# yutongwangBIT/multi_orbslam3

Hardware: AMD Instinct MI355X
Metric: tracking+localBA frames/sec (aggregate over agents; 1 agent per GPU) (higher is better)
Workload: dtype u8/int32 (ORB front-end, Hamming), f64 (local BA)

## Files before the change

include/orbgpu.h:

```cpp
#ifndef ORBGPU_H_
#define ORBGPU_H_

#include <stdint.h>

#ifdef __cplusplus
extern "C" {
#endif

enum {
  ORBG_OK = 0,
  ORBG_EMPTY = -1,
  ORBG_BAD_ARG = -2,
  ORBG_CAP_EXCEEDED = -3,
  ORBG_HIP_ERROR = -4,
  ORBG_NO_DEVICE = -5,
  ORBG_INTERNAL = -6
};

enum {
  LBA_APPLIED = 0,
  LBA_ABORTED_BEFORE_OPT = 1,
  LBA_REJECTED_OUTLIERS = 2
};

// ... 4 lines not shown
#define ORBG_MAX_FRAME_FEATURES 65535


typedef struct orbx_config {
  int32_t n_features;
  float   scale_factor;
  int32_t n_levels;
  int32_t ini_th_fast;
  int32_t min_th_fast;
  int32_t max_width;
  int32_t max_height;
  int32_t n_cams;
  int32_t device;
  int32_t gauss_taps[4];
  int32_t octree_oldest_first;
} orbx_config;

typedef struct orbx_keypoint {
  float   x, y;
  float   size;
  float   angle;
  float   response;
  int32_t octave;
} orbx_keypoint;

typedef struct orbx_handle orbx_handle;

int orbx_create(const orbx_config* cfg, orbx_handle** out);
int orbx_destroy(orbx_handle* h);

int orbx_get_tables(const orbx_handle* h, float* scale, float* inv_scale, float* sigma2,
                    float* inv_sigma2, int32_t* features_per_level);

int orbx_extract(orbx_handle* h, int cam, const uint8_t* img, int width, int height, int stride,
                 int lap0, int lap1, orbx_keypoint* kps, uint8_t* desc, int cap, int* n, int* n_mono);

int orbx_extract_stereo(orbx_handle* h, const uint8_t* img_left, const uint8_t* img_right,
                        int width, int height, int stride,
                        orbx_keypoint* kps_left, uint8_t* desc_left, int cap_left, int* n_left,
                        orbx_keypoint* kps_right, uint8_t* desc_right, int cap_right, int* n_right);

int orbx_extract_stereo_dev(orbx_handle* h, const uint8_t* d_img_left, const uint8_t* d_img_right,
                            int width, int height, int stride,
                            orbx_keypoint* kps_left, uint8_t* desc_left, int cap_left, int* n_left,
                            orbx_keypoint* kps_right, uint8_t* desc_right, int cap_right, int* n_right);

int orbx_get_level(orbx_handle* h, int cam, int level, uint8_t* host_out, int* width, int* height);
int orbx_get_level_bordered(orbx_handle* h, int cam, int level, uint8_t* host_out, int* width, int* height);

int orbx_get_candidates(orbx_handle* h, int cam, int level, int32_t* xys, int cap, int* n);

int orbx_stereo_match(orbx_handle* h, float bf, float b, float* uright, float* depth);


typedef struct orbm_frame_view {
  int32_t n;
  const orbx_keypoint* kps;
  const uint8_t* desc;
  const float* uright;
  const float* depth;
  float min_x, max_x, min_y, max_y;
  float fx, fy, cx, cy, bf, b;
  int32_t n_levels;
  float   scale_factor;
} orbm_frame_view;

typedef struct orbm_frame orbm_frame;

int orbm_frame_create(int device, int cap_features, orbm_frame** out);
int orbm_frame_destroy(orbm_frame* f);
int orbm_frame_upload(orbm_frame* f, const orbm_frame_view* view);
int orbm_frame_from_extractor(orbm_frame* f, orbx_handle* h, const orbm_frame_view* view);
int orbx_frame_stereo(orbx_handle* h, orbm_frame* frame, const orbm_frame_view* view, const uint8_t* img_left,
                      const uint8_t* img_right, int width, int height, int stride, float bf, float b,
                      orbx_keypoint* kps_left, uint8_t* desc_left, float* uright, float* depth, int cap_left,
                      int* n_left, int* n_right);
int orbx_frame_stereo_dev(orbx_handle* h, orbm_frame* frame, const orbm_frame_view* view, const uint8_t* d_img_left,
                          const uint8_t* d_img_right, int width, int height, int stride, float bf, float b,
                          orbx_keypoint* kps_left, uint8_t* desc_left, float* uright, float* depth, int cap_left,
                          int* n_left, int* n_right);
int orbx_frame_stereo_dev_submit(orbx_handle* h, orbm_frame* frame, const orbm_frame_view* view, const uint8_t* d_img_left,
                                 const uint8_t* d_img_right, int width, int height, int stride, float bf, float b);
int orbx_frame_stereo_dev_wait(orbx_handle* h, int* n_left, int* n_right);
#define ORBX_SUBMIT_ASYNC 1
int orbx_set_frame_outputs(orbx_handle* h, orbx_keypoint* kps_left, uint8_t* desc_left, float* uright, float* depth, int cap_left);
int orbx_frame_stereo_submit(orbx_handle* h, orbm_frame* frame, const orbm_frame_view* view, const uint8_t* img_left,
                             const uint8_t* img_right, int width, int height, int stride, float bf, float b, int flags);
int orbx_frame_stereo_wait(orbx_handle* h, int* n_left, int* n_right);
typedef struct orbx_distortion { float k1, k2, p1, p2, k3; } orbx_distortion;
int orbx_frame_mono(orbx_handle* h, orbm_frame* frame, const orbm_frame_view* view, const orbx_distortion* dist, const uint8_t* img,
                    int width, int height, int stride, orbx_keypoint* kps, orbx_keypoint* kps_un, uint8_t* desc, int cap, int* n);
int orbx_frame_mono_dev(orbx_handle* h, orbm_frame* frame, const orbm_frame_view* view, const orbx_distortion* dist, const uint8_t* d_img,
                        int width, int height, int stride, orbx_keypoint* kps, orbx_keypoint* kps_un, uint8_t* desc, int cap, int* n);
int orbx_frame_mono_submit(orbx_handle* h, orbm_frame* frame, const orbm_frame_view* view, const orbx_distortion* dist, const uint8_t* img,
                           int width, int height, int stride, int flags);
int orbx_frame_mono_dev_submit(orbx_handle* h, orbm_frame* frame, const orbm_frame_view* view, const orbx_distortion* dist,
                               const uint8_t* d_img, int width, int height, int stride);
int orbx_frame_mono_wait(orbx_handle* h, int* n);
int orbx_set_frame_outputs_un(orbx_handle* h, orbx_keypoint* kps_un );
int orbx_undistort_points(int device, const float* xy_in, int n, float fx, float fy, float cx, float cy, const orbx_distortion* dist,
                          float* xy_out);
int orbm_frame_get_grid(orbm_frame* f, int32_t* cell_start , int32_t* cell_items );

int orbm_hamming_matrix(int device, const uint8_t* q, int nq, const uint8_t* t, int nt, int32_t* dist);
int orbm_hamming_best2(int device, const uint8_t* q, int nq, const uint8_t* t, int nt, int32_t* out4);

typedef struct orbm_mappoints_view {
  int32_t m;
  const uint8_t* track_in_view;
  const uint8_t* bad;
  const float* proj_x;
  const float* proj_y;
  const float* proj_xr;
  const float* track_depth;
  const int32_t* scale_level;
  const float* view_cos;
  const uint8_t* desc;
  const int32_t* n_obs;
} orbm_mappoints_view;

typedef struct orbm_worldpoints_view {
  int32_t m;
  const float* pos;
  const float* normal;
  const float* min_dist;
  const float* max_dist;
  const uint8_t* desc;
  const int32_t* n_obs;
  const uint8_t* bad;
  const uint8_t* skip;
} orbm_worldpoints_view;

int orbm_is_in_frustum(orbm_frame* f, const float* Tcw , const orbm_worldpoints_view* pts,
                       float viewing_cos_limit, uint8_t* track_in_view, float* proj_x, float* proj_y,
                       float* proj_xr, float* track_depth, int32_t* scale_level, float* view_cos);

int orbm_search_by_projection_mps(orbm_frame* f, const orbm_mappoints_view* mps, float th,
                                  int far_points, float th_far_points, float nnratio,
                                  int32_t* assigned_mp, int32_t* assigned_obs, int* nmatches);

typedef struct orbm_map orbm_map;
int orbm_map_create(int device, int cap_points, orbm_map** out);
int orbm_map_destroy(orbm_map* m);
int orbm_map_upload(orbm_map* m, const orbm_worldpoints_view* pts);
int orbm_map_set_observations(orbm_map* m, const int32_t* n_obs );
int orbm_search_local_points(orbm_frame* f, orbm_map* m, const float* Tcw, const uint8_t* skip ,
                             float th, int far_points, float th_far_points, float nnratio,
                             int32_t* assigned_mp, int32_t* assigned_obs, int* nmatches);
int orbm_search_local_points_vis(orbm_frame* f, orbm_map* m, const float* Tcw, const uint8_t* skip ,
                                 float th, int far_points, float th_far_points, float nnratio,
                                 int32_t* assigned_mp, int32_t* assigned_obs, int* nmatches, uint8_t* in_frustum );

typedef struct orbm_lastframe_view {
  int32_t n;
  const uint8_t* mp_valid;
  const uint8_t* outlier;
  const float* world_pos;
  const uint8_t* desc;
  const int32_t* octave;
  const float* angle;
  const int32_t* n_obs;
  float Tcw[16];
} orbm_lastframe_view;

int orbm_search_by_projection_frame(orbm_frame* cur, const float* Tcw_cur, const orbm_lastframe_view* last,
                                    float th, int mono, int check_orientation,
                                    int32_t* assigned_mp, int32_t* assigned_obs, int* nmatches);

typedef struct orbm_lastview orbm_lastview;
int orbm_lastview_create(int device, int cap_features, orbm_lastview** out);
int orbm_lastview_destroy(orbm_lastview* v);
int orbm_lastview_upload(orbm_lastview* v, const orbm_lastframe_view* last);
int orbm_search_by_projection_frame_resident(orbm_frame* cur, const float* Tcw_cur, orbm_lastview* last, float th, int mono,
                                             int check_orientation, int32_t* assigned_mp, int32_t* assigned_obs, int* nmatches);

typedef struct orbm_featvec_view {
  int32_t n_nodes;
  const uint32_t* node_id;
  const uint32_t* start;
  const uint32_t* feat_idx;
} orbm_featvec_view;

int orbm_search_by_bow(orbm_frame* f, const orbm_featvec_view* fv_frame,
                       const uint8_t* kf_desc, int nkf, const uint8_t* kf_mp_valid, const float* kf_angle,
                       const orbm_featvec_view* fv_kf, float nnratio, int check_orientation,
                       int32_t* matches, int* nmatches);

int orbm_search_by_projection_sim3(orbm_frame* kf, orbm_map* pts, const float* Scw ,
                                   const uint8_t* already_found, int th, float ratio_hamming, int camera_project,
                                   int32_t* matched, int* nmatches);

int orbm_search_by_projection_reloc(orbm_frame* cur, orbm_map* kf_points, const float* Tcw_cur , const uint8_t* already_found ,
                                    const float* kf_angle , float th, int orb_dist, int check_orientation,
                                    int32_t* assigned_mp, int* nmatches);
struct orbg_camera;
int orbm_search_by_projection_sim3_cam(orbm_frame* kf, orbm_map* pts, const float* Scw , const struct orbg_camera* cam,
                                       const uint8_t* already_found, int th, float ratio_hamming, int32_t* matched, int* nmatches);
int orbm_search_by_projection_reloc_cam(orbm_frame* cur, orbm_map* kf_points, const float* Tcw_cur , const struct orbg_camera* cam,
                                        const uint8_t* already_found , const float* kf_angle , float th, int orb_dist,
                                        int check_orientation, int32_t* assigned_mp, int* nmatches);
int orbm_search_by_bow_kf(orbm_frame* kf2, const orbm_featvec_view* fv2, const uint8_t* mp_valid2,
                          const uint8_t* desc1, int n1, const uint8_t* mp_valid1, const float* angle1,
                          const orbm_featvec_view* fv1, float nnratio, int check_orientation,
                          int32_t* matches12, int* nmatches);

typedef struct orbm_sim3_problem {
  uint32_t struct_size;
  int32_t  n;
  const float* X3Dc1;
  const float* X3Dc2;
  const uint32_t* max_err1;
  const uint32_t* max_err2;
  float fx1, fy1, cx1, cy1;
  float fx2, fy2, cx2, cy2;
  int32_t camera_model1, camera_model2;
  int32_t fix_scale;
} orbm_sim3_problem;

typedef struct orbm_sim3_params {
  double  probability;
  int32_t min_inliers;
  int32_t max_iterations;
} orbm_sim3_params;

typedef struct orbm_sim3_result {
  uint32_t struct_size;
  int32_t  no_more;
  int32_t  converged;
  int32_t  n_inliers;
  int32_t  iterations_done;
  int32_t  iterations_run;
  int32_t  improved_in_this_call;
  int32_t  best_iteration;
  int32_t  have_best;
  float    T12[16];
  float    R[9];
  float    t[3];
  float    s;
  uint8_t* inliers;
  int32_t* hyp_n_inliers;
  float*   hyp_T12;
  uint64_t* hyp_masks;
} orbm_sim3_result;

typedef struct orbm_sim3 orbm_sim3;

int orbm_sim3_create(int device, orbm_sim3** out);
int orbm_sim3_destroy(orbm_sim3* h);
int orbm_sim3_set_stream(orbm_sim3* h, void* hip_stream);
int orbm_sim3_set_problem(orbm_sim3* h, const orbm_sim3_problem* p);
int orbm_sim3_set_ransac_parameters(orbm_sim3* h, double probability, int min_inliers, int max_iterations);
int orbm_sim3_ransac_iterations(int n, double probability, int min_inliers, int max_iterations, int* out);
int orbm_sim3_resolve_draws(int n, const int32_t* draws, int n_iterations, int32_t* idx);
int orbm_sim3_iterate(orbm_sim3* h, int n_iterations, const int32_t* draws, orbm_sim3_result* result);
int orbm_sim3_solve_batch(int device, const orbm_sim3_problem* problems, int B, const orbm_sim3_params* params,
                          const int32_t* const* draws, orbm_sim3_result* results);

// ... 340 lines not shown
```

multi_orbslam3_amd/_capi.py:

```python
import ctypes as C
import os

import numpy as np

_HERE = os.path.dirname(os.path.abspath(__file__))
LIB_PATH = os.environ.get("ORBG_LIB") or os.path.join(_HERE, "liborbgpu.so")

ORBG_OK, ORBG_EMPTY, ORBG_BAD_ARG, ORBG_CAP_EXCEEDED, ORBG_HIP_ERROR, ORBG_NO_DEVICE, ORBG_INTERNAL = 0, -1, -2, -3, -4, -5, -6
LBA_APPLIED, LBA_ABORTED_BEFORE_OPT, LBA_REJECTED_OUTLIERS = 0, 1, 2
GRID_COLS, GRID_ROWS = 64, 48

u8p = C.POINTER(C.c_uint8)
i32p = C.POINTER(C.c_int32)
u32p = C.POINTER(C.c_uint32)
f32p = C.POINTER(C.c_float)
f64p = C.POINTER(C.c_double)

KEYPOINT_DTYPE = np.dtype([("x", "<f4"), ("y", "<f4"), ("size", "<f4"), ("angle", "<f4"),
                           ("response", "<f4"), ("octave", "<i4")])
EDGE_DTYPE = np.dtype([("pose", "<i4"), ("point", "<i4"), ("u", "<f4"), ("v", "<f4"), ("ur", "<f4"),
                       ("inv_sigma2", "<f4")])
assert KEYPOINT_DTYPE.itemsize == 24 and EDGE_DTYPE.itemsize == 24


# ... 136 lines not shown
                ("obs1", C.c_void_p), ("obs2", C.c_void_p), ("inv_sigma2_1", C.c_void_p), ("inv_sigma2_2", C.c_void_p),
                ("fx1", C.c_float), ("fy1", C.c_float), ("cx1", C.c_float), ("cy1", C.c_float),
                ("fx2", C.c_float), ("fy2", C.c_float), ("cx2", C.c_float), ("cy2", C.c_float),
                ("camera_model1", C.c_int32), ("camera_model2", C.c_int32), ("fix_scale", C.c_int32), ("th2", C.c_float),
                ("q", C.c_double * 4), ("t", C.c_double * 3), ("s", C.c_double), ("n_correspondences", C.c_int32)]


class Sim3OptResult(C.Structure):
    _fields_ = [("struct_size", C.c_uint32), ("n_in", C.c_int32), ("returned_early", C.c_int32), ("n_bad_round1", C.c_int32),
                ("q", C.c_double * 4), ("t", C.c_double * 3), ("s", C.c_double), ("removed", C.c_void_p),
                ("iters", C.c_int32 * 2), ("chi2", C.c_double * 2), ("trace", C.c_void_p), ("trace_cap", C.c_int32),
                ("trace_len", C.c_int32), ("edge_chi2", C.c_void_p)]


class NewPointsKF(C.Structure):
    _fields_ = [("struct_size", C.c_uint32), ("frame", C.c_void_p), ("featvec", FeatVecView), ("has_mp", C.c_void_p),
                ("keys_xy", C.c_void_p), ("Tcw", C.c_float * 12), ("Twc", C.c_float * 12), ("Ow", C.c_float * 3),
                ("fx", C.c_float), ("fy", C.c_float), ("cx", C.c_float), ("cy", C.c_float), ("invfx", C.c_float),
                ("invfy", C.c_float), ("mb", C.c_float), ("mbf", C.c_float), ("n_levels", C.c_int32),
                ("scale_factors", C.c_void_p), ("level_sigma2", C.c_void_p), ("scale_factor", C.c_float)]


class NewPointsParams(C.Structure):
    _fields_ = [("struct_size", C.c_uint32), ("only_stereo", C.c_int32), ("coarse", C.c_int32), ("check_orientation", C.c_int32),
                ("far_points", C.c_int32), ("th_far_points", C.c_float)]


NEWPOINTS_MAX_NEIGHBOURS = 64
(NP_ACCEPTED, NP_HAS_POINT, NP_NOT_STEREO, NP_NO_NODE, NP_NO_MATCH, NP_W_ZERO, NP_LOW_PARALLAX, NP_EMPTY, NP_Z1, NP_Z2, NP_REPROJ1,
 NP_REPROJ2, NP_DIST_ZERO, NP_FAR, NP_SCALE) = range(15)
NEWPOINTS_RECORD_DTYPE = np.dtype([("idx2", "<i4"), ("dist", "<i4"), ("status", "<i4"), ("x3D", "<f4", (3,)), ("w", "<f4"),
                                   ("cos_parallax", "<f4")])
NEWPOINT_DTYPE = np.dtype([("neighbour", "<i4"), ("idx1", "<i4"), ("idx2", "<i4"), ("x3D", "<f4", (3,))])
assert NEWPOINTS_RECORD_DTYPE.itemsize == 32 and NEWPOINT_DTYPE.itemsize == 24


class FuseKF(C.Structure):
    _fields_ = [("struct_size", C.c_uint32), ("frame", C.c_void_p), ("Tcw", C.c_float * 12), ("Ow", C.c_float * 3),
                ("Scw", C.c_float * 16), ("fx", C.c_float), ("fy", C.c_float), ("cx", C.c_float), ("cy", C.c_float),
                ("mbf", C.c_float), ("n_levels", C.c_int32), ("scale_factors", C.c_void_p), ("inv_level_sigma2", C.c_void_p),
                ("log_scale_factor", C.c_float)]


class FuseParams(C.Structure):
    _fields_ = [("struct_size", C.c_uint32), ("th", C.c_float), ("sim3_form", C.c_int32)]


FUSE_MAX_KEYFRAMES, FUSE_CAND_CAP = 512, 16
(FUSE_CANDIDATES, FUSE_NEG_DEPTH, FUSE_NOT_IN_IMAGE, FUSE_DISTANCE, FUSE_NORMAL, FUSE_EMPTY_WINDOW, FUSE_NO_CANDIDATE,
 FUSE_SKIPPED) = range(8)
FUSE_RECORD_DTYPE = np.dtype([("status", "<i4"), ("best_idx", "<i4"), ("best_dist", "<i4"), ("level", "<i4"), ("n_cand", "<i4")])
assert FUSE_RECORD_DTYPE.itemsize == 20


class PoseOptResult(C.Structure):
    _fields_ = [("Tcw", C.c_float * 16), ("outlier", C.c_void_p), ("n_inliers", C.c_int32), ("n_bad", C.c_int32),
                ("iters", C.c_int32 * 4), ("chi2", C.c_double * 4)]


def ptr(a):
    if a is None:
        return None
    assert a.flags["C_CONTIGUOUS"], "array must be C-contiguous"
    return a.ctypes.data


EXPORTED_SYMBOLS = [
    "orbx_create", "orbx_destroy", "orbx_get_tables", "orbx_extract", "orbx_extract_stereo",
    "orbx_extract_stereo_dev", "orbx_get_level", "orbx_get_level_bordered", "orbx_get_candidates", "orbx_stereo_match",
    "orbm_frame_create", "orbm_frame_destroy", "orbm_frame_upload", "orbm_frame_from_extractor", "orbx_frame_stereo_dev", "orbx_frame_stereo", "orbx_frame_stereo_dev_submit", "orbx_frame_stereo_dev_wait", "orbx_frame_stereo_submit", "orbx_frame_stereo_wait", "orbx_set_frame_outputs",
    "orbm_frame_get_grid", "orbm_hamming_matrix", "orbm_hamming_best2", "orbm_is_in_frustum",
    "orbm_search_by_projection_mps", "orbm_is_in_frustum_rig", "orbm_search_by_projection_mps_rig", "orbm_search_by_projection_frame_rig", "orbm_search_by_bow_rig", "orbx_fisheye_stereo_matches", "orbm_map_create", "orbm_map_destroy", "orbm_map_upload",
    "orbm_search_local_points", "orbm_search_local_points_vis", "orbm_search_by_projection_frame", "orbm_search_by_bow",
    "orbm_search_by_projection_sim3", "orbm_search_by_bow_kf",
    "orbv_vocab_create", "orbv_vocab_destroy", "orbv_text_load", "orbv_text_view", "orbv_text_free", "orbv_vocab_from_text", "orbv_transform", "orbv_transform_frame", "orbv_bow_assemble",
    "orbm_distinctive_descriptors", "orbv_score_l1", "orbk_wire_bytes", "orbk_pack_frame", "orbk_frame_from_wire",
    "orbm_frame_download",
    "lba_solve", "lba_create", "lba_destroy", "lba_solve_h", "lba_solve_async", "lba_wait", "pose_optimize",
    "lba_solve_b", "lba_solve_hb", "lba_solve_async_b",
    "lba_set_profiling", "lba_get_solver_stats", "lba_event_overhead", "lba_get_watchdog_count",
    "orbd_database_create", "orbd_database_destroy", "orbd_detect_n_best_candidates",
    "orbx_set_stream", "orbm_frame_set_stream", "orbm_map_set_stream", "lba_set_stream", "orbv_vocab_set_stream", "orbd_database_set_stream",
    "pose_opt_set_stream", "orbx_get_ctor_timeline", "orbm_map_set_observations", "orbm_search_by_projection_reloc", "orbm_search_by_projection_reloc_cam", "orbm_search_by_projection_sim3_cam", "orbm_lastview_create", "orbm_lastview_destroy", "orbm_lastview_upload",
    "orbm_search_by_projection_frame_resident", "orbg_quiesce", "orbg_set_wait_policy", "orbg_get_wait_policy",
    "orbx_frame_mono", "orbx_frame_mono_dev", "orbx_frame_mono_submit", "orbx_frame_mono_dev_submit", "orbx_frame_mono_wait",
    "orbx_set_frame_outputs_un", "orbx_undistort_points",
    "orbm_sim3_create", "orbm_sim3_destroy", "orbm_sim3_set_stream", "orbm_sim3_set_problem", "orbm_sim3_set_ransac_parameters",
    "orbm_sim3_ransac_iterations", "orbm_sim3_resolve_draws", "orbm_sim3_iterate", "orbm_sim3_solve_batch",
    "orbm_sim3_optimize", "orbm_sim3_optimize_batch",
    "orbm_create_new_points", "orbm_search_for_triangulation", "orbm_fuse",
    "orbg_version", "orbg_strerror", "orbg_device_count", "orbx_get_timings", "orbx_event_overhead", "orbx_set_profile_interval", "orbx_set_profile_kernel", "orbx_get_fast_kernel_stats", "orbx_set_profiling",
]

_lib = None


class OrbGpuError(RuntimeError):
    def __init__(self, code, where=""):
        self.code = code
        msg = "orbgpu error %d" % code
        try:
            msg += " (%s)" % load().orbg_strerror(code).decode()
        except Exception:
            pass
        super().__init__(msg + (" in " + where if where else ""))


def load():
    global _lib
    if _lib is not None:
        return _lib
    if not os.path.exists(LIB_PATH):
        raise ImportError("liborbgpu.so not built: run `python -c 'import __graft_entry__ as g; g.build()'` "
                          "(expected at %s). There is no CPU fallback." % LIB_PATH)
    try:
        import torch
    except ImportError:
        pass
    lib = C.CDLL(LIB_PATH)
    lib.orbg_version.restype = C.c_char_p
    lib.orbg_strerror.restype = C.c_char_p
    lib.orbg_strerror.argtypes = [C.c_int]
    lib.orbm_sim3_ransac_iterations.argtypes = [C.c_int, C.c_double, C.c_int, C.c_int, C.c_void_p]
    lib.orbm_sim3_set_ransac_parameters.argtypes = [C.c_void_p, C.c_double, C.c_int, C.c_int]
    lib.orbm_sim3_optimize.argtypes = [C.c_int, C.c_void_p, C.c_void_p]
    lib.orbm_sim3_optimize_batch.argtypes = [C.c_int, C.c_void_p, C.c_int, C.c_void_p]
    lib.orbm_create_new_points.argtypes = [C.c_void_p, C.c_void_p, C.c_int, C.c_void_p, C.c_void_p, C.c_int, C.c_void_p, C.c_void_p, C.c_void_p]
    lib.orbm_search_for_triangulation.argtypes = [C.c_void_p, C.c_void_p, C.c_void_p, C.c_void_p, C.c_int, C.c_void_p]
    lib.orbm_fuse.argtypes = [C.c_void_p, C.c_int, C.c_void_p, C.c_void_p, C.c_void_p, C.c_void_p, C.c_void_p]
    for name in EXPORTED_SYMBOLS:
        fn = getattr(lib, name)
        if name not in ("orbg_version", "orbg_strerror"):
            fn.restype = C.c_int
    _lib = lib
    return lib


def check(code, where=""):
    if code != ORBG_OK:
        raise OrbGpuError(code, where)
```

multi_orbslam3_amd/api.py:

```python
import ctypes as C

import numpy as np

from . import _capi as capi
from . import views


def _vp(a):
    return None if a is None else C.c_void_p(a.ctypes.data)


class ORBextractor:

    def __init__(self, nfeatures=1000, scaleFactor=1.2, nlevels=8, iniThFAST=20, minThFAST=7, max_width=640,
                 max_height=480, n_cams=1, device=0, gauss_taps=None, octree_oldest_first=False):
        self.lib = capi.load()
        self.cfg = capi.OrbxConfig(nfeatures, scaleFactor, nlevels, iniThFAST, minThFAST, max_width, max_height,
                                   n_cams, device, (C.c_int32 * 4)(*(gauss_taps or (0, 0, 0, 0))), int(bool(octree_oldest_first)))
        self.h = C.c_void_p()
        capi.check(self.lib.orbx_create(C.byref(self.cfg), C.byref(self.h)), "orbx_create")
        self.cap = 2 * nfeatures + 256

    def close(self):
        if getattr(self, "h", None):
# ... 65 lines not shown
        if download_left:
            return nl.value, nr.value, kl[: nl.value], dl[: nl.value]
        return nl.value, nr.value

    def frame_stereo(self, frame, fv, im_left, im_right, bf, b, download=True):
        im_left = np.ascontiguousarray(im_left, np.uint8)
        im_right = np.ascontiguousarray(im_right, np.uint8)
        self._host_imgs = (im_left, im_right)
        return self.frame_stereo_dev(frame, fv, im_left.ctypes.data, im_right.ctypes.data, im_left.shape[1], im_left.shape[0],
                                     im_left.strides[0], bf, b, download, _fn=self.lib.orbx_frame_stereo)

    def frame_stereo_dev_submit(self, frame, fv, d_left, d_right, width, height, stride, bf, b):
        self._pending = (frame, fv)
        rc = self.lib.orbx_frame_stereo_dev_submit(self.h, frame.h if frame is not None else None, C.byref(fv), C.c_void_p(d_left),
                                                   C.c_void_p(d_right), width, height, stride, C.c_float(bf), C.c_float(b))
        capi.check(rc, "orbx_frame_stereo_dev_submit")

    def frame_stereo_submit(self, frame, fv, im_left, im_right, bf, b, async_ingest=False):
        assert im_left.dtype == np.uint8 and im_right.dtype == np.uint8 and im_left.shape == im_right.shape
        assert im_left.strides[1] == 1 and im_right.strides == im_left.strides
        self._pending = (frame, fv, im_left, im_right)
        rc = self.lib.orbx_frame_stereo_submit(self.h, frame.h if frame is not None else None, C.byref(fv), C.c_void_p(im_left.ctypes.data),
                                               C.c_void_p(im_right.ctypes.data), im_left.shape[1], im_left.shape[0], im_left.strides[0],
                                               C.c_float(bf), C.c_float(b), 1 if async_ingest else 0)
        capi.check(rc, "orbx_frame_stereo_submit")

    def set_frame_outputs(self, cap):
        if cap <= 0:
            capi.check(self.lib.orbx_set_frame_outputs(self.h, None, None, None, None, 0), "orbx_set_frame_outputs")
            self._outputs = None
            return None
        out = dict(kps=np.zeros(cap, capi.KEYPOINT_DTYPE), desc=np.zeros((cap, 32), np.uint8), uright=np.zeros(cap, np.float32),
                   depth=np.zeros(cap, np.float32), kps_un=np.zeros(cap, capi.KEYPOINT_DTYPE))
        capi.check(self.lib.orbx_set_frame_outputs(self.h, C.c_void_p(capi.ptr(out["kps"])), C.c_void_p(capi.ptr(out["desc"])),
                                                   C.c_void_p(capi.ptr(out["uright"])), C.c_void_p(capi.ptr(out["depth"])), int(cap)),
                   "orbx_set_frame_outputs")
        capi.check(self.lib.orbx_set_frame_outputs_un(self.h, C.c_void_p(capi.ptr(out["kps_un"]))), "orbx_set_frame_outputs_un")
        self._outputs = out
        return out

    @staticmethod
    def _dist(dist):
        if dist is None:
            return None, None
        d = dist if isinstance(dist, capi.OrbxDistortion) else capi.OrbxDistortion(*([float(v) for v in dist] + [0.0] * (5 - len(dist))))
        return d, C.byref(d)

    def frame_mono(self, frame, fv, image, dist=None, download=True, device_ptr=None, size=None):
        n = C.c_int(0)
        kps = kun = desc = None
        if download:
            kps = np.zeros(self.cap, capi.KEYPOINT_DTYPE); kun = np.zeros(self.cap, capi.KEYPOINT_DTYPE); desc = np.zeros((self.cap, 32), np.uint8)
        dk, darg = self._dist(dist)
        if device_ptr is not None:
            w, h, stride = size
            rc = self.lib.orbx_frame_mono_dev(self.h, frame.h if frame is not None else None, C.byref(fv), darg, C.c_void_p(device_ptr), w, h, stride,
                                              _vp(kps), _vp(kun), _vp(desc), self.cap, C.byref(n))
        else:
            image = np.ascontiguousarray(image, np.uint8)
            rc = self.lib.orbx_frame_mono(self.h, frame.h if frame is not None else None, C.byref(fv), darg, _vp(image), image.shape[1],
                                          image.shape[0], image.strides[0], _vp(kps), _vp(kun), _vp(desc), self.cap, C.byref(n))
        capi.check(rc, "orbx_frame_mono")
        if frame is not None:
            frame.n = n.value
        if download:
            return n.value, kps[: n.value].copy(), kun[: n.value].copy(), desc[: n.value].copy()
        return n.value

    def frame_mono_submit(self, frame, fv, image, dist=None, async_ingest=False, device_ptr=None, size=None):
        dk, darg = self._dist(dist)
        if device_ptr is not None:
            w, h, stride = size
            self._pending = (frame, fv, dk)
            rc = self.lib.orbx_frame_mono_dev_submit(self.h, frame.h if frame is not None else None, C.byref(fv), darg, C.c_void_p(device_ptr), w, h, stride)
        else:
            assert image.dtype == np.uint8 and image.strides[1] == 1
            self._pending = (frame, fv, dk, image)
            rc = self.lib.orbx_frame_mono_submit(self.h, frame.h if frame is not None else None, C.byref(fv), darg, C.c_void_p(image.ctypes.data),
                                                 image.shape[1], image.shape[0], image.strides[0], 1 if async_ingest else 0)
        capi.check(rc, "orbx_frame_mono_submit")

    def frame_mono_wait(self):
        return self.frame_stereo_dev_wait()[0]

    def frame_stereo_dev_wait(self):
        nl, nr = C.c_int(0), C.c_int(0)
        capi.check(self.lib.orbx_frame_stereo_dev_wait(self.h, C.byref(nl), C.byref(nr)), "orbx_frame_stereo_dev_wait")
        frame = self._pending[0] if getattr(self, "_pending", None) else None
        if frame is not None:
            frame.n = nl.value
        self._pending = None
        return nl.value, nr.value

    def frame_stereo_dev(self, frame, fv, d_left, d_right, width, height, stride, bf, b, download=False, _fn=None):
        nl, nr = C.c_int(0), C.c_int(0)
        kl = dl = ur = dp = None
        if download:
            if not hasattr(self, "_kl"):
                self._kl = np.zeros(self.cap, capi.KEYPOINT_DTYPE)
                self._dl = np.zeros((self.cap, 32), np.uint8)
            if not hasattr(self, "_ur"):
                self._ur = np.zeros(self.cap, np.float32)
                self._dp = np.zeros(self.cap, np.float32)
            kl, dl, ur, dp = self._kl, self._dl, self._ur, self._dp
        fn = _fn if _fn is not None else self.lib.orbx_frame_stereo_dev
        rc = fn(self.h, frame.h if frame is not None else None, C.byref(fv), C.c_void_p(d_left),
                C.c_void_p(d_right), width, height, stride, C.c_float(bf), C.c_float(b), _vp(kl),
                _vp(dl), _vp(ur), _vp(dp), self.cap, C.byref(nl), C.byref(nr))
        capi.check(rc, "orbx_frame_stereo_dev")
        if frame is not None:
            frame.n = nl.value
        if download:
            n = nl.value
            return n, nr.value, kl[:n], dl[:n], ur[:n], dp[:n]
        return nl.value, nr.value

    def level(self, cam, level, border=False):
        w, h = C.c_int(0), C.c_int(0)
        fn = self.lib.orbx_get_level_bordered if border else self.lib.orbx_get_level
        capi.check(fn(self.h, cam, level, None, C.byref(w), C.byref(h)))
        e = 38 if border else 0
        out = np.zeros((h.value + e, w.value + e), np.uint8)
        capi.check(fn(self.h, cam, level, _vp(out), C.byref(w), C.byref(h)))
        return out

    def candidates(self, cam, level, cap=1 << 18):
        out = np.zeros((cap, 3), np.int32)
        n = C.c_int(0)
        capi.check(self.lib.orbx_get_candidates(self.h, cam, level, _vp(out), cap, C.byref(n)))
        return out[: n.value].copy()

    def ComputeStereoMatches(self, bf, b, n_left=None, download=True):
        if not download:
            capi.check(self.lib.orbx_stereo_match(self.h, C.c_float(bf), C.c_float(b), None, None))
            return None
        ur = np.zeros(max(n_left if n_left is not None else self.cap, 1), np.float32)
        dp = np.zeros_like(ur)
        capi.check(self.lib.orbx_stereo_match(self.h, C.c_float(bf), C.c_float(b), _vp(ur), _vp(dp)), "orbx_stereo_match")
        if n_left is not None:
            return ur[:n_left], dp[:n_left]
        return ur, dp

    def ctor_timeline(self, reset=False):
        out = np.zeros((512, 5), np.float32)
        n = C.c_int(0)
        capi.check(self.lib.orbx_get_ctor_timeline(self.h, _vp(out), 512, C.byref(n), int(bool(reset))), "orbx_get_ctor_timeline")
        return out[: n.value].copy()

    def set_profiling(self, level):
        capi.check(self.lib.orbx_set_profiling(self.h, int(level)))

    def set_profile_interval(self, interval, reset=True):
        capi.check(self.lib.orbx_set_profile_interval(self.h, int(interval), int(bool(reset))), "orbx_set_profile_interval")

    PROF_KERNELS = {"fast_cells_kernel": 0, "octree_kernel": 1, "orient_desc_gpu_kernel": 2, "pyr_tower_kernel": 3}

    def set_profile_kernel(self, name):
        capi.check(self.lib.orbx_set_profile_kernel(self.h, self.PROF_KERNELS[name]), "orbx_set_profile_kernel")

    def fast_kernel_stats(self):
        s, n = C.c_double(0.0), C.c_int64(0)
        capi.check(self.lib.orbx_get_fast_kernel_stats(self.h, C.byref(s), C.byref(n)), "orbx_get_fast_kernel_stats")
        return s.value, n.value

    def event_overhead_ms(self, reps=50):
        ms = C.c_float(0.0)
# ... 177 lines not shown

    def DescriptorDistance(self, q, t):
        q = np.ascontiguousarray(q, np.uint8).reshape(-1, 32)
        t = np.ascontiguousarray(t, np.uint8).reshape(-1, 32)
        d = np.zeros((len(q), len(t)), np.int32)
        capi.check(self.lib.orbm_hamming_matrix(self.device, _vp(q), len(q), _vp(t), len(t), _vp(d)), "orbm_hamming_matrix")
        return d

    def best2(self, q, t):
        q = np.ascontiguousarray(q, np.uint8).reshape(-1, 32)
        t = np.ascontiguousarray(t, np.uint8).reshape(-1, 32)
        o = np.zeros((len(q), 4), np.int32)
        capi.check(self.lib.orbm_hamming_best2(self.device, _vp(q), len(q), _vp(t), len(t), _vp(o)), "orbm_hamming_best2")
        return o

    def SearchByProjection(self, F, mv, th=1.0, bFarPoints=False, thFarPoints=50.0, assigned_mp=None, assigned_obs=None):
        amp = np.ascontiguousarray(assigned_mp, np.int32).copy()
        aob = np.ascontiguousarray(assigned_obs, np.int32).copy()
        n = C.c_int(0)
        capi.check(self.lib.orbm_search_by_projection_mps(F.h, C.byref(mv), C.c_float(th), int(bFarPoints),
                                                          C.c_float(thFarPoints), C.c_float(self.mfNNratio), _vp(amp),
                                                          _vp(aob), C.byref(n)), "orbm_search_by_projection_mps")
        return amp, aob, n.value

    def SearchByProjectionRig(self, FL, FR, mv, mv_r, left_to_right, right_to_left, th=1.0, bFarPoints=False, thFarPoints=50.0,
                              assigned_mp=None, assigned_obs=None):
        amp = np.ascontiguousarray(assigned_mp, np.int32).copy()
        aob = np.ascontiguousarray(assigned_obs, np.int32).copy()
        l2r = np.ascontiguousarray(left_to_right, np.int32); r2l = np.ascontiguousarray(right_to_left, np.int32)
        n = C.c_int(0)
        capi.check(self.lib.orbm_search_by_projection_mps_rig(FL.h, FR.h, C.byref(mv), C.byref(mv_r), _vp(l2r), _vp(r2l), C.c_float(th),
                                                              int(bFarPoints), C.c_float(thFarPoints), C.c_float(self.mfNNratio), _vp(amp),
                                                              _vp(aob), C.byref(n)), "orbm_search_by_projection_mps_rig")
        return amp, aob, n.value

    def SearchByProjectionFrameRig(self, FL, FR, Tcw_cur, rig, lv, th, bMono=False, assigned_mp=None, assigned_obs=None):
        amp = np.ascontiguousarray(assigned_mp, np.int32).copy()
        aob = np.ascontiguousarray(assigned_obs, np.int32).copy()
        T = np.ascontiguousarray(Tcw_cur, np.float32).reshape(16)
        n = C.c_int(0)
        capi.check(self.lib.orbm_search_by_projection_frame_rig(FL.h, FR.h if FR is not None else None, _vp(T), C.byref(rig), C.byref(lv), C.c_float(th), int(bMono),
                                                                int(self.mbCheckOrientation), _vp(amp), _vp(aob), C.byref(n)),
                   "orbm_search_by_projection_frame_rig")
        return amp, aob, n.value

    def SearchLocalPoints(self, F, local_map, Tcw, th=1.0, bFarPoints=False, thFarPoints=50.0, assigned_mp=None,
                          assigned_obs=None, skip=None, inplace=False, in_frustum=None):
        amp, aob = self._state(assigned_mp, assigned_obs, inplace)
        T = np.ascontiguousarray(Tcw, np.float32).reshape(16)
        sk = None if skip is None else np.ascontiguousarray(skip, np.uint8)
        n = C.c_int(0)
        if in_frustum is not None:
            assert in_frustum.dtype == np.uint8 and in_frustum.flags["C_CONTIGUOUS"]
        capi.check(self.lib.orbm_search_local_points_vis(F.h, local_map.h, _vp(T), _vp(sk), C.c_float(th), int(bFarPoints),
                                                         C.c_float(thFarPoints), C.c_float(self.mfNNratio), _vp(amp), _vp(aob),
                                                         C.byref(n), _vp(in_frustum)), "orbm_search_local_points")
        return amp, aob, n.value

    @staticmethod
    def _state(assigned_mp, assigned_obs, inplace):
        if inplace:
            assert assigned_mp.dtype == np.int32 and assigned_obs.dtype == np.int32
            return assigned_mp, assigned_obs
        return np.ascontiguousarray(assigned_mp, np.int32).copy(), np.ascontiguousarray(assigned_obs, np.int32).copy()

    def SearchByProjectionFrame(self, CurrentFrame, Tcw_cur, lv, th, bMono, assigned_mp, assigned_obs, inplace=False):
        amp, aob = self._state(assigned_mp, assigned_obs, inplace)
        T = np.ascontiguousarray(Tcw_cur, np.float32).reshape(16)
        n = C.c_int(0)
        capi.check(self.lib.orbm_search_by_projection_frame(CurrentFrame.h, _vp(T), C.byref(lv), C.c_float(th), int(bMono),
                                                            int(self.mbCheckOrientation), _vp(amp), _vp(aob), C.byref(n)),
                   "orbm_search_by_projection_frame")
        return amp, aob, n.value

    def SearchByProjectionFrameResident(self, CurrentFrame, Tcw_cur, last_on_device, th, bMono, assigned_mp, assigned_obs):
        amp, aob = self._state(assigned_mp, assigned_obs, False)
        T = np.ascontiguousarray(Tcw_cur, np.float32).reshape(16)
        n = C.c_int(0)
        capi.check(self.lib.orbm_search_by_projection_frame_resident(CurrentFrame.h, _vp(T), last_on_device.h, C.c_float(th), int(bool(bMono)),
                                                                     int(self.mbCheckOrientation), _vp(amp), _vp(aob), C.byref(n)),
                   "orbm_search_by_projection_frame_resident")
        return amp, aob, n.value

    def SearchByBoW(self, F, fvF, kf_desc, kf_mp_valid, kf_angle, fvK):
        kf_desc = np.ascontiguousarray(kf_desc, np.uint8)
        kf_mp_valid = np.ascontiguousarray(kf_mp_valid, np.uint8)
        kf_angle = np.ascontiguousarray(kf_angle, np.float32)
        matches = np.zeros(max(F.n, 1), np.int32)
        n = C.c_int(0)
        capi.check(self.lib.orbm_search_by_bow(F.h, C.byref(fvF), _vp(kf_desc), len(kf_desc), _vp(kf_mp_valid), _vp(kf_angle),
                                               C.byref(fvK), C.c_float(self.mfNNratio), int(self.mbCheckOrientation),
                                               _vp(matches), C.byref(n)), "orbm_search_by_bow")
        return matches[: F.n].copy(), n.value


    def SearchByBoWRig(self, F, n_left, fvF, kf_desc, kf_mp_valid, kf_angle, fvK):
        kf_desc = np.ascontiguousarray(kf_desc, np.uint8)
        kf_mp_valid = np.ascontiguousarray(kf_mp_valid, np.uint8)
        kf_angle = np.ascontiguousarray(kf_angle, np.float32)
        matches = np.zeros(max(F.n, 1), np.int32)
        n = C.c_int(0)
        capi.check(self.lib.orbm_search_by_bow_rig(F.h, int(n_left), C.byref(fvF), _vp(kf_desc), len(kf_desc), _vp(kf_mp_valid), _vp(kf_angle),
                                                   C.byref(fvK), C.c_float(self.mfNNratio), int(self.mbCheckOrientation), _vp(matches), C.byref(n)),
                   "orbm_search_by_bow_rig")
        return matches[: F.n].copy(), n.value

    def SearchByProjectionSim3(self, pKF, Scw, points, vpMatched, th, ratioHamming=1.0, already_found=None, with_kfs=False, camera=None):
        matched = np.ascontiguousarray(vpMatched, np.int32).copy()
        S = np.ascontiguousarray(Scw, np.float32).reshape(16)
        af = None if already_found is None else np.ascontiguousarray(already_found, np.uint8)
        n = C.c_int(0)
        if camera is not None:
            capi.check(self.lib.orbm_search_by_projection_sim3_cam(pKF.h, points.h, _vp(S), C.byref(camera), _vp(af), int(th), C.c_float(ratioHamming),
                                                                   _vp(matched), C.byref(n)), "orbm_search_by_projection_sim3_cam")
            return matched, n.value
        capi.check(self.lib.orbm_search_by_projection_sim3(pKF.h, points.h, _vp(S), _vp(af), int(th), C.c_float(ratioHamming),
                                                           0 if with_kfs else 1, _vp(matched), C.byref(n)),
                   "orbm_search_by_projection_sim3")
        return matched, n.value

    def SearchByProjectionReloc(self, CurrentFrame, Tcw, kf_points, kf_angle, assigned_mp, th, ORBdist, already_found=None, camera=None):
        amp = np.ascontiguousarray(assigned_mp, np.int32).copy()
        T = np.ascontiguousarray(Tcw, np.float32).reshape(16)
        ang = np.ascontiguousarray(kf_angle, np.float32)
        af = None if already_found is None else np.ascontiguousarray(already_found, np.uint8)
        n = C.c_int(0)
        if camera is not None:
            capi.check(self.lib.orbm_search_by_projection_reloc_cam(CurrentFrame.h, kf_points.h, _vp(T), C.byref(camera), _vp(af), _vp(ang), C.c_float(th),
                                                                    int(ORBdist), int(self.mbCheckOrientation), _vp(amp), C.byref(n)),
                       "orbm_search_by_projection_reloc_cam")
            return amp, n.value
        capi.check(self.lib.orbm_search_by_projection_reloc(CurrentFrame.h, kf_points.h, _vp(T), _vp(af), _vp(ang), C.c_float(th), int(ORBdist),
                                                            int(self.mbCheckOrientation), _vp(amp), C.byref(n)),
                   "orbm_search_by_projection_reloc")
        return amp, n.value

    def SearchByBoWKF(self, pKF2, fv2, mp_valid2, desc1, mp_valid1, angle1, fv1):
        desc1 = np.ascontiguousarray(desc1, np.uint8)
        mp_valid1 = np.ascontiguousarray(mp_valid1, np.uint8)
        mp_valid2 = np.ascontiguousarray(mp_valid2, np.uint8)
        angle1 = np.ascontiguousarray(angle1, np.float32)
        matches = np.zeros(max(len(desc1), 1), np.int32)
        n = C.c_int(0)
        capi.check(self.lib.orbm_search_by_bow_kf(pKF2.h, C.byref(fv2), _vp(mp_valid2), _vp(desc1), len(desc1), _vp(mp_valid1),
                                                  _vp(angle1), C.byref(fv1), C.c_float(self.mfNNratio),
                                                  int(self.mbCheckOrientation), _vp(matches), C.byref(n)),
                   "orbm_search_by_bow_kf")
        return matches[: len(desc1)].copy(), n.value


class ORBVocabulary:

    def __init__(self, view, keep=None, device=0):
        self.lib = capi.load()
        self.h = C.c_void_p()
        self._keep = keep
        if view is not None:
            capi.check(self.lib.orbv_vocab_create(device, C.byref(view), C.byref(self.h)), "orbv_vocab_create")

    @classmethod
    def loadFromTextFile(cls, path, device=0, keep_trailing_node=False):
        voc = cls(None, None, device)
        flags = capi.ORBV_TEXT_KEEP_TRAILING_NODE if keep_trailing_node else 0
        capi.check(voc.lib.orbv_vocab_from_text(int(device), str(path).encode(), flags, C.byref(voc.h)), "orbv_vocab_from_text")
        return voc

# ... 627 lines not shown
```

multi_orbslam3_amd/csrc/agent_loop.cpp:

```cpp
#include <time.h>

#include <cstdint>
#include <cstring>
#include <vector>

#include "../../include/orbgpu.h"

extern "C" {

typedef struct agent_frame_in {
  const uint8_t* host_left; const uint8_t* host_right;
  const uint8_t* dev_left; const uint8_t* dev_right;
  const float* Tcw_guess;
  const orbm_lastframe_view* last_view;
} agent_frame_in;

typedef struct agent_cfg {
  orbx_handle* ex[4]; orbm_frame* fr[4];
  orbm_map* local_map; lba_handle* lba;
  const orbm_frame_view* frame_view;
  int width, height, stride; float bf, b;
  const agent_frame_in* frames; int n_frames;
  const int32_t* seq; int n_seq;
  const orbm_worldpoints_view* const* kf_maps; int n_kf_maps;
  const lba_problem* lba_prob; lba_result* lba_out;
  const pose_opt_problem* po[2]; pose_opt_result* po_out[2];
  int frames_per_kf;
  int pipelined, host_images, ingest_async, submit_first, lba_async, pose_opt;
  float th_frame; int mono; float nn_frame, nn_map;
  int32_t* amp; int32_t* aob; int cap;
  int32_t in_flight[4];
  int32_t ahead, ring;
  int32_t lba_in_flight;
  orbm_lastview* last_view_dev;
  int32_t last_view_frame;
  int32_t* amp_after_frame;
  int32_t mono_agent;
  const orbx_distortion* dist;
  orbx_keypoint* sync_kps; orbx_keypoint* sync_kps_un; uint8_t* sync_desc; float* sync_uright; float* sync_depth; int32_t sync_cap;
} agent_cfg;

typedef struct agent_stats {
  double stage_s[8];
  double lba_s; int64_t lba_calls, lba_iters;
  int64_t kp, m_frame, m_map;
  int32_t error, error_step;
  double worst_step_s, worst_stage_s[8];
  int64_t worst_step_index;
  int32_t last_nl, last_nr, last_n1, last_n2;
} agent_stats;

int agent_sizeof(int which) { return which == 0 ? (int)sizeof(agent_cfg) : which == 1 ? (int)sizeof(agent_stats) : (int)sizeof(agent_frame_in); }

static inline double now_s() { timespec t; clock_gettime(CLOCK_MONOTONIC, &t); return (double)t.tv_sec + 1e-9 * (double)t.tv_nsec; }

static int submit_ctor(agent_cfg* c, int slot, int k) {
  const agent_frame_in& f = c->frames[k];
  if (c->mono_agent) {
    if (c->host_images)
      return orbx_frame_mono_submit(c->ex[slot], c->fr[slot], c->frame_view, c->dist, f.host_left, c->width, c->height, c->stride,
                                    c->ingest_async ? ORBX_SUBMIT_ASYNC : 0);
    return orbx_frame_mono_dev_submit(c->ex[slot], c->fr[slot], c->frame_view, c->dist, f.dev_left, c->width, c->height, c->stride);
  }
  if (c->host_images)
    return orbx_frame_stereo_submit(c->ex[slot], c->fr[slot], c->frame_view, f.host_left, f.host_right, c->width, c->height, c->stride, c->bf, c->b,
                                    c->ingest_async ? ORBX_SUBMIT_ASYNC : 0);
  return orbx_frame_stereo_dev_submit(c->ex[slot], c->fr[slot], c->frame_view, f.dev_left, f.dev_right, c->width, c->height, c->stride, c->bf, c->b);
}

static int collect_lba(agent_cfg* c, agent_stats* st, int timed) {
  if (!c->lba_in_flight) return ORBG_OK;
  double ms = 0;
  const int rc = lba_wait(c->lba, &ms);
  c->lba_in_flight = 0;
  if (rc) return rc;
  if (timed && st) { st->lba_s += 1e-3 * ms; st->lba_calls++; st->lba_iters += c->lba_out->iters_round1 + c->lba_out->iters_round2; }
  return ORBG_OK;
}

int agent_run(agent_cfg* c, int64_t first_step, int n_steps, int last_is_final, int timed, double* step_s, agent_stats* st) {
  if (!c || !st || n_steps < 0) return ORBG_BAD_ARG;
  int rc = ORBG_OK, s_done = 0;
  for (int s = 0; s < n_steps && rc == ORBG_OK; s++) {
    s_done = s;
    const int64_t i = first_step + s;
    const int k = c->seq[i % c->n_seq], k_last = c->seq[(i + c->n_seq - 1) % c->n_seq];
    const agent_frame_in& fin = c->frames[k];
    const double t0 = now_s();
    int nl = 0, nr = 0, cur = 0;
    if (c->pipelined) {
      const int ring = c->ring < 2 ? 2 : c->ring > 4 ? 4 : c->ring, ahead = c->ahead < 1 ? 1 : c->ahead > ring - 1 ? ring - 1 : c->ahead;
      cur = (int)(i % ring);
      auto submit_ahead = [&](int d0, int d1) -> int {
        for (int d = d0; d <= d1; d++) {
          const int slot = (int)((i + d) % ring);
          if (c->in_flight[slot] || (last_is_final && s + d >= n_steps)) continue;
          const int r = submit_ctor(c, slot, c->seq[(i + d) % c->n_seq]);
          if (r) return r;
          c->in_flight[slot] = 1;
        }
        return ORBG_OK;
      };
      if ((rc = submit_ahead(0, 0))) break;
      if (!c->submit_first || (rc = submit_ahead(1, ahead)) == ORBG_OK) rc = orbx_frame_stereo_dev_wait(c->ex[cur], &nl, &nr);
      if (rc) break;
      c->in_flight[cur] = 0;
      if (!c->submit_first && (rc = submit_ahead(1, ahead))) break;
    } else if (c->mono_agent) {
      rc = c->host_images ? orbx_frame_mono(c->ex[0], c->fr[0], c->frame_view, c->dist, fin.host_left, c->width, c->height, c->stride, c->sync_kps,
                                            c->sync_kps_un, c->sync_desc, c->sync_cap, &nl)
                          : orbx_frame_mono_dev(c->ex[0], c->fr[0], c->frame_view, c->dist, fin.dev_left, c->width, c->height, c->stride, c->sync_kps,
                                                c->sync_kps_un, c->sync_desc, c->sync_cap, &nl);
    } else if (c->host_images) {
      rc = orbx_frame_stereo(c->ex[0], c->fr[0], c->frame_view, fin.host_left, fin.host_right, c->width, c->height, c->stride, c->bf, c->b,
                             c->sync_kps, c->sync_desc, c->sync_uright, c->sync_depth, c->sync_cap, &nl, &nr);
    } else {
      rc = orbx_frame_stereo_dev(c->ex[0], c->fr[0], c->frame_view, fin.dev_left, fin.dev_right, c->width, c->height, c->stride, c->bf, c->b,
                                 c->sync_kps, c->sync_desc, c->sync_uright, c->sync_depth, c->sync_cap, &nl, &nr);
    }
    if (rc) break;
    if (nl > c->cap) { rc = ORBG_CAP_EXCEEDED; break; }
    orbm_frame* F = c->fr[cur];
    const double t1 = now_s();
    for (int j = 0; j < nl; j++) c->amp[j] = -1;
    memset(c->aob, 0, sizeof(int32_t) * (size_t)nl);
    int n1 = 0, n2 = 0;
    if (c->last_view_dev) {
      if (c->last_view_frame != k_last) {
        if ((rc = orbm_lastview_upload(c->last_view_dev, c->frames[k_last].last_view))) break;
        c->last_view_frame = k_last;
      }
      if ((rc = orbm_search_by_projection_frame_resident(F, fin.Tcw_guess, c->last_view_dev, c->th_frame, c->mono, 1, c->amp, c->aob, &n1))) break;
    } else if ((rc = orbm_search_by_projection_frame(F, fin.Tcw_guess, c->frames[k_last].last_view, c->th_frame, c->mono, 1, c->amp, c->aob, &n1))) break;
    if (c->amp_after_frame) memcpy(c->amp_after_frame, c->amp, sizeof(int32_t) * (size_t)nl);
    const double t2 = now_s();
    double t_po = 0;
    if (c->pose_opt && c->po[0]) {
      const double a = now_s();
      if ((rc = pose_optimize(c->po[0], c->po_out[0]))) break;
      t_po += now_s() - a;
    }
    const double t2b = now_s();
    if ((rc = orbm_search_local_points(F, c->local_map, fin.Tcw_guess, nullptr, 1.0f, 0, 0.0f, c->nn_map, c->amp, c->aob, &n2))) break;
    const double t3 = now_s();
    if (c->pose_opt && c->po[1]) {
      const double a = now_s();
      if ((rc = pose_optimize(c->po[1], c->po_out[1]))) break;
      t_po += now_s() - a;
    }
    double t_lv = 0;
    if (c->last_view_dev) {
      const double a = now_s();
      if ((rc = orbm_lastview_upload(c->last_view_dev, fin.last_view))) break;
      c->last_view_frame = k;
      t_lv = now_s() - a;
    }
    const double t4 = now_s();
    double t5 = t4, t6 = t4;
    if (i % c->frames_per_kf == 0) {
      if ((rc = orbm_map_upload(c->local_map, c->kf_maps[(i / c->frames_per_kf) % c->n_kf_maps]))) break;
      t5 = now_s();
      if (c->lba_async) {
        if ((rc = collect_lba(c, st, timed))) break;
        if ((rc = lba_solve_async(c->lba, c->lba_prob, nullptr, c->lba_out))) break;
        c->lba_in_flight = 1;
      } else {
        const double a = now_s();
        if ((rc = lba_solve_h(c->lba, c->lba_prob, nullptr, c->lba_out))) break;
        if (timed) { st->lba_s += now_s() - a; st->lba_calls++; st->lba_iters += c->lba_out->iters_round1 + c->lba_out->iters_round2; }
      }
      t6 = now_s();
    }
    st->last_nl = nl; st->last_nr = nr; st->last_n1 = n1; st->last_n2 = n2;
    if (timed) {
      st->stage_s[0] += t1 - t0; st->stage_s[1] += t2 - t1; st->stage_s[2] += t3 - t2b; st->stage_s[3] += t_po;
      st->stage_s[4] += t5 - t4; st->stage_s[5] += t6 - t5; st->stage_s[6] += t_lv;
      st->kp += nl + nr; st->m_frame += n1; st->m_map += n2;
      const double t_step = now_s() - t0;
      if (step_s) step_s[s] = t_step;
      if (t_step > st->worst_step_s) {
        st->worst_step_s = t_step;
        st->worst_step_index = i;
        const double w[8] = {t1 - t0, t2 - t1, t3 - t2b, t_po, t5 - t4, t6 - t5, t_lv, 0.0};
        for (int q = 0; q < 8; q++) st->worst_stage_s[q] = w[q];
      }
    }
  }
  st->error = rc;
  if (rc) st->error_step = (int32_t)s_done;
  return rc;
}

int agent_drain(agent_cfg* c, agent_stats* st, int timed) {
  if (!c) return ORBG_BAD_ARG;
  int rc = collect_lba(c, st, timed);
  for (int s = 0; s < 4; s++)
    if (c->in_flight[s]) {
      int nl, nr;
      const int r2 = orbx_frame_stereo_dev_wait(c->ex[s], &nl, &nr);
      c->in_flight[s] = 0;
      if (!rc) rc = r2;
    }
  return rc;
}

}
```

multi_orbslam3_amd/csrc/extractor.hip:

```cpp

#include "common.hpp"
#include "wave.hpp"
#include "stereo_finalize.hpp"
#include "grid_build.hpp"

#include <algorithm>
#include <atomic>
#include <chrono>
#include <cmath>
#include <condition_variable>
#include <functional>
#include <memory>
#include <mutex>
#include <thread>

using namespace orbg;

namespace {


struct LevelGeom {
  int w, h;
  int stride;
  int off;
// ... 1845 lines not shown
  return ORBG_OK;
}



extern "C" int orbx_destroy(orbx_handle* h) {
  if (!h) return ORBG_BAD_ARG;
  (void)hipSetDevice(h->device);
  while (h->ingest_state.load(std::memory_order_acquire) == 1) std::this_thread::yield();
  (void)hipStreamSynchronize(h->stream);
  h->d_pyr.release(); h->d_img.release(); h->h_img.release(); h->up_ready.release(); h->d_xtab.release(); h->d_ytab.release(); h->d_tower_x.release(); h->d_tower_y.release(); h->d_cells.release();
  h->d_slots.release(); h->d_counts.release(); h->hdr.release(); h->cand.release(); h->sel.release();
  h->d_kps.release(); h->d_desc.release(); h->h_kps.release(); h->h_desc.release();
  h->d_uright.release(); h->d_depth.release(); h->d_sad.release(); h->h_stereo.release();
  h->d_cand.release(); h->d_hdr.release(); h->d_lvlcount.release(); h->d_nkp.release(); h->d_overflow.release();
  h->d_selreg.release(); h->h_nkp.release(); h->sig.release();
  for (auto& e : h->ev) if (e) (void)hipEventDestroy(e);
  if (!h->ext_stream) orbg::release_stream(h->stream);
  delete_pending(h->pending);
  delete h;
  return ORBG_OK;
}

extern "C" int orbx_get_tables(const orbx_handle* h, float* scale, float* inv_scale, float* sigma2, float* inv_sigma2,
                               int32_t* fpl) {
  if (!h) return ORBG_BAD_ARG;
  for (int i = 0; i < h->cfg.n_levels; i++) {
    if (scale) scale[i] = h->scale[i];
    if (inv_scale) inv_scale[i] = h->inv_scale[i];
    if (sigma2) sigma2[i] = h->sigma2[i];
    if (inv_sigma2) inv_sigma2[i] = h->inv_sigma2[i];
    if (fpl) fpl[i] = h->feats_per_level[i];
  }
  return ORBG_OK;
}

struct PostOps {
  bool stereo = false;
  float bf = 0, b = 0;
  float* uright = nullptr;
  float* depth = nullptr;
  orbm_frame* frame = nullptr;
  const orbm_frame_view* view = nullptr;
  bool mono = false, undist = false;
  orbx_distortion dist{};
  orbx_keypoint* kps_un_out = nullptr;
};
struct ExtractPending {
  bool active = false;
  bool finished = false;
  unsigned cams_mask = 0;
  const uint8_t* d_img0 = nullptr; const uint8_t* d_img1 = nullptr;
  int w = 0, hgt = 0, stride = 0, ncams = 0, prof = 0;
  int lap[2][2] = {{0, 0}, {0, 0}};
  orbx_keypoint* kps_out[2] = {nullptr, nullptr};
  uint8_t* desc_out[2] = {nullptr, nullptr};
  int cap[2] = {0, 0};
  int* n_out[2] = {nullptr, nullptr};
  int* n_mono_out[2] = {nullptr, nullptr};
  bool has_post = false;
  PostOps post;
  orbm_frame_view view_copy;
  int reverse[2] = {0, 0};
  bool stereo_out = false;
  int n_res[2] = {0, 0};
};
static void delete_pending(ExtractPending* p) { delete p; }
int orbm_internal_attach(orbm_frame* f, orbx_handle* h, const orbm_frame_view* v, int n, hipStream_t stream, const int* d_n,
                         volatile unsigned* done_flag, unsigned done_seq, const StereoFinalizeArgs* fin, const orbg::UndistortArgs* un = nullptr,
                         bool mono = false);
static int make_undistort_args(orbx_handle* h, const PostOps* post, orbg::UndistortArgs* ua) {
  memset(ua, 0, sizeof(*ua));
  if (!post || !post->undist) return ORBG_OK;
  const size_t cap = h->d_kps.cap;
  int rc;
  if ((rc = h->d_kps_un.reserve(cap)) || (rc = h->h_kps_un.reserve(cap))) return rc;
  ua->on = 1;
  ua->fx = post->view->fx; ua->fy = post->view->fy; ua->cx = post->view->cx; ua->cy = post->view->cy;
  ua->k1 = post->dist.k1; ua->k2 = post->dist.k2; ua->p1 = post->dist.p1; ua->p2 = post->dist.p2; ua->k3 = post->dist.k3;
  ua->src = h->d_kps.p; ua->dst = h->d_kps_un.p; ua->dst_host = h->h_kps_un.d;
  return ORBG_OK;
}
void orbm_internal_set_n(orbm_frame* f, int n);
int orbx_internal_kp_capacity(orbx_handle* h);
static int launch_stereo(orbx_handle* h, float bf, float b, hipStream_t st, bool device_counts, float* host_mirror,
                         StereoFinalizeArgs* defer_finalize = nullptr);

static int extract_core(orbx_handle* h, unsigned cams_mask, const uint8_t* d_img0, const uint8_t* d_img1, int w, int hgt,
                        int stride, const int lap[2][2], orbx_keypoint* kps_out[2], uint8_t* desc_out[2], const int cap[2],
                        int* n_out[2], int* n_mono_out[2], const PostOps* post = nullptr, bool force_host = false,
                        bool submit_only = false);
static int extract_finish_gpu(orbx_handle* h, ExtractPending& c);

static int extract_core(orbx_handle* h, unsigned cams_mask, const uint8_t* d_img0, const uint8_t* d_img1, int w, int hgt,
                        int stride, const int lap[2][2], orbx_keypoint* kps_out[2], uint8_t* desc_out[2], const int cap[2],
                        int* n_out[2], int* n_mono_out[2], const PostOps* post, bool force_host, bool submit_only) {
  if (h->pending && h->pending->active) return ORBG_BAD_ARG;
  int rc = setup_geometry(h, w, hgt);
  if (rc) return rc;
  const PyrGeom& g = h->geom;
  const int nl = g.n_levels;
  const int ncams = (cams_mask & 2) ? 2 : 1;
  if (cams_mask == 2) return ORBG_BAD_ARG;
  const int n_cells = (int)h->cells.size();
  hipStream_t st = h->stream;
  int prof = h->profile;
  if (prof == 1 && h->profile_interval > 1 && (h->extract_calls % (unsigned)h->profile_interval) != 0) prof = 0;
  h->extract_calls++;
  bool use_gpu = h->gpu_octree && n_cells > 0 && !force_host;
  int reverse[2] = {0, 0};
  for (int c = 0; c < ncams && use_gpu; c++) {
    const float xmin = (float)kEdge, xmax = (float)w;
    if ((float)lap[c][1] < xmin || (float)lap[c][0] > xmax) reverse[c] = 0;
    else if ((float)lap[c][0] <= xmin && (float)lap[c][1] >= xmax) reverse[c] = 1;
    else use_gpu = false;
  }
  h->last_was_gpu = use_gpu;
  if (!use_gpu) h->pool->prepare();
  const bool want_desc = desc_out[0] || desc_out[1];
  const bool do_stereo = use_gpu && post && post->stereo && ncams == 2;
  const bool stereo_out = do_stereo && (post->uright || post->depth);
  OctCfg oc = h->octcfg;
  oc.n_cams = ncams;
  const uint8_t* const img1 = d_img1 ? d_img1 : d_img0;
  auto launch_chain = [&](int prof_) -> int {
    if (prof_ >= 2) ORBG_HIP(hipEventRecord(h->ev[0], st));
    const int pk = h->prof_kernel;
    auto br0 = [&](int which) -> int { if (prof_ >= 1 && pk == which) ORBG_HIP(hipEventRecord(h->ev[1], st)); return ORBG_OK; };
    auto br1 = [&](int which) -> int { if (prof_ >= 1 && pk == which) ORBG_HIP(hipEventRecord(h->ev[7], st)); return ORBG_OK; };
    if (br0(ORBX_PROF_PYRAMID)) return ORBG_HIP_ERROR;
    if (h->tower_T > 0) {
      hipLaunchKernelGGL(pyr_tower_kernel, dim3(h->tower_ntx, h->tower_nty, ncams), dim3(kTwThreads), 0, st, d_img0, img1,
                         stride, h->d_pyr.p, g, h->d_xtab.p, h->d_ytab.p, h->d_tower_x.p, h->d_tower_y.p);
    } else {
      const LevelGeom& L0 = g.lv[0];
      dim3 grid((L0.w + 2 * kEdge + 63) / 64, (L0.h + 2 * kEdge + 3) / 4, ncams);
      hipLaunchKernelGGL(pyr_level0_kernel, grid, dim3(256), 0, st, d_img0, img1, stride, h->d_pyr.p, g);
      for (int l = 1; l < nl; l++) {
        const LevelGeom& L = g.lv[l];
        dim3 gr((L.w + 2 * kEdge + 63) / 64, (L.h + 2 * kEdge + 3) / 4, ncams);
        hipLaunchKernelGGL(pyr_resize_kernel, gr, dim3(256), 0, st, h->d_pyr.p, g, l, h->d_xtab.p, h->d_ytab.p);
      }
    }
    if (br1(ORBX_PROF_PYRAMID)) return ORBG_HIP_ERROR;
    if (prof_ >= 2 && pk != ORBX_PROF_FAST) ORBG_HIP(hipEventRecord(h->ev[8], st));
    if (n_cells > 0) {
      if (br0(ORBX_PROF_FAST)) return ORBG_HIP_ERROR;
      hipLaunchKernelGGL(fast_cells_kernel, dim3(8 * ((n_cells + 7) / 8), ncams), dim3(256), 0, st, h->d_pyr.p, g, h->d_cells.p, n_cells,
                         std::max(h->cfg.ini_th_fast, 1), std::max(h->cfg.min_th_fast, 1), h->d_slots.p, h->d_counts.p);
      if (br1(ORBX_PROF_FAST)) return ORBG_HIP_ERROR;
      if (!use_gpu)
        hipLaunchKernelGGL(gather_cells_kernel, dim3(n_cells, ncams), dim3(256), 0, st, h->d_slots.p, h->d_counts.p, g,
                           h->d_cells.p, n_cells, ncams, use_gpu ? h->d_hdr.p : h->hdr.d, use_gpu ? h->d_cand.p : h->cand.d, h->cand_cap);
    }
    if (use_gpu) {
      if (br0(ORBX_PROF_OCTREE)) return ORBG_HIP_ERROR;
      hipLaunchKernelGGL(octree_kernel, dim3(ncams * nl), dim3(kOctThreads), 0, st, h->d_cand.p, h->d_hdr.p, g, oc,
                         h->d_selreg.p, h->d_lvlcount.p, h->d_overflow.p, h->cand_cap, h->d_slots.p, h->d_counts.p, n_cells);
      if (br1(ORBX_PROF_OCTREE)) return ORBG_HIP_ERROR;
      if (br0(ORBX_PROF_ORIENT_DESC)) return ORBG_HIP_ERROR;
      auto launch_od = [&](auto kern) {
        hipLaunchKernelGGL(kern, dim3((h->sel_bound + kKpPerBlock - 1) / kKpPerBlock), dim3(256), 0, st, h->d_pyr.p, g,
                           oc, h->d_selreg.p, h->d_lvlcount.p, h->umax, reverse[0], reverse[1], h->d_kps.p, h->d_desc.p, h->h_kps.d,
                           want_desc ? h->h_desc.d : (uint8_t*)nullptr, h->d_nkp.p, h->h_nkp.d, h->d_overflow.p);
      };
      if (h->taps_variant == 0) launch_od(orient_desc_gpu_kernel<0>);
// ... 438 lines not shown

namespace {
struct IngestJob {
  orbx_handle* h; orbm_frame* frame; orbm_frame_view view; bool has_view; const uint8_t* L; const uint8_t* R; int w, hgt, stride; float bf, b;
  bool mono = false, has_dist = false; orbx_distortion dist{};
};
struct IngestWorker {
  std::mutex mu;
  std::condition_variable cv;
  std::vector<IngestJob> q;
  std::atomic<int> queued{0};
  bool quit = false;
  std::thread th;
  static bool spin_ok() { return orbg::poll_allowed(); }
  void run() {
    orbg::set_thread_role(orbg::kRoleIngest);
    for (;;) {
      bool have = false;
      if (spin_ok()) {
        const auto t0 = std::chrono::steady_clock::now();
        for (unsigned spins = 0;; spins++) {
          if (queued.load(std::memory_order_acquire) > 0) { have = true; break; }
#if defined(__x86_64__)
          __builtin_ia32_pause();
#endif
          if ((spins & 0xFF) == 0xFF && std::chrono::steady_clock::now() - t0 > std::chrono::microseconds(400)) break;
        }
      }
      IngestJob job;
      {
        std::unique_lock<std::mutex> lk(mu);
        if (!have) cv.wait(lk, [this]() { return quit || !q.empty(); });
        if (quit && q.empty()) return;
        if (q.empty()) continue;
        job = q.front();
        q.erase(q.begin());
        queued.fetch_sub(1, std::memory_order_acq_rel);
      }
      job.h->ingest_rc = frame_submit_impl(job.h, job.frame, job.has_view ? &job.view : nullptr, job.L, job.R, false, job.w, job.hgt,
                                           job.stride, job.bf, job.b, job.mono, job.has_dist ? &job.dist : nullptr);
      job.h->ingest_state.store(2, std::memory_order_release);
    }
  }
  void push(const IngestJob& j) {
    {
      std::unique_lock<std::mutex> lk(mu);
      if (!th.joinable()) th = std::thread([this]() { run(); });
      q.push_back(j);
      queued.fetch_add(1, std::memory_order_acq_rel);
    }
    cv.notify_one();
  }
  ~IngestWorker() {
    { std::unique_lock<std::mutex> lk(mu); quit = true; }
    cv.notify_all();
    if (th.joinable()) th.join();
  }
};
IngestWorker& ingest_worker() { static IngestWorker w; return w; }
}

extern "C" int orbx_frame_stereo_submit(orbx_handle* h, orbm_frame* frame, const orbm_frame_view* view, const uint8_t* img_left,
                                        const uint8_t* img_right, int width, int height, int stride, float bf, float b, int flags) {
  if (!h || h->cfg.n_cams != 2) return ORBG_BAD_ARG;
  if (frame && !view) return ORBG_BAD_ARG;
  if (!img_left || !img_right || width <= 0 || height <= 0) return ORBG_EMPTY;
  if (stride < width || width > h->cfg.max_width || height > h->cfg.max_height) return ORBG_BAD_ARG;
  if (frame && !view_is_undistorted(view, width, height)) return ORBG_BAD_ARG;
  if (h->ingest_state.load(std::memory_order_acquire) != 0) return ORBG_BAD_ARG;
  if (h->pending && (h->pending->active || h->pending->finished)) return ORBG_BAD_ARG;
  h->tl_begin();
  if (!(flags & ORBX_SUBMIT_ASYNC)) return frame_submit_impl(h, frame, view, img_left, img_right, false, width, height, stride, bf, b);
  int rc = select_device(h->device);
  if (rc) return rc;
  IngestJob j;
  j.h = h; j.frame = frame; j.has_view = view != nullptr; j.L = img_left; j.R = img_right; j.w = width; j.hgt = height; j.stride = stride;
  j.bf = bf; j.b = b;
  if (view) j.view = *view;
  h->ingest_state.store(1, std::memory_order_release);
  ingest_worker().push(j);
  return ORBG_OK;
}

extern "C" int orbx_frame_stereo_dev_wait(orbx_handle* h, int* n_left, int* n_right) {
  if (!h) return ORBG_BAD_ARG;
  int rc;
  const double t_wait0 = host_now_us();
  if (h->ingest_state.load(std::memory_order_acquire) != 0) {
    for (unsigned spins = 0; h->ingest_state.load(std::memory_order_acquire) != 2; spins++) {
#if defined(__x86_64__)
      __builtin_ia32_pause();
#endif
      if (!IngestWorker::spin_ok() || (spins & 0xFFFF) == 0xFFFF) std::this_thread::yield();
    }
    rc = h->ingest_rc;
    h->ingest_state.store(0, std::memory_order_release);
    if (rc) return rc;
  }
  if (!h->pending || !(h->pending->active || h->pending->finished)) return ORBG_BAD_ARG;
  if ((rc = select_device(h->device))) return rc;
  ExtractPending& P = *h->pending;
  if (P.active) {
    P.active = false;
    rc = extract_finish_gpu(h, P);
  }
  P.finished = false;
  if (rc) return rc;
  h->tl_commit(host_now_us() - t_wait0);
  if (n_left) *n_left = P.n_res[0];
  if (n_right) *n_right = P.n_res[1];
  return ORBG_OK;
}

extern "C" int orbx_get_ctor_timeline(orbx_handle* h, float* out, int cap, int* n, int reset) {
  if (!h || !n || cap < 0 || (cap > 0 && !out)) return ORBG_BAD_ARG;
  const unsigned long long have = std::min<unsigned long long>(h->tl_n, orbx_handle::kTlCap);
  const int take = (int)std::min<unsigned long long>(have, (unsigned long long)cap);
  for (int i = 0; i < take; i++) {
    const float* e = h->tl[(h->tl_n - take + i) % orbx_handle::kTlCap];
    for (int f = 0; f < orbx_handle::kTlFields; f++) out[i * orbx_handle::kTlFields + f] = e[f];
  }
  *n = take;
  if (reset) h->tl_n = 0;
  return ORBG_OK;
}
extern "C" int orbx_set_stream(orbx_handle* h, void* hip_stream) {
  if (!h) return ORBG_BAD_ARG;
  if (h->ingest_state.load(std::memory_order_acquire) != 0 || (h->pending && (h->pending->active || h->pending->finished))) return ORBG_BAD_ARG;
  int rc = select_device(h->device);
  if (rc) return rc;
  return orbg::swap_stream(&h->stream, &h->ext_stream, hip_stream, "ex");
}

extern "C" int orbx_frame_stereo_wait(orbx_handle* h, int* n_left, int* n_right) { return orbx_frame_stereo_dev_wait(h, n_left, n_right); }

extern "C" int orbx_frame_stereo(orbx_handle* h, orbm_frame* frame, const orbm_frame_view* view, const uint8_t* img_left,
                                 const uint8_t* img_right, int width, int height, int stride, float bf, float b,
                                 orbx_keypoint* kps_left, uint8_t* desc_left, float* uright, float* depth, int cap_left,
                                 int* n_left, int* n_right) {
  if (h) h->tl_begin();
  const int rc = frame_stereo_impl(h, frame, view, img_left, img_right, false, width, height, stride, bf, b, kps_left, desc_left, uright,
                                   depth, cap_left, n_left, n_right);
  if (h && rc == ORBG_OK) h->tl_commit(0.0);
  return rc;
}

static int mono_args_ok(orbx_handle* h, orbm_frame* frame, const orbm_frame_view* view, const orbx_distortion* dist, const uint8_t* img,
                        int width, int height, int stride) {
  if (!h) return ORBG_BAD_ARG;
  if (frame && !view) return ORBG_BAD_ARG;
  if (dist_active(dist) && !frame) return ORBG_BAD_ARG;
  if (!img || width <= 0 || height <= 0) return ORBG_EMPTY;
  if (stride < width || width > h->cfg.max_width || height > h->cfg.max_height) return ORBG_BAD_ARG;
  if (frame && !dist_active(dist) && !view_is_undistorted(view, width, height)) return ORBG_BAD_ARG;
  if (frame && dist_active(dist) && !(view->fx > 0.0f && view->fy > 0.0f && view->max_x > view->min_x && view->max_y > view->min_y)) return ORBG_BAD_ARG;
  return ORBG_OK;
}

static int frame_mono_impl(orbx_handle* h, orbm_frame* frame, const orbm_frame_view* view, const orbx_distortion* dist, const uint8_t* img,
                           bool on_device, int width, int height, int stride, orbx_keypoint* kps, orbx_keypoint* kps_un, uint8_t* desc, int cap,
                           int* n) {
  if (!n) return ORBG_BAD_ARG;
  int rc = mono_args_ok(h, frame, view, dist, img, width, height, stride);
  if (rc) return rc;
  if (handle_busy(h)) return ORBG_BAD_ARG;
  if ((rc = select_device(h->device))) return rc;
  const uint8_t* d_img = img;
  if (!on_device) {
    if ((rc = setup_geometry(h, width, height))) return rc;
    if ((rc = stage_images(h, &img, 1, width, height, stride))) return rc;
    d_img = h->d_img.p;
    stride = width;
  }
  PostOps post;
  fill_mono_post(&post, frame, view, dist, kps_un);
  orbx_keypoint* ko[2] = {kps, nullptr};
  uint8_t* dout[2] = {desc, nullptr};
  const int caps[2] = {cap, 0};
// ... 73 lines not shown
  memset(&ua, 0, sizeof(ua));
  ua.on = 1; ua.fx = fx; ua.fy = fy; ua.cx = cx; ua.cy = cy; ua.k1 = dist->k1; ua.k2 = dist->k2; ua.p1 = dist->p1; ua.p2 = dist->p2; ua.k3 = dist->k3;
  hipError_t e = hipMemcpyAsync(d_in.p, xy_in, (size_t)n * 8, hipMemcpyHostToDevice, ms.s);
  if (e == hipSuccess) {
    hipLaunchKernelGGL(undistort_points_kernel, dim3((n + 255) / 256), dim3(256), 0, ms.s, ua, d_in.p, d_out.p, n);
    e = hipGetLastError();
  }
  if (e == hipSuccess) e = hipMemcpyAsync(xy_out, d_out.p, (size_t)n * 8, hipMemcpyDeviceToHost, ms.s);
  if (e == hipSuccess) e = hipStreamSynchronize(ms.s);
  d_in.release(); d_out.release();
  return e == hipSuccess ? ORBG_OK : ORBG_HIP_ERROR;
}

extern "C" int orbx_get_level(orbx_handle* h, int cam, int level, uint8_t* host_out, int* width, int* height) {
  if (!h || cam < 0 || cam >= h->cfg.n_cams || level < 0 || level >= h->cfg.n_levels || h->cur_w == 0) return ORBG_BAD_ARG;
  const LevelGeom& L = h->geom.lv[level];
  if (width) *width = L.w;
  if (height) *height = L.h;
  if (host_out) {
    int rc = select_device(h->device);
    if (rc) return rc;
    const uint8_t* src = h->d_pyr.p + (size_t)cam * h->geom.cam_stride + L.off + (size_t)kEdge * L.stride + kEdge;
    ORBG_HIP(hipMemcpy2D(host_out, L.w, src, L.stride, L.w, L.h, hipMemcpyDeviceToHost));
  }
  return ORBG_OK;
}

extern "C" int orbx_get_level_bordered(orbx_handle* h, int cam, int level, uint8_t* host_out, int* width, int* height) {
  if (!h || cam < 0 || cam >= h->cfg.n_cams || level < 0 || level >= h->cfg.n_levels || h->cur_w == 0) return ORBG_BAD_ARG;
  const LevelGeom& L = h->geom.lv[level];
  if (width) *width = L.w;
  if (height) *height = L.h;
  if (host_out) {
    int rc = select_device(h->device);
    if (rc) return rc;
    const uint8_t* src = h->d_pyr.p + (size_t)cam * h->geom.cam_stride + L.off;
    ORBG_HIP(hipMemcpy2D(host_out, L.w + 2 * kEdge, src, L.stride, L.w + 2 * kEdge, L.h + 2 * kEdge, hipMemcpyDeviceToHost));
  }
  return ORBG_OK;
}

extern "C" int orbx_get_candidates(orbx_handle* h, int cam, int level, int32_t* xys, int cap, int* n) {
  if (!h || cam < 0 || cam >= h->cfg.n_cams || level < 0 || level >= h->cfg.n_levels || !n) return ORBG_BAD_ARG;
  if (h->last_was_gpu) {
    int rc = select_device(h->device);
    if (rc) return rc;
    if (!h->cells.empty()) {
      const int ncams = h->cfg.n_cams, n_cells = (int)h->cells.size();
      hipLaunchKernelGGL(gather_cells_kernel, dim3(n_cells, ncams), dim3(256), 0, h->stream, h->d_slots.p, h->d_counts.p, h->geom,
                         h->d_cells.p, n_cells, ncams, h->d_hdr.p, h->d_cand.p, h->cand_cap);
      ORBG_HIP(hipGetLastError());
      ORBG_HIP(hipStreamSynchronize(h->stream));
    }
    std::vector<int> hdr(2 * ORBG_MAX_LEVELS + 4);
    ORBG_HIP(hipMemcpy(hdr.data(), h->d_hdr.p, hdr.size() * sizeof(int), hipMemcpyDeviceToHost));
    const PyrGeom& g = h->geom;
    const int nl = g.n_levels;
    std::vector<Cand>& cvw = h->last_cands[cam][level];
    cvw.clear();
    if (g.lv[level].cell_end != g.lv[level].cell_begin) {
      const int b = hdr[cam * ORBG_MAX_LEVELS + level];
      int nlv = level + 1;
      while (nlv < nl && g.lv[nlv].cell_end == g.lv[nlv].cell_begin) nlv++;
      const int e = nlv < nl ? hdr[cam * ORBG_MAX_LEVELS + nlv] : hdr[2 * ORBG_MAX_LEVELS + 1 + cam];
      std::vector<uint32_t> raw(std::max(e - b, 0));
      if (e > b) ORBG_HIP(hipMemcpy(raw.data(), h->d_cand.p + b, (size_t)(e - b) * 4, hipMemcpyDeviceToHost));
      for (uint32_t pk : raw) cvw.push_back(Cand{(int)(pk & 0xFFF), (int)((pk >> 12) & 0xFFF), (int)(pk >> 24)});
    }
  }
  const std::vector<Cand>& cv = h->last_cands[cam][level];
  *n = (int)cv.size();
  for (int i = 0; i < *n && i < cap; i++) { xys[3 * i] = cv[i].x; xys[3 * i + 1] = cv[i].y; xys[3 * i + 2] = cv[i].score; }
  return *n > cap ? ORBG_CAP_EXCEEDED : ORBG_OK;
}

static int extract_finish_gpu(orbx_handle* h, ExtractPending& c) {
  int rc;
  hipStream_t st = h->stream;
  if ((rc = h->sig.wait(st))) return rc;
  if (h->up_seq && h->up_ready.h && h->up_ready.h[8] == h->up_seq) return ORBG_INTERNAL;
  const PostOps* post = c.has_post ? &c.post : nullptr;
  if (h->h_nkp.h[2]) {
    ORBG_HIP(hipMemsetAsync(h->d_overflow.p, 0, sizeof(int), st));
    return extract_core(h, c.cams_mask, c.d_img0, c.d_img1, c.w, c.hgt, c.stride, c.lap, c.kps_out, c.desc_out, c.cap, c.n_out, c.n_mono_out,
                        post, true, false);
  }
  const int ncams = c.ncams;
  h->n_kp[0] = h->h_nkp.h[0];
  h->n_kp[1] = ncams == 2 ? h->h_nkp.h[1] : 0;
  int base = 0;
  for (int cam = 0; cam < ncams; cam++) {
    const int nk = h->n_kp[cam];
    if (c.n_out[cam]) *c.n_out[cam] = nk;
    if (c.n_mono_out[cam]) *c.n_mono_out[cam] = c.reverse[cam] ? 0 : nk;
    if ((c.kps_out[cam] || c.desc_out[cam]) && nk > c.cap[cam]) return ORBG_CAP_EXCEEDED;
    if (c.kps_out[cam]) memcpy(c.kps_out[cam], h->h_kps.h + base, (size_t)nk * sizeof(orbx_keypoint));
    if (c.desc_out[cam]) memcpy(c.desc_out[cam], h->h_desc.h + (size_t)base * 32, (size_t)nk * 32);
    base += nk;
  }
  if (post && post->frame) orbm_internal_set_n(post->frame, h->n_kp[0]);
  if (post && post->kps_un_out) {
    if (h->n_kp[0] > c.cap[0]) return ORBG_CAP_EXCEEDED;
    memcpy(post->kps_un_out, (post->undist && post->frame) ? h->h_kps_un.h : h->h_kps.h, (size_t)h->n_kp[0] * sizeof(orbx_keypoint));
  }
  if (c.stereo_out && h->n_kp[0] > c.cap[0]) return ORBG_CAP_EXCEEDED;
  if (c.stereo_out) {
    if (post->uright) memcpy(post->uright, h->h_stereo.h, (size_t)h->n_kp[0] * 4);
    if (post->depth) memcpy(post->depth, h->h_stereo.h + h->n_kp[0], (size_t)h->n_kp[0] * 4);
  }
  float ms;
  h->timings[2] = 0;
  if (c.prof >= 1 && hipEventElapsedTime(&ms, h->ev[1], h->ev[7]) == hipSuccess) { h->timings[5] = ms; h->fast_ms_sum += ms; h->fast_ms_n++; }
  return ORBG_OK;
}

static int launch_stereo(orbx_handle* h, float bf, float b, hipStream_t st, bool device_counts, float* host_mirror,
                         StereoFinalizeArgs* defer_finalize) {
  const int nl = device_counts ? h->sel_bound : h->n_kp[0], nr = h->n_kp[1];
  if (nl >= ORBG_MAX_FRAME_FEATURES || nr >= ORBG_MAX_FRAME_FEATURES || (device_counts && orbx_internal_kp_capacity(h) >= 2 * ORBG_MAX_FRAME_FEATURES))
    return ORBG_CAP_EXCEEDED;
  if (h->profile >= 2) ORBG_HIP(hipEventRecord(h->ev[5], st));
  if (nl > 0) {
    const int* dn = device_counts ? h->d_nkp.p : nullptr;
    hipLaunchKernelGGL(stereo_match_kernel, dim3((nl + 3) / 4), dim3(256), 0, st, h->d_pyr.p, h->geom, h->d_kps.p, h->d_desc.p,
                       nl, h->d_kps.p + nl, h->d_desc.p + (size_t)nl * 32, nr, bf, b, h->d_uright.p, h->d_depth.p, h->d_sad.p, dn);
    if (defer_finalize) *defer_finalize = StereoFinalizeArgs{h->d_uright.p, h->d_depth.p, h->d_sad.p, nl, dn, host_mirror, nullptr};
    else hipLaunchKernelGGL(stereo_finalize_kernel, dim3(1), dim3(256), 0, st, h->d_uright.p, h->d_depth.p, h->d_sad.p, nl, dn, host_mirror);
  }
  if (h->profile >= 2) ORBG_HIP(hipEventRecord(h->ev[6], st));
  return ORBG_OK;
}

extern "C" int orbx_stereo_match(orbx_handle* h, float bf, float b, float* uright, float* depth) {
  if (!h || h->cfg.n_cams != 2 || h->cur_w == 0) return ORBG_BAD_ARG;
  int rc = select_device(h->device);
  if (rc) return rc;
  const int nl = h->n_kp[0];
  hipStream_t st = h->stream;
  if ((rc = launch_stereo(h, bf, b, st, false, nullptr))) return rc;
  if (nl > 0 && (uright || depth)) {
    ORBG_HIP(hipMemcpyAsync(h->h_stereo.h, h->d_uright.p, (size_t)nl * 4, hipMemcpyDeviceToHost, st));
    ORBG_HIP(hipMemcpyAsync(h->h_stereo.h + nl, h->d_depth.p, (size_t)nl * 4, hipMemcpyDeviceToHost, st));
  }
  ORBG_HIP(hipStreamSynchronize(st));
  if (nl > 0 && uright) memcpy(uright, h->h_stereo.h, (size_t)nl * 4);
  if (nl > 0 && depth) memcpy(depth, h->h_stereo.h + nl, (size_t)nl * 4);
  float ms;
  if (h->profile >= 2 && hipEventElapsedTime(&ms, h->ev[5], h->ev[6]) == hipSuccess) h->timings[4] = ms;
  return ORBG_OK;
}

extern "C" int orbx_set_profile_kernel(orbx_handle* h, int which) {
  if (!h || which < ORBX_PROF_FAST || which > ORBX_PROF_PYRAMID) return ORBG_BAD_ARG;
  h->prof_kernel = which;
  h->fast_ms_sum = 0; h->fast_ms_n = 0;
  return ORBG_OK;
}

extern "C" int orbx_set_profile_interval(orbx_handle* h, int interval, int reset) {
  if (!h || interval < 1) return ORBG_BAD_ARG;
  h->profile_interval = interval;
  if (reset) { h->fast_ms_sum = 0; h->fast_ms_n = 0; h->extract_calls = 0; }
  return ORBG_OK;
}

extern "C" int orbx_get_fast_kernel_stats(orbx_handle* h, double* sum_ms, int64_t* n) {
// ... 47 lines not shown
```

multi_orbslam3_amd/csrc/lba.hip:

```cpp

#include <time.h>

#include <condition_variable>
#include <atomic>
#include <unistd.h>
#include <mutex>
#include <thread>

#include "common.hpp"
#include "wave.hpp"

#include <algorithm>
#include <cmath>
#include <limits>
#include <numeric>
#include <type_traits>

using namespace orbg;

#include "ldlt_mfma.hpp"
#include "ldlt_xcd.hpp"
#include "se3.hpp"

using namespace orbg_se3;
// ... 882 lines not shown
                                               const int* __restrict__ ok_flag, HostRec* __restrict__ rec, unsigned seq, int n_edge_blocks,
                                               int nL, const int* __restrict__ pt_start, const int* __restrict__ pt_edges,
                                               double* __restrict__ Hll, double* __restrict__ bl, LmIn lm) {
  int bid = (int)blockIdx.x;
  if (bid >= n_errlin_blocks) {
    bid -= n_errlin_blocks;
    if (bid < n_sort_blocks) { sort_pf_block<256, kPrep256Cap>(bid, nL, pf_start, pf_edges_w, pf_col_w, lm_mask, edges, pose_col); return; }
    bid -= n_sort_blocks;
    if (bid < kPrep256Pad) { if (St) ldltm::image_pad_range(n_unknowns, St, bid * 256 + (int)threadIdx.x, kPrep256Pad * 256); return; }
    bid -= kPrep256Pad;
    for (int i = bid * 256 + (int)threadIdx.x; i < n_zero; i += kPrep256Zero * 256) xzero[i] = 0.0;
    return;
  }

  
  if (bid < nP) {
    lin_poses_block<true>(bid, ps_start, ps_edges, edges, poses, points, c, hb, err, chi2, Hpp, bp);
  } else if (bid < nP + n_edge_blocks) {
    linearize_block<true>(bid - nP, n_edges, edges, poses, points, c, hb, err, chi2, pose_col, point_col, EB,
                          TrialPublish{partial, ticket, scale_partial, n_scale_partial, ok_flag, rec, seq, n_edge_blocks, lm});
  } else if (bid - nP - n_edge_blocks < errlin_point_blocks(nL)) {
    lin_points_block(bid - nP - n_edge_blocks, nL, pt_start, pt_edges, edges, poses, points, c, hb, Hll, bl);
  } else {
    publish_trial_when_all_arrived(n_edge_blocks, partial, ticket, scale_partial, n_scale_partial, ok_flag, rec, seq, lm);
  }
}

__global__ __launch_bounds__(kSortPfThreads) void k_prep(int n_sort_blocks, int nL, const int* __restrict__ pf_start, int* __restrict__ pf_edges,
                                                        int* __restrict__ pf_col, unsigned long long* __restrict__ lm_mask,
                                                        const lba_edge* __restrict__ edges, const int* __restrict__ pose_col,
                                                        int n, double* __restrict__ St, double* __restrict__ xzero, int n_zero) {
  constexpr int kPadBlocks = 32;
  const int bid = (int)blockIdx.x;
  if (bid < n_sort_blocks) { sort_pf_block<kSortPfThreads, kSortPfCap>(bid, nL, pf_start, pf_edges, pf_col, lm_mask, edges, pose_col); return; }
  if (bid < n_sort_blocks + kPadBlocks) {
    if (St) ldltm::image_pad_range(n, St, (bid - n_sort_blocks) * kSortPfThreads + (int)threadIdx.x, kPadBlocks * kSortPfThreads);
    return;
  }
  const int nz = (int)gridDim.x - n_sort_blocks - kPadBlocks;
  for (int i = (bid - n_sort_blocks - kPadBlocks) * kSortPfThreads + (int)threadIdx.x; i < n_zero; i += nz * kSortPfThreads) xzero[i] = 0.0;
}

__device__ __forceinline__ void build_items_block(int pr, int nP, int nL, const unsigned long long* __restrict__ lm_mask,
                                                  const int* __restrict__ pf_start, const int* __restrict__ pf_edges,
                                                  const int* __restrict__ pf_col, PairItem* __restrict__ items, int cap,
                                                  int* __restrict__ pair_count) {
  __shared__ int wcount[4];
  const int tid = threadIdx.x, lane = tid & 63, wv = tid >> 6;
  int i1 = 0, rem = pr;
  while (rem >= nP - i1) { rem -= nP - i1; i1++; }
  const int i2 = i1 + rem;
  const unsigned long long need = (1ull << i1) | (1ull << i2);
  PairItem* out = items + (size_t)pr * cap;
  int running = 0;
  for (int l0 = 0; l0 < nL; l0 += 256) {
    const int l = l0 + tid;
    const unsigned long long m = l < nL ? lm_mask[l] : 0ull;
    const bool has = (m & need) == need;
    const unsigned long long bal = __ballot(has);
    if (lane == 0) wcount[wv] = __popcll(bal);
    __syncthreads();
    int before = 0, total = 0;
#pragma unroll
    for (int w = 0; w < 4; w++) { const int c = wcount[w]; if (w < wv) before += c; total += c; }
    if (has) {
      const int pos = running + before + __popcll(bal & ((1ull << lane) - 1ull));
      const int b0 = pf_start[l];
      const int ea = pf_edges[b0 + __popcll(m & ((1ull << i1) - 1ull))];
      const int eb = pf_edges[b0 + __popcll(m & ((1ull << i2) - 1ull))];
      if (pos < cap) out[pos] = PairItem{ea, eb, l};
    }
    running += total;
    __syncthreads();
  }
  if (tid == 0) pair_count[pr] = min(running, cap);
}
__global__ __launch_bounds__(256) void k_build_items(int nP, int nL, const unsigned long long* __restrict__ lm_mask,
                                                    const int* __restrict__ pf_start, const int* __restrict__ pf_edges,
                                                    const int* __restrict__ pf_col, PairItem* __restrict__ items, int cap,
                                                    int* __restrict__ pair_count) {
  build_items_block((int)blockIdx.x, nP, nL, lm_mask, pf_start, pf_edges, pf_col, items, cap, pair_count);
}

template <int PASSES>
__global__ __launch_bounds__(kSchurThreads) void k_schur(int nP, const int* __restrict__ pair_i1, const int* __restrict__ pair_i2,
                                                        const int* __restrict__ pair_start, const PairItem* __restrict__ items,
                                                        const double* __restrict__ EB, const double* __restrict__ Hll,
                                                        const double* __restrict__ bl, const double* __restrict__ Hpp,
                                                        const double* __restrict__ bp, double lambda_v, double* __restrict__ S,
                                                        double* __restrict__ bs, const double* __restrict__ lambda_p, int item_cap,
                                                        const int* __restrict__ pair_count, double* __restrict__ St) {
  const double lambda = lambda_p ? *lambda_p : lambda_v;
  constexpr int kSeg = 65, kRow = 4 * kSeg + 1, kPass = 42 / PASSES;
  __shared__ double red[kPass * kRow];
  __shared__ double part[42][4];
  LBA_PROF_BEGIN(1);
  int pr;
  {
    const int nb = gridDim.x, q = nb >> 3, r = nb & 7, k = blockIdx.x & 7;
    pr = k * q + min(k, r) + (blockIdx.x >> 3);
  }
  int i1, i2;
  if (pair_i1) { i1 = pair_i1[pr]; i2 = pair_i2[pr]; }
  else {
    int rem = pr; i1 = 0;
    while (rem >= nP - i1) { rem -= nP - i1; i1++; }
    i2 = i1 + rem;
  }
  const int tid = threadIdx.x;
  double acc[36], cacc[6];
#pragma unroll
  for (int i = 0; i < 36; i++) acc[i] = 0;
#pragma unroll
  for (int i = 0; i < 6; i++) cacc[i] = 0;
  const bool diag = i1 == i2;
  const int j0 = pair_start ? pair_start[pr] : pr * item_cap;
  const int j1 = pair_start ? pair_start[pr + 1] : j0 + pair_count[pr];
  for (int j = j0 + tid; j < j1; j += kSchurThreads) {
    const PairItem it = items[j];
    double Dinv[9];
    inv3_sym(Hll + 6 * (size_t)it.l, lambda, Dinv);
    const double* Bi = EB + (size_t)it.ea * kEB;
    const double* Bj = EB + (size_t)it.eb * kEB;
    double BD[18];
#pragma unroll
    for (int a = 0; a < 6; a++)
#pragma unroll
      for (int c = 0; c < 3; c++) BD[3 * a + c] = Bi[3 * a] * Dinv[c] + Bi[3 * a + 1] * Dinv[3 + c] + Bi[3 * a + 2] * Dinv[6 + c];
#pragma unroll
    for (int a = 0; a < 6; a++)
#pragma unroll
      for (int c = 0; c < 6; c++) acc[6 * a + c] += BD[3 * a] * Bj[3 * c] + BD[3 * a + 1] * Bj[3 * c + 1] + BD[3 * a + 2] * Bj[3 * c + 2];
    if (diag) {
      const double* b = bl + 3 * (size_t)it.l;
#pragma unroll
      for (int a = 0; a < 6; a++) cacc[a] += BD[3 * a] * b[0] + BD[3 * a + 1] * b[1] + BD[3 * a + 2] * b[2];
    }
  }
  LBA_PROF_PHASE(0, 0);
  const int slot = (tid >> 6) * kSeg + (tid & 63);
  const int nval = diag ? 42 : 36;
#pragma unroll
  for (int ps = 0; ps < PASSES; ps++) {
    if (ps == 1) __syncthreads();
#pragma unroll
    for (int i = 0; i < kPass; i++) {
      const int v = ps * kPass + i;
      red[i * kRow + slot] = v < 36 ? acc[v < 36 ? v : 0] : cacc[v >= 36 ? v - 36 : 0];
    }
    __syncthreads();
    if (tid < 4 * kPass && ps * kPass + (tid >> 2) < nval) {
      const int o = tid >> 2, q = tid & 3;
      const double* r = red + o * kRow + q * kSeg;
      double s = 0;
#pragma unroll
      for (int k0 = 0; k0 < 64; k0 += 16) {
        double v[16];
#pragma unroll
        for (int u = 0; u < 16; u++) v[u] = r[k0 + u];
#pragma unroll
        for (int u = 0; u < 16; u++) s += v[u];
      }
      part[ps * kPass + o][q] = s;
    }
  }
  __syncthreads();
  LBA_PROF_PHASE(0, 1);
  const int n = 6 * nP;
  if (tid < 36) {
    const double s = ((part[tid][0] + part[tid][1]) + part[tid][2]) + part[tid][3];
    const int a = tid / 6, c = tid % 6;
    double v = -s;
    if (diag) {
      const int lo = a < c ? a : c, hi = a < c ? c : a;
      const int u = lo * 6 - lo * (lo - 1) / 2 + (hi - lo);
      v += Hpp[21 * (size_t)i1 + u] + (a == c ? lambda : 0.0);
    }
    if (St) {
      const int r = 6 * i1 + a, cc = 6 * i2 + c;
      const int p0 = ldltm::tile_image_pos(r, cc), p1 = ldltm::tile_image_pos(cc, r);
      if (p0 >= 0) St[p0] = v;
      if (p1 >= 0 && r != cc) St[p1] = v;
    } else {
      S[(size_t)(6 * i1 + a) * n + 6 * i2 + c] = v;
      if (!diag) S[(size_t)(6 * i2 + c) * n + 6 * i1 + a] = v;
    }
  } else if (diag && tid < 42) {
    const int a = tid - 36;
    const double s = ((part[tid][0] + part[tid][1]) + part[tid][2]) + part[tid][3];
    const double v = bp[6 * (size_t)i1 + a] - s;
    bs[6 * i1 + a] = v;
    if (St) ldltm::image_put_rhs(St, n, 6 * i1 + a, v);
  }
  LBA_PROF_END();
}

__global__ __launch_bounds__(256) void k_wide_panel(int n, int kb, double* S, const double* __restrict__ b, double* yw, double* z,
                                                    int* __restrict__ ok_flag) {
  __shared__ double Lk[16][17];
  __shared__ double Aw[16][17];
  const int tid = threadIdx.x, r = tid >> 4, c = tid & 15;
  const int k0 = 16 * kb;
  {
    const int gr = k0 + r, gc = k0 + c;
    const int lo = gr < gc ? gr : gc, hi = gr < gc ? gc : gr;
    Lk[r][c] = (gr < n && gc < n) ? S[(size_t)lo * n + hi] : (r == c ? 1.0 : 0.0);
  }
  if (blockIdx.x == 0 && kb == 0 && tid == 0) *ok_flag = 1;
  __syncthreads();
  bool bad = false;
  for (int j = 0; j < 16; j++) {
    const double d = Lk[j][j];
    if (d == 0.0 || !(d == d) || fabs(d) == INFINITY) bad = true;
    const bool below = r > j, upd = below && c > j && c <= r;
    double v = 0.0, wc = 0.0;
    if (below) v = Lk[r][j];
    if (upd) wc = Lk[c][j];
    __syncthreads();
    const double l = v / d;
    if (upd) Lk[r][c] -= l * wc;
    if (below && c == j) Lk[r][j] = l;
    __syncthreads();
  }
  if (blockIdx.x == 0) {
    if (bad && tid == 0) *ok_flag = 0;
    const int gr = k0 + r, gc = k0 + c;
    if (gr < n && gc < n && c < r) S[(size_t)gr * n + gc] = Lk[r][c];
    const double* src = kb == 0 ? b : yw;
    Aw[r][c] = (r == 0 && k0 + c < n) ? src[k0 + c] : 0.0;
    __syncthreads();
    for (int m = 0; m < 15; m++) {
      if (r == 0 && c > m) Aw[0][c] -= Aw[0][m] * Lk[c][m];
      __syncthreads();
    }
    if (r == 0 && k0 + c < n) { const double w = Aw[0][c]; yw[k0 + c] = w; z[k0 + c] = w / Lk[c][c]; }
    return;
  }
  const int i0 = 16 * (kb + (int)blockIdx.x);
  Aw[r][c] = i0 + r < n ? S[(size_t)(i0 + r) * n + k0 + c] : 0.0;
  __syncthreads();
  for (int m = 0; m < 15; m++) {
    if (c > m) Aw[r][c] -= Aw[r][m] * Lk[c][m];
    __syncthreads();
  }
  if (i0 + r < n) {
    const double w = Aw[r][c];
    S[(size_t)(i0 + r) * n + k0 + c] = w / Lk[c][c];
    S[(size_t)(k0 + c) * n + i0 + r] = w;
  }
}

__global__ __launch_bounds__(256) void k_wide_update(int n, int kb, double* S, const double* __restrict__ b, double* yw) {
  const int m_blocks = gridDim.x, jj = blockIdx.x, ii = blockIdx.y;
  if (ii < m_blocks && ii < jj) return;
  __shared__ double Wt[16][17];
  __shared__ double Lj[16][17];
  const int tid = threadIdx.x, r = tid >> 4, c = tid & 15;
  const int k0 = 16 * kb, j0 = 16 * (kb + 1 + jj);
  Lj[r][c] = j0 + r < n ? S[(size_t)(j0 + r) * n + k0 + c] : 0.0;
  if (ii == m_blocks) {
    if (r == 0) Wt[0][c] = yw[k0 + c];
    __syncthreads();
    if (r == 0 && j0 + c < n) {
      double acc = 0.0;
      for (int m = 0; m < 16; m++) acc += Wt[0][m] * Lj[c][m];
      yw[j0 + c] = (kb == 0 ? b[j0 + c] : yw[j0 + c]) - acc;
    }
    return;
  }
  const int i0 = 16 * (kb + 1 + ii);
  Wt[c][r] = i0 + c < n ? S[(size_t)(k0 + r) * n + i0 + c] : 0.0;
  __syncthreads();
  if (i0 + r < n && j0 + c < n) {
    double acc = 0.0;
    for (int m = 0; m < 16; m++) acc += Wt[r][m] * Lj[c][m];
// ... 1273 lines not shown
```

multi_orbslam3_amd/csrc/matcher.hip:

```cpp

#include "common.hpp"
#include "wave.hpp"
#include "stereo_finalize.hpp"
#include "rot_hist.hpp"
#include "null_vector4.hpp"

#include <algorithm>
#include <cmath>

using namespace orbg;

int orbx_internal_left_features(orbx_handle* h, const orbx_keypoint** d_kps, const uint8_t** d_desc, const float** d_uright,
                                const float** d_depth, const orbx_keypoint** h_kps, int* n, hipStream_t* stream);

#include "grid_build.hpp"

namespace {

constexpr int TH_HIGH = 100;
constexpr int TH_LOW = 50;
using orbg::HISTO_LENGTH;
using orbg::RotHist;
using orbg::rot_bin;
using orbg::null_vector4;
// ... 186 lines not shown
  const float Pc_dist = norm3d(Pc);
  if (Pc[2] < 0.0f) return f;
  float uv[2];
  rig_project(S.cam, Pc, uv);
  if (uv[0] < fp.min_x || uv[0] > fp.max_x) return f;
  if (uv[1] < fp.min_y || uv[1] > fp.max_y) return f;
  const float maxDistance = 1.2f * max_raw, minDistance = 0.8f * min_raw;
  const float PO[3] = {X[0] - S.twc[0], X[1] - S.twc[1], X[2] - S.twc[2]};
  const float dist = norm3d(PO);
  if (dist < minDistance || dist > maxDistance) return f;
  const double dot = (double)PO[0] * Pn[0] + (double)PO[1] * Pn[1] + (double)PO[2] * Pn[2];
  const float viewCos = (float)(dot / (double)dist);
  if (viewCos < limit) return f;
  const float ratio = max_raw / dist;
  const float lg = (float)log((double)ratio);
  int nScale = (int)ceilf(lg / fp.log_sf);
  if (nScale < 0) nScale = 0;
  else if (nScale >= fp.n_levels) nScale = fp.n_levels - 1;
  f.in_view = 1; f.px = uv[0]; f.py = uv[1]; f.depth = Pc_dist; f.level = nScale; f.view_cos = viewCos;
  return f;
}

__global__ __launch_bounds__(256) void frustum_rig_kernel(FrameParams fp, RigSideF L, RigSideF R, int has_right, WorldPtsDev w, float limit, TrackDev tl, TrackDev tr) {
  const int i = blockIdx.x * 256 + threadIdx.x;
  if (i >= w.m) return;
  const float X[3] = {w.pos[3 * i], w.pos[3 * i + 1], w.pos[3 * i + 2]};
  const float N[3] = {w.normal[3 * i], w.normal[3 * i + 1], w.normal[3 * i + 2]};
  const float mn = w.min_dist[i], mx = w.max_dist[i];
  const TrackFields a = rig_frustum_check(fp, L, X, N, mn, mx, limit);
  tl.in_view[i] = (uint8_t)a.in_view; tl.px[i] = a.px; tl.py[i] = a.py; tl.depth[i] = a.depth; tl.level[i] = a.level; tl.view_cos[i] = a.view_cos;
  if (!has_right) return;
  const TrackFields b = rig_frustum_check(fp, R, X, N, mn, mx, limit);
  tr.in_view[i] = (uint8_t)b.in_view; tr.px[i] = b.px; tr.py[i] = b.py; tr.depth[i] = b.depth; tr.level[i] = b.level; tr.view_cos[i] = b.view_cos;
}


struct Top4 { unsigned k[4]; int i[4]; };

__device__ __forceinline__ void top4_init(Top4& t) {
#pragma unroll
  for (int j = 0; j < 4; j++) { t.k[j] = 0xFFFFFFFFu; t.i[j] = -1; }
}

__device__ __forceinline__ void top4_insert(Top4& t, unsigned key, int idx) {
  if (key >= t.k[3]) return;
#pragma unroll
  for (int j = 3; j >= 0; j--) {
    const bool shift = j > 0 && key < t.k[j - 1];
    if (shift) { t.k[j] = t.k[j - 1]; t.i[j] = t.i[j - 1]; }
    else { t.k[j] = key; t.i[j] = idx; break; }
  }
}

__device__ __forceinline__ void top4_wave_emit(Top4& t, QResult& res) {
  res.n_top = 0;
#pragma unroll
  for (int r = 0; r < 4; r++) {
    res.idx[r] = 0xFFFF; res.dist[r] = 256;
    const unsigned m = wave_min(t.k[0]);
    if (m != 0xFFFFFFFFu) {
      const bool own = t.k[0] == m;
      const int owner = __ffsll((unsigned long long)__ballot(own)) - 1;
      const int idx = __builtin_amdgcn_readlane(t.i[0], owner);
      res.idx[r] = (unsigned short)idx; res.dist[r] = (unsigned short)(m >> 20);
      res.n_top = (unsigned short)(r + 1);
      if (own) {
        t.k[0] = t.k[1]; t.i[0] = t.i[1]; t.k[1] = t.k[2]; t.i[1] = t.i[2]; t.k[2] = t.k[3]; t.i[2] = t.i[3];
        t.k[3] = 0xFFFFFFFFu; t.i[3] = -1;
      }
    }
  }
}

constexpr int kOccBits = 4096;
struct FrameDev {
  const orbx_keypoint* kps; const uint8_t* desc; const float* uright;
  const int* cell_start; const int* cell_items;
  const int* assigned_mp; const int* assigned_obs;
  int use_mask;
  uint32_t occ[kOccBits / 32];
};

__device__ __forceinline__ bool feature_occupied(const FrameDev& F, int idx) {
  if (F.use_mask) return (F.occ[idx >> 5] >> (idx & 31)) & 1u;
  return F.assigned_mp[idx] >= 0 && (!F.assigned_obs || F.assigned_obs[idx] > 0);
}

struct Query { int valid; float x, y, r; int min_level, max_level; float ur_ref; };

constexpr int kSlot = 16;
constexpr int kListStage = 64;

struct QDesc { uint4 a0, a1; };
__device__ __forceinline__ QDesc load_qdesc(const uint8_t* p) {
  QDesc d;
  d.a0 = *reinterpret_cast<const uint4*>(p); d.a1 = *reinterpret_cast<const uint4*>(p + 16);
  return d;
}

__device__ __forceinline__ void window_search(const FrameParams& fp, const FrameDev& F, const Query& q, const QDesc& qd,
                                              int qid, int n_queries, int* __restrict__ list_counter,
                                              uint32_t* __restrict__ list, int list_cap, QResult* __restrict__ out,
                                              uint32_t* __restrict__ s_list ,
                                              unsigned short flags = 0) {
  const int lane = threadIdx.x & 63;
  QResult res;
  res.base = 0; res.count = flags; res.n_top = 0;
#pragma unroll
  for (int j = 0; j < 4; j++) { res.idx[j] = 0xFFFF; res.dist[j] = 256; }
  bool empty = !q.valid;
  int nMinCellX = 0, nMaxCellX = -1, nMinCellY = 0, nMaxCellY = -1;
  if (!empty) {
    nMinCellX = max(0, (int)floorf((q.x - fp.min_x - q.r) * fp.w_inv));
    nMaxCellX = min(ORBG_GRID_COLS - 1, (int)ceilf((q.x - fp.min_x + q.r) * fp.w_inv));
    nMinCellY = max(0, (int)floorf((q.y - fp.min_y - q.r) * fp.h_inv));
    nMaxCellY = min(ORBG_GRID_ROWS - 1, (int)ceilf((q.y - fp.min_y + q.r) * fp.h_inv));
    if (nMinCellX >= ORBG_GRID_COLS || nMaxCellX < 0 || nMinCellY >= ORBG_GRID_ROWS || nMaxCellY < 0) empty = true;
  }
  if (empty) {
    if (lane == 0) *out = res;
    return;
  }
  const int ncy = nMaxCellY - nMinCellY + 1, ncx = nMaxCellX - nMinCellX + 1;
  const int ncell = ncx * ncy;
  int total = 0;
  for (int c = lane; c < ncell; c += 64) {
    const int ix = nMinCellX + c / ncy, iy = nMinCellY + c % ncy;
    const int cell = ix * ORBG_GRID_ROWS + iy;
    total += F.cell_start[cell + 1] - F.cell_start[cell];
  }
  total = wave_sum(total);
  if (total == 0) {
    if (lane == 0) *out = res;
    return;
  }
  int base = qid * kSlot;
  if (total > kSlot) {
    if (lane == 0) base = n_queries * kSlot + atomicAdd(list_counter, total);
    base = __shfl(base, 0, 64);
  }
  const uint4 a0 = qd.a0, a1 = qd.a1;
  const bool bCheckLevels = (q.min_level > 0) || (q.max_level >= 0);
  Top4 t;
  top4_init(t);
  int run = 0;
  for (int c0 = 0; c0 < ncell; c0 += 64) {
    const int c = c0 + lane;
    int s = 0, n = 0;
    if (c < ncell) {
      const int ix = nMinCellX + c / ncy, iy = nMinCellY + c % ncy;
      const int cell = ix * ORBG_GRID_ROWS + iy;
      s = F.cell_start[cell];
      n = F.cell_start[cell + 1] - s;
    }
    const int inc = wave_incl_scan_add(n);
    const int chunk_total = __builtin_amdgcn_readlane(inc, 63);
    const int my_pos0 = run + inc - n;
    const int nmax = wave_max(n);
    int idx_next = n > 0 ? F.cell_items[s] : 0;
    for (int j = 0; j < nmax; j++) {
      const int idx = idx_next;
      if (j + 1 < n) idx_next = F.cell_items[s + j + 1];
      if (j < n) {
        const int pos = my_pos0 + j;
        const orbx_keypoint kp = F.kps[idx];
        const float ur_c = F.uright ? F.uright[idx] : 0.f;
        const uint4 b0 = *reinterpret_cast<const uint4*>(F.desc + (size_t)idx * 32);
// ... 430 lines not shown
  top4_init(tt);
  for (int j = lane; j < nt; j += 64) {
    const uint4 b0 = *reinterpret_cast<const uint4*>(t + (size_t)j * 32);
    const uint4 b1 = *reinterpret_cast<const uint4*>(t + (size_t)j * 32 + 16);
    top4_insert(tt, ((unsigned)popc256(a0, a1, b0, b1) << 20) | (unsigned)j, j);
  }
  int od[2] = {256, 256}, oi[2] = {-1, -1};
#pragma unroll
  for (int r = 0; r < 2; r++) {
    const unsigned m = wave_min(tt.k[0]);
    if (m != 0xFFFFFFFFu) {
      od[r] = (int)(m >> 20); oi[r] = (int)(m & 0xFFFFFu);
      if (tt.k[0] == m) { tt.k[0] = tt.k[1]; tt.k[1] = tt.k[2]; tt.k[2] = tt.k[3]; tt.k[3] = 0xFFFFFFFFu; }
    }
  }
  if (lane == 0) {
    out4[4 * qi] = od[0]; out4[4 * qi + 1] = oi[0];
    out4[4 * qi + 2] = od[1]; out4[4 * qi + 3] = oi[1];
  }
}

constexpr int kWireKp = 15, kWireDesc = 32;

__device__ __forceinline__ void wire_put_f32(uint8_t* p, float v) {
  const unsigned u = __float_as_uint(v);
  p[0] = (uint8_t)u; p[1] = (uint8_t)(u >> 8); p[2] = (uint8_t)(u >> 16); p[3] = (uint8_t)(u >> 24);
}
__device__ __forceinline__ float wire_get_f32(const uint8_t* p) {
  return __uint_as_float((unsigned)p[0] | ((unsigned)p[1] << 8) | ((unsigned)p[2] << 16) | ((unsigned)p[3] << 24));
}

__global__ __launch_bounds__(256) void wire_pack_kernel(const orbx_keypoint* __restrict__ kps, const uint8_t* __restrict__ desc, int n,
                                                       uint8_t* __restrict__ wire) {
  const int i = blockIdx.x * 256 + threadIdx.x;
  if (i >= n) return;
  const orbx_keypoint k = kps[i];
  uint8_t* p = wire + (size_t)i * kWireKp;
  wire_put_f32(p, k.x); wire_put_f32(p + 4, k.y);
  p[8] = (uint8_t)k.size;
  wire_put_f32(p + 9, k.angle);
  p[13] = (uint8_t)k.response;
  p[14] = (uint8_t)(int8_t)k.octave;
  const uint4* s = reinterpret_cast<const uint4*>(desc + (size_t)i * 32);
  uint8_t* d = wire + (size_t)n * kWireKp + (size_t)i * kWireDesc;
  const uint4 a = s[0], b = s[1];
  const unsigned w[8] = {a.x, a.y, a.z, a.w, b.x, b.y, b.z, b.w};
#pragma unroll
  for (int q = 0; q < 8; q++) { d[4 * q] = (uint8_t)w[q]; d[4 * q + 1] = (uint8_t)(w[q] >> 8); d[4 * q + 2] = (uint8_t)(w[q] >> 16); d[4 * q + 3] = (uint8_t)(w[q] >> 24); }
}

__global__ __launch_bounds__(256) void wire_unpack_kernel(const uint8_t* __restrict__ wire, int n, orbx_keypoint* __restrict__ kps,
                                                         uint8_t* __restrict__ desc, orbx_keypoint* __restrict__ kps_host) {
  const int i = blockIdx.x * 256 + threadIdx.x;
  if (i >= n) return;
  const uint8_t* p = wire + (size_t)i * kWireKp;
  orbx_keypoint k;
  k.x = wire_get_f32(p); k.y = wire_get_f32(p + 4);
  k.size = (float)p[8];
  k.angle = wire_get_f32(p + 9);
  k.response = (float)p[13];
  k.octave = (int)(int8_t)p[14];
  kps[i] = k;
  if (kps_host) kps_host[i] = k;
  const uint8_t* d = wire + (size_t)n * kWireKp + (size_t)i * kWireDesc;
  for (int q = 0; q < 32; q++) desc[(size_t)i * 32 + q] = d[q];
}


void make_pose(const float* T, PoseF* P) {
  for (int i = 0; i < 3; i++) {
    for (int j = 0; j < 3; j++) P->R[3 * i + j] = T[4 * i + j];
    P->t[i] = T[4 * i + 3];
  }
  for (int i = 0; i < 3; i++) {
    double s = 0;
    for (int k = 0; k < 3; k++) s += (double)P->R[3 * k + i] * (double)P->t[k];
    P->Ow[i] = (float)(-s);
  }
}

}


struct orbm_frame {
  hipStream_t own_stream = nullptr;
  bool ext_stream = false;
  std::vector<uint8_t> claimed_buf;
  std::vector<uint32_t> rot_entries;
  std::vector<float> hk_angle;
  std::vector<int8_t> hk_oct;
  const orbx_keypoint* hk_cached_from = nullptr;
  int hk_cached_n = -1;
  int device = 0;
  hipStream_t stream = nullptr;
  hipEvent_t ev[2] = {};
  int cap = 0;
  FrameParams fp;
  bool has_uright = false;
  DevBuf<orbx_keypoint> d_kps;
  DevBuf<uint8_t> d_desc;
  DevBuf<float> d_uright, d_depth;
  DevBuf<int> d_cell_of, d_cell_start, d_cell_items;
  const orbx_keypoint* kps_p = nullptr;
  const uint8_t* desc_p = nullptr;
  const float* uright_p = nullptr;
  const float* depth_p = nullptr;
  std::vector<orbx_keypoint> h_kps_own;
  PinnedBuf<orbx_keypoint> h_kps_pin;
  DevBuf<uint8_t> d_qflag;
  DevBuf<int> d_blk_cnt, d_slot_pt, d_total;
  PinnedBuf<int> h_slot_pt;
  PinnedBuf<uint8_t> h_vis;
  const orbx_keypoint* hk = nullptr;
  PinnedBuf<uint8_t> stage;
  DevBuf<uint8_t> d_stage;
  size_t stage_off = 0;
  const int* d_assigned_mp = nullptr;
  const int* d_assigned_obs = nullptr;
  bool occ_mask = false;
  uint32_t occ[kOccBits / 32];
  size_t copy_lo = 0, copy_hi = 0;
  unsigned search_seq = 0;
  StreamSignal sig;
  DevBuf<int> d_counter;
  PinnedBuf<uint32_t> list;
  PinnedBuf<QResult> results;
  float last_ms = 0;
};

static int frame_set_params(orbm_frame* f, const orbm_frame_view* v, int n) {
  if (v->n_levels < 1 || v->n_levels > ORBG_MAX_LEVELS) return ORBG_BAD_ARG;
  if (n >= ORBG_MAX_FRAME_FEATURES) return ORBG_CAP_EXCEEDED;
  FrameParams& p = f->fp;
  p.n = n;
  p.min_x = v->min_x; p.max_x = v->max_x; p.min_y = v->min_y; p.max_y = v->max_y;
  p.w_inv = static_cast<float>(ORBG_GRID_COLS) / static_cast<float>(v->max_x - v->min_x);
  p.h_inv = static_cast<float>(ORBG_GRID_ROWS) / static_cast<float>(v->max_y - v->min_y);
  p.fx = v->fx; p.fy = v->fy; p.cx = v->cx; p.cy = v->cy; p.bf = v->bf; p.b = v->b;
  p.n_levels = v->n_levels;
  p.log_sf = std::log(v->scale_factor);
  p.scale[0] = 1.0f;
  for (int i = 1; i < v->n_levels; i++) p.scale[i] = p.scale[i - 1] * v->scale_factor;
  for (int i = v->n_levels; i < ORBG_MAX_LEVELS; i++) p.scale[i] = 0;
  return ORBG_OK;
}

static int frame_reserve(orbm_frame* f, int n) {
  int rc;
  const size_t c = (size_t)std::max(n, 1);
  if ((rc = f->d_kps.reserve(c)) || (rc = f->d_desc.reserve(c * 32)) || (rc = f->d_uright.reserve(c)) ||
      (rc = f->d_depth.reserve(c)) || (rc = f->d_cell_of.reserve(c)) || (rc = f->d_cell_start.reserve(kCells + 1)) ||
      (rc = f->d_cell_items.reserve(c)))
    return rc;
  if (!f->d_counter.p) {
    if ((rc = f->d_counter.reserve(4))) return rc;
    ORBG_HIP(hipMemsetAsync(f->d_counter.p, 0, f->d_counter.cap * sizeof(int), f->stream));
    ORBG_HIP(hipStreamSynchronize(f->stream));
  }
  return ORBG_OK;
}

static int frame_build_grid(orbm_frame* f) {
  hipLaunchKernelGGL(grid_build_kernel, dim3(1), dim3(1024), 0, f->stream, f->kps_p, f->fp, f->d_cell_of.p,
                     f->d_cell_start.p, f->d_cell_items.p, (const int*)nullptr, (volatile unsigned*)nullptr, 0u);
  ORBG_HIP(hipGetLastError());
  return ORBG_OK;
}

extern "C" int orbm_frame_create(int device, int cap_features, orbm_frame** out) {
  if (!out || cap_features < 0) return ORBG_BAD_ARG;
  int rc = select_device(device);
  if (rc) return rc;
  orbm_frame* f = new orbm_frame();
  f->device = device;
  f->cap = cap_features;
  memset(&f->fp, 0, sizeof(f->fp));
  if (orbg::create_stream(&f->own_stream, "fr") != hipSuccess) { delete f; return ORBG_HIP_ERROR; }
  f->stream = f->own_stream;
  for (auto& e : f->ev) if (hipEventCreate(&e) != hipSuccess) { delete f; return ORBG_HIP_ERROR; }
  if ((rc = frame_reserve(f, cap_features))) { delete f; return rc; }
  *out = f;
  return ORBG_OK;
}

extern "C" int orbm_frame_destroy(orbm_frame* f) {
  if (!f) return ORBG_BAD_ARG;
  (void)hipSetDevice(f->device);
  (void)hipStreamSynchronize(f->stream);
  if (f->own_stream != f->stream) (void)hipStreamSynchronize(f->own_stream);
  f->d_kps.release(); f->d_desc.release(); f->d_uright.release(); f->d_depth.release(); f->d_cell_of.release();
  f->d_cell_start.release(); f->d_cell_items.release(); f->stage.release(); f->d_stage.release();
  f->d_counter.release(); f->list.release(); f->results.release(); f->sig.release(); f->h_kps_pin.release(); f->d_qflag.release(); f->d_blk_cnt.release(); f->d_slot_pt.release(); f->d_total.release(); f->h_slot_pt.release(); f->h_vis.release();
  for (auto& e : f->ev) if (e) (void)hipEventDestroy(e);
  if (!f->ext_stream) orbg::release_stream(f->own_stream);
  delete f;
  return ORBG_OK;
}

extern "C" int orbm_frame_set_stream(orbm_frame* f, void* hip_stream) {
  if (!f) return ORBG_BAD_ARG;
  int rc = select_device(f->device);
  if (rc) return rc;
  const bool on_own = f->stream == f->own_stream;
  if (!on_own) ORBG_HIP(hipStreamSynchronize(f->stream));
  if ((rc = orbg::swap_stream(&f->own_stream, &f->ext_stream, hip_stream, "fr"))) return rc;
  if (on_own) f->stream = f->own_stream;
  return ORBG_OK;
}

extern "C" int orbm_frame_upload(orbm_frame* f, const orbm_frame_view* v) {
  if (!f || !v || v->n < 0 || (v->n > 0 && (!v->kps || !v->desc))) return ORBG_BAD_ARG;
  int rc = select_device(f->device);
  if (rc) return rc;
  if ((rc = frame_set_params(f, v, v->n))) return rc;
  if ((rc = frame_reserve(f, v->n))) return rc;
  const int n = v->n;
  f->h_kps_own.assign(v->kps, v->kps + n);
  f->hk = f->h_kps_own.data(); f->hk_cached_n = -1;
  f->stream = f->own_stream;
  f->kps_p = f->d_kps.p; f->desc_p = f->d_desc.p; f->uright_p = f->d_uright.p; f->depth_p = f->d_depth.p;
  f->has_uright = v->uright != nullptr;
  if (n > 0) {
    ORBG_HIP(hipMemcpyAsync(f->d_kps.p, v->kps, (size_t)n * sizeof(orbx_keypoint), hipMemcpyHostToDevice, f->stream));
    ORBG_HIP(hipMemcpyAsync(f->d_desc.p, v->desc, (size_t)n * 32, hipMemcpyHostToDevice, f->stream));
    if (v->uright) ORBG_HIP(hipMemcpyAsync(f->d_uright.p, v->uright, (size_t)n * 4, hipMemcpyHostToDevice, f->stream));
    if (v->depth) ORBG_HIP(hipMemcpyAsync(f->d_depth.p, v->depth, (size_t)n * 4, hipMemcpyHostToDevice, f->stream));
  }
  if ((rc = frame_build_grid(f))) return rc;
  ORBG_HIP(hipStreamSynchronize(f->stream));
  return ORBG_OK;
}

extern "C" int orbm_frame_from_extractor(orbm_frame* f, orbx_handle* h, const orbm_frame_view* v) {
  if (!f || !h || !v) return ORBG_BAD_ARG;
  int rc = select_device(f->device);
  if (rc) return rc;
  const orbx_keypoint* dk; const uint8_t* dd; const float* du; const float* dz; const orbx_keypoint* hk; int n; hipStream_t xs;
  if ((rc = orbx_internal_left_features(h, &dk, &dd, &du, &dz, &hk, &n, &xs))) return rc;
  if (v->n >= 0 && v->n != n) return ORBG_BAD_ARG;
  if ((rc = frame_set_params(f, v, n))) return rc;
  if ((rc = frame_reserve(f, n))) return rc;
  f->has_uright = true;
  f->kps_p = dk; f->desc_p = dd; f->uright_p = du; f->depth_p = dz; f->hk = hk; f->hk_cached_n = -1;
  f->stream = xs;
  return frame_build_grid(f);
}

int orbx_internal_kp_capacity(orbx_handle* h);
int orbm_internal_attach(orbm_frame* f, orbx_handle* h, const orbm_frame_view* v, int n, hipStream_t stream, const int* d_n,
                         volatile unsigned* done_flag, unsigned done_seq, const StereoFinalizeArgs* fin, const orbg::UndistortArgs* un,
                         bool mono) {
  if (!f || !h || !v) return ORBG_BAD_ARG;
  const orbx_keypoint* dk; const uint8_t* dd; const float* du; const float* dz; const orbx_keypoint* hk; int n0; hipStream_t xs;
  int rc = orbx_internal_left_features(h, &dk, &dd, &du, &dz, &hk, &n0, &xs);
  if (rc) return rc;
  if ((rc = frame_set_params(f, v, n < 0 ? 0 : n))) return rc;
  const int xcap = orbx_internal_kp_capacity(h);
  if (n < 0 && xcap >= ORBG_MAX_FRAME_FEATURES) return ORBG_CAP_EXCEEDED;
  if ((rc = frame_reserve(f, n < 0 ? std::max(std::max(f->cap, 4096), xcap) : n))) return rc;
  f->has_uright = !mono;
  f->kps_p = (un && un->on) ? un->dst : dk;
  f->desc_p = dd; f->uright_p = du; f->depth_p = dz; f->hk = hk; f->hk_cached_n = -1;
  f->stream = stream;
  if (un && un->on)
    hipLaunchKernelGGL(undistort_grid_kernel, dim3(1), dim3(1024), 0, stream, *un, f->fp, f->d_cell_of.p, f->d_cell_start.p, f->d_cell_items.p,
                       d_n, done_flag, done_seq);
  else if (fin)
    hipLaunchKernelGGL(grid_build_finalize_kernel, dim3(2), dim3(1024), 0, stream, f->kps_p, f->fp, f->d_cell_of.p, f->d_cell_start.p,
                       f->d_cell_items.p, d_n, done_flag, done_seq, *fin);
  else
    hipLaunchKernelGGL(grid_build_kernel, dim3(1), dim3(1024), 0, stream, f->kps_p, f->fp, f->d_cell_of.p, f->d_cell_start.p,
                       f->d_cell_items.p, d_n, done_flag, done_seq);
  ORBG_HIP(hipGetLastError());
  return ORBG_OK;
}

void orbm_internal_set_n(orbm_frame* f, int n) {
  f->fp.n = n; f->hk_cached_n = -1;
  f->stream = f->own_stream;
}

int orbm_internal_kf_features(orbm_frame* f, const orbx_keypoint** d_kps, const uint8_t** d_desc, const float** d_uright,
                              const float** d_depth, const orbx_keypoint** h_kps, int* n, int* device, hipStream_t* stream) {
  if (!f || (f->fp.n > 0 && (!f->kps_p || !f->desc_p))) return ORBG_BAD_ARG;
  *d_kps = f->kps_p; *d_desc = f->desc_p; *d_uright = f->has_uright ? f->uright_p : nullptr; *d_depth = f->depth_p;
  *h_kps = f->hk; *n = f->fp.n; *device = f->device; *stream = f->stream;
  return ORBG_OK;
}

int orbm_internal_kf_grid(orbm_frame* f, const int** d_cell_start, const int** d_cell_items, FrameParams* fp) {
  if (!f || !f->d_cell_start.p || !f->d_cell_items.p) return ORBG_BAD_ARG;
  *d_cell_start = f->d_cell_start.p; *d_cell_items = f->d_cell_items.p; *fp = f->fp;
  return ORBG_OK;
}

int orbm_internal_order_after(orbm_frame* f, hipStream_t st) {
  if (f->stream == st) return ORBG_OK;
  ORBG_HIP(hipEventRecord(f->ev[1], f->stream));
  ORBG_HIP(hipStreamWaitEvent(st, f->ev[1], 0));
  return ORBG_OK;
}

int orbm_internal_features(orbm_frame* f, const uint8_t** d_desc, int* n, hipStream_t* stream) {
  if (!f || !f->desc_p) return ORBG_BAD_ARG;
  *d_desc = f->desc_p; *n = f->fp.n; *stream = f->stream;
  return ORBG_OK;
}

extern "C" int orbm_frame_get_grid(orbm_frame* f, int32_t* cell_start, int32_t* cell_items) {
  if (!f || !cell_start) return ORBG_BAD_ARG;
  int rc = select_device(f->device);
  if (rc) return rc;
  ORBG_HIP(hipStreamSynchronize(f->stream));
  ORBG_HIP(hipMemcpy(cell_start, f->d_cell_start.p, (kCells + 1) * sizeof(int), hipMemcpyDeviceToHost));
  const int total = cell_start[kCells];
  if (cell_items && total > 0) ORBG_HIP(hipMemcpy(cell_items, f->d_cell_items.p, (size_t)total * sizeof(int), hipMemcpyDeviceToHost));
  return ORBG_OK;
}

extern "C" int orbk_wire_bytes(int n) { return n < 0 ? ORBG_BAD_ARG : n * (kWireKp + kWireDesc); }

extern "C" int orbk_pack_frame(orbm_frame* f, uint8_t* wire, int wire_on_device) {
  if (!f || !f->kps_p || (f->fp.n > 0 && !wire)) return ORBG_BAD_ARG;
  int rc = select_device(f->device);
  if (rc) return rc;
  const int n = f->fp.n;
  if (n == 0) return ORBG_OK;
  const size_t bytes = (size_t)n * (kWireKp + kWireDesc);
  uint8_t* d_wire = wire;
  if (!wire_on_device) {
    if ((rc = f->d_stage.reserve(bytes))) return rc;
    d_wire = f->d_stage.p;
  }
  hipLaunchKernelGGL(wire_pack_kernel, dim3((n + 255) / 256), dim3(256), 0, f->stream, f->kps_p, f->desc_p, n, d_wire);
  ORBG_HIP(hipGetLastError());
  if (!wire_on_device) ORBG_HIP(hipMemcpyAsync(wire, d_wire, bytes, hipMemcpyDeviceToHost, f->stream));
  ORBG_HIP(hipStreamSynchronize(f->stream));
  return ORBG_OK;
}

extern "C" int orbk_frame_from_wire(orbm_frame* f, const orbm_frame_view* v, const uint8_t* wire, int n, int wire_on_device) {
  if (!f || !v || n < 0 || (n > 0 && !wire)) return ORBG_BAD_ARG;
  int rc = select_device(f->device);
  if (rc) return rc;
  if ((rc = frame_set_params(f, v, n))) return rc;
  if ((rc = frame_reserve(f, n))) return rc;
  f->kps_p = f->d_kps.p; f->desc_p = f->d_desc.p; f->uright_p = f->d_uright.p; f->depth_p = f->d_depth.p;
  f->has_uright = false;
  if ((rc = f->h_kps_pin.reserve((size_t)std::max(n, 1)))) return rc;
  f->hk = f->h_kps_pin.h; f->hk_cached_n = -1; f->hk_cached_from = nullptr;
  f->stream = f->own_stream;
  if (n > 0) {
    const size_t bytes = (size_t)n * (kWireKp + kWireDesc);
    const uint8_t* d_wire = wire;
    if (!wire_on_device) {
      if ((rc = f->d_stage.reserve(bytes))) return rc;
      ORBG_HIP(hipMemcpyAsync(f->d_stage.p, wire, bytes, hipMemcpyHostToDevice, f->stream));
      d_wire = f->d_stage.p;
    }
    hipLaunchKernelGGL(wire_unpack_kernel, dim3((n + 255) / 256), dim3(256), 0, f->stream, d_wire, n, f->d_kps.p, f->d_desc.p,
                       f->h_kps_pin.d);
    ORBG_HIP(hipGetLastError());
// ... 378 lines not shown
  F.cell_start = f->d_cell_start.p; F.cell_items = f->d_cell_items.p;
  F.assigned_mp = f->d_assigned_mp; F.assigned_obs = f->d_assigned_obs;
  F.use_mask = f->occ_mask;
  if (f->occ_mask) memcpy(F.occ, f->occ, sizeof(F.occ));
  return F;
}

static void cache_keypoint_fields(orbm_frame* f) {
  const int n = f->fp.n;
  if (f->hk_cached_from == f->hk && f->hk_cached_n == n) return;
  f->hk_angle.resize((size_t)std::max(n, 1));
  f->hk_oct.resize((size_t)std::max(n, 1));
  for (int i = 0; i < n; i++) { f->hk_angle[i] = f->hk[i].angle; f->hk_oct[i] = (int8_t)f->hk[i].octave; }
  f->hk_cached_from = f->hk; f->hk_cached_n = n;
}

static int stage_begin(orbm_frame* f, size_t total_bytes) {
  int rc;
  const size_t need = total_bytes + 64 * 16;
  if ((rc = f->stage.reserve(need)) || (rc = f->d_stage.reserve(need))) return rc;
  f->stage_off = 0;
  f->copy_lo = f->copy_hi = 0;
  return ORBG_OK;
}
template <typename T>
static const T* stage_add(orbm_frame* f, const T* src, size_t count, bool dev_copy = false) {
  f->stage_off = (f->stage_off + 15) & ~(size_t)15;
  if (count) memcpy(f->stage.h + f->stage_off, src, count * sizeof(T));
  const T* dev = reinterpret_cast<const T*>((dev_copy ? f->d_stage.p : f->stage.d) + f->stage_off);
  if (dev_copy && count) {
    if (f->copy_hi == f->copy_lo) f->copy_lo = f->stage_off;
    f->copy_hi = f->stage_off + count * sizeof(T);
  }
  f->stage_off += count * sizeof(T);
  return dev;
}
static int stage_commit(orbm_frame* f) {
  if (f->copy_hi > f->copy_lo)
    ORBG_HIP(hipMemcpyAsync(f->d_stage.p + f->copy_lo, f->stage.h + f->copy_lo, f->copy_hi - f->copy_lo, hipMemcpyHostToDevice, f->stream));
  return ORBG_OK;
}
static int frustum_zero_copy(orbm_frame* f, const float* Tcw, const orbm_worldpoints_view* pts, float limit, uint8_t* track_in_view,
                             float* proj_x, float* proj_y, float* proj_xr, float* track_depth, int32_t* scale_level, float* view_cos) {
  const size_t n = (size_t)pts->m;
  int rc;
  if ((rc = stage_begin(f, n * (32 + 25) + 16 * 16))) return rc;
  WorldPtsDev w;
  w.m = pts->m;
  w.pos = stage_add(f, pts->pos, 3 * n); w.normal = stage_add(f, pts->normal, 3 * n);
  w.min_dist = stage_add(f, pts->min_dist, n); w.max_dist = stage_add(f, pts->max_dist, n);
  w.desc = nullptr; w.bad = nullptr; w.skip = nullptr;
  auto out_region = [&](size_t bytes) { f->stage_off = (f->stage_off + 15) & ~(size_t)15; const size_t o = f->stage_off; f->stage_off += bytes; return o; };
  const size_t o_iv = out_region(n), o_px = out_region(4 * n), o_py = out_region(4 * n), o_pxr = out_region(4 * n), o_dep = out_region(4 * n),
               o_lvl = out_region(4 * n), o_vc = out_region(4 * n);
  uint8_t* D = f->stage.d;
  TrackDev t;
  t.in_view = D + o_iv; t.px = reinterpret_cast<float*>(D + o_px); t.py = reinterpret_cast<float*>(D + o_py);
  t.pxr = reinterpret_cast<float*>(D + o_pxr); t.depth = reinterpret_cast<float*>(D + o_dep); t.level = reinterpret_cast<int*>(D + o_lvl);
  t.view_cos = reinterpret_cast<float*>(D + o_vc);
  PoseF P;
  make_pose(Tcw, &P);
  hipLaunchKernelGGL(frustum_kernel, dim3((pts->m + 255) / 256), dim3(256), 0, f->stream, f->fp, P, w, limit, t);
  ORBG_HIP(hipGetLastError());
  if ((rc = f->sig.sync(f->stream))) return rc;
  const uint8_t* Hh = f->stage.h;
  memcpy(track_in_view, Hh + o_iv, n); memcpy(proj_x, Hh + o_px, 4 * n); memcpy(proj_y, Hh + o_py, 4 * n); memcpy(proj_xr, Hh + o_pxr, 4 * n);
  memcpy(track_depth, Hh + o_dep, 4 * n); memcpy(scale_level, Hh + o_lvl, 4 * n); memcpy(view_cos, Hh + o_vc, 4 * n);
  return ORBG_OK;
}

static void stage_occupancy(orbm_frame* f, const int32_t* amp, const int32_t* aob, int n) {
  f->occ_mask = n <= kOccBits;
  if (f->occ_mask) {
    memset(f->occ, 0, sizeof(f->occ));
    for (int i = 0; i < n; i++)
      if (amp[i] >= 0 && (!aob || aob[i] > 0)) f->occ[i >> 5] |= 1u << (i & 31);
    f->d_assigned_mp = nullptr; f->d_assigned_obs = nullptr;
  } else {
    f->d_assigned_mp = stage_add(f, amp, n, true);
    f->d_assigned_obs = aob ? stage_add(f, aob, n, true) : nullptr;
  }
}

template <typename LaunchFn>
static int run_search(orbm_frame* f, int n_queries, LaunchFn launch, const volatile int* n_scan_host = nullptr) {
  int rc;
  if ((rc = f->results.reserve((size_t)std::max(n_queries, 1)))) return rc;
  const size_t slots = (size_t)n_queries * kSlot;
  if (f->list.cap < slots + (1 << 16) && (rc = f->list.reserve(slots + (1 << 18)))) return rc;
  for (int attempt = 0; attempt < 3; attempt++) {
    int* cur = f->d_counter.p + (f->search_seq & 1);
    int* nxt = f->d_counter.p + ((f->search_seq + 1) & 1);
    f->search_seq++;
    launch((int)std::min<size_t>(f->list.cap, (size_t)1 << 30), cur, nxt);
    ORBG_HIP(hipGetLastError());
    if ((rc = f->sig.sync(f->stream))) return rc;
    size_t total = 0;
    const QResult* R = f->results.h;
    const int n_scan = n_scan_host ? std::min((int)*n_scan_host, n_queries) : n_queries;
    for (int i = 0; i < n_scan; i++) total = std::max(total, (size_t)R[i].base + (size_t)(R[i].count & kQCountMask));
    if (total <= f->list.cap) return ORBG_OK;
    if ((rc = f->list.reserve(total + total / 4))) return rc;
  }
  return ORBG_CAP_EXCEEDED;
}

template <typename LaunchA, typename LaunchB>
static int run_search_pair(orbm_frame* a, orbm_frame* b, int n_queries, LaunchA launch_a, LaunchB launch_b) {
  int rc;
  orbm_frame* fs[2] = {a, b};
  for (orbm_frame* f : fs) {
    if ((rc = f->results.reserve((size_t)std::max(n_queries, 1)))) return rc;
    const size_t slots = (size_t)n_queries * kSlot;
    if (f->list.cap < slots + (1 << 16) && (rc = f->list.reserve(slots + (1 << 18)))) return rc;
  }
  for (int k = 0; k < 2; k++) {
    orbm_frame* f = fs[k];
    int* cur = f->d_counter.p + (f->search_seq & 1);
    int* nxt = f->d_counter.p + ((f->search_seq + 1) & 1);
    f->search_seq++;
    const int cap = (int)std::min<size_t>(f->list.cap, (size_t)1 << 30);
    if (k == 0) launch_a(cap, cur, nxt); else launch_b(cap, cur, nxt);
    ORBG_HIP(hipGetLastError());
    if ((rc = f->sig.post(f->stream))) return rc;
  }
  for (orbm_frame* f : fs)
    if ((rc = f->sig.wait(f->stream))) return rc;
  for (int k = 0; k < 2; k++) {
    orbm_frame* f = fs[k];
    size_t total = 0;
    const QResult* R = f->results.h;
    for (int i = 0; i < n_queries; i++) total = std::max(total, (size_t)R[i].base + (size_t)(R[i].count & kQCountMask));
    if (total <= f->list.cap) continue;
    if ((rc = f->list.reserve(total + total / 4))) return rc;
    if ((rc = k == 0 ? run_search(f, n_queries, launch_a) : run_search(f, n_queries, launch_b))) return rc;
  }
  return ORBG_OK;
}

struct Pick { int idx1 = -1, dist1 = 256, idx2 = -1, dist2 = 256; };
template <typename ClaimedFn>
static int pick_unclaimed(orbm_frame* f, const QResult& r, int want, ClaimedFn claimed, Pick* out) {
  Pick p;
  int found = 0;
  for (int k = 0; k < r.n_top && found < want; k++) {
    const int idx = r.idx[k];
    if (claimed(idx)) continue;
    if (found == 0) { p.idx1 = idx; p.dist1 = r.dist[k]; } else { p.idx2 = idx; p.dist2 = r.dist[k]; }
    found++;
  }
  if (found < want && r.n_top == 4) {
    p = Pick();
    const uint32_t* list = f->list.h + r.base;
    for (int k = 0; k < (r.count & kQCountMask); k++) {
      const uint32_t e = list[k];
      if (e == 0xFFFFFFFFu) continue;
      const int idx = (int)(e & 0xFFFF), dist = (int)(e >> 16);
      if (claimed(idx)) continue;
      if (dist < p.dist1) { p.dist2 = p.dist1; p.idx2 = p.idx1; p.dist1 = dist; p.idx1 = idx; }
      else if (dist < p.dist2) { p.dist2 = dist; p.idx2 = idx; }
    }
  }
  *out = p;
  return ORBG_OK;
}

static int commit_mps(orbm_frame* f, int m, const int32_t* n_obs, float nnratio, int32_t* amp, int32_t* aob, int* nmatches_out,
                      const int* slot_pt = nullptr) {
  const int n = f->fp.n;
  cache_keypoint_fields(f);
  f->claimed_buf.assign((size_t)std::max(n, 1), 0);
  uint8_t* claimed = f->claimed_buf.data();
  int nmatches = 0;
  const QResult* R = f->results.h;
  auto is_claimed = [&](int idx) { return claimed[idx] != 0; };
  for (int s = 0; s < m; s++) {
    __builtin_prefetch(&R[s + 16]);
    const QResult& r = R[s];
    if (r.n_top == 0) continue;
    const int i = slot_pt ? slot_pt[s] : s;
    Pick pk;
    int rc = pick_unclaimed(f, r, 2, is_claimed, &pk);
    if (rc) return rc;
    if (pk.idx1 < 0) continue;
    const int bestDist = pk.dist1, bestIdx = pk.idx1, bestDist2 = pk.dist2, idx2 = pk.idx2;
    const int bestLevel = f->hk_oct[bestIdx];
    const int bestLevel2 = idx2 >= 0 ? f->hk_oct[idx2] : -1;
    if (bestDist <= TH_HIGH) {
      if (bestLevel == bestLevel2 && bestDist > nnratio * bestDist2) continue;
      if (bestLevel != bestLevel2 || bestDist <= nnratio * bestDist2) {
        amp[bestIdx] = i;
        aob[bestIdx] = n_obs[i];
        if (n_obs[i] > 0) claimed[bestIdx] = 1;
        nmatches++;
      }
    }
  }
// ... 251 lines not shown
    }
  }
  return ORBG_INTERNAL;
}

extern "C" int orbm_search_by_projection_frame_rig(orbm_frame* FL, orbm_frame* FR, const float* Tcw_cur, const orbg_camera_rig* rig,
                                                   const orbm_lastframe_view* last, float th, int mono, int check_orientation,
                                                   int32_t* amp, int32_t* aob, int* nmatches_out) {
  if (!FL || !Tcw_cur || !rig || !last || !amp || !aob || last->n < 0) return ORBG_BAD_ARG;
  const bool two = rig->has_right != 0;
  if (two ? (!FR || FL == FR || FL->device != FR->device) : FR != nullptr) return ORBG_BAD_ARG;
  if (rig->left.model != ORBG_CAM_PINHOLE && rig->left.model != ORBG_CAM_KANNALA_BRANDT8) return ORBG_BAD_ARG;
  int rc = select_device(FL->device);
  if (rc) return rc;
  const int m = last->n, nl = FL->fp.n;
  if (nmatches_out) *nmatches_out = 0;
  if (m == 0) return ORBG_OK;
  PoseF Pc, Pl;
  make_pose(Tcw_cur, &Pc);
  make_pose(last->Tcw, &Pl);
  float tlc[3];
  for (int i = 0; i < 3; i++) {
    const float t0 = Pl.R[3 * i] * Pc.Ow[0] + Pl.R[3 * i + 1] * Pc.Ow[1] + Pl.R[3 * i + 2] * Pc.Ow[2];
    tlc[i] = t0 + Pl.t[i];
  }
  const int forward = tlc[2] > FL->fp.b && !mono;
  const int backward = -tlc[2] > FL->fp.b && !mono;
  const RigCamF cam = rig_cam_of(rig->left);
  TrlF Trl;
  memcpy(Trl.m, rig->Trl, sizeof(Trl.m));
  LastDev Ls[2]; FrameDev Fs[2];
  for (int side = 0; side < (two ? 2 : 1); side++) {
    orbm_frame* f = side ? FR : FL;
    const int n = f->fp.n;
    if ((rc = stage_begin(f, (size_t)n * 8 + (size_t)m * (2 + 32 + 12 + 4)))) return rc;
    const std::vector<int32_t> none((size_t)std::max(n, 1), -1);
    stage_occupancy(f, none.data(), nullptr, n);
    LastDev& L = Ls[side];
    L.n = m;
    L.mp_valid = stage_add(f, last->mp_valid, m); L.outlier = stage_add(f, last->outlier, m);
    L.desc = stage_add(f, last->desc, (size_t)m * 32);
    L.world_pos = stage_add(f, last->world_pos, (size_t)m * 3);
    L.octave = stage_add(f, last->octave, m);
    if ((rc = stage_commit(f))) return rc;
    Fs[side] = frame_dev(f);
    Fs[side].uright = nullptr;
  }
  auto launch = [&](int side) {
    return [&, side](int list_cap, int* cnt, int* cnt_next) {
      orbm_frame* f = side ? FR : FL;
      hipLaunchKernelGGL(search_frame_rig_kernel, dim3((m + 3) / 4), dim3(256), 0, f->stream, f->fp, Fs[side], Ls[side], Pc, cam, Trl, side, th, forward,
                         backward, cnt, cnt_next, f->list.d, list_cap, f->results.d);
    };
  };
  if ((rc = two ? run_search_pair(FL, FR, m, launch(0), launch(1)) : run_search(FL, m, launch(0)))) return rc;
  cache_keypoint_fields(FL);
  if (two) cache_keypoint_fields(FR);
  RotHist rotHist(FL->rot_entries);
  int nmatches = 0;
  const QResult* RL = FL->results.h;
  const QResult* RR = two ? FR->results.h : nullptr;
  for (int i = 0; i < m; i++) {
    if (RL[i].n_top == 0) continue;
    Pick pk;
    if ((rc = pick_unclaimed(FL, RL[i], 1, [&](int idx) { return amp[idx] >= 0 && aob[idx] > 0; }, &pk))) return rc;
    if (pk.idx1 >= 0 && pk.dist1 <= TH_HIGH) {
      amp[pk.idx1] = i; aob[pk.idx1] = last->n_obs[i];
      nmatches++;
      if (check_orientation) rotHist.add(rot_bin(last->angle[i], FL->hk_angle[pk.idx1]), pk.idx1);
    }
    if (!two || RR[i].n_top == 0) continue;
    if ((rc = pick_unclaimed(FR, RR[i], 1, [&](int idx) { return amp[idx + nl] >= 0 && aob[idx + nl] > 0; }, &pk))) return rc;
    if (pk.idx1 >= 0 && pk.dist1 <= TH_HIGH) {
      amp[pk.idx1 + nl] = i; aob[pk.idx1 + nl] = last->n_obs[i];
      nmatches++;
      if (check_orientation) rotHist.add(rot_bin(last->angle[i], FR->hk_angle[pk.idx1]), pk.idx1 + nl);
    }
  }
  if (check_orientation) rotHist.reject_outside_three_maxima([&](int idx) { amp[idx] = -1; aob[idx] = 0; nmatches--; });
  if (nmatches_out) *nmatches_out = nmatches;
  return ORBG_OK;
}

static int search_frame_common(orbm_frame* f, const float* Tcw_cur, const float* Tcw_last, int m, LastDev L, const int32_t* n_obs_last,
                               const float* angle_last, hipEvent_t wait_ev, float th, int mono, int check_orientation,
                               int32_t* assigned_mp, int32_t* assigned_obs, int* nmatches_out) {
  int rc;
  const int n = f->fp.n;
  hipStream_t st = f->stream;
  PoseF Pc, Pl;
  make_pose(Tcw_cur, &Pc);
  make_pose(Tcw_last, &Pl);
  float tlc[3];
  for (int i = 0; i < 3; i++) {
    const float t0 = Pl.R[3 * i] * Pc.Ow[0] + Pl.R[3 * i + 1] * Pc.Ow[1] + Pl.R[3 * i + 2] * Pc.Ow[2];
    tlc[i] = t0 + Pl.t[i];
  }
  const int forward = tlc[2] > f->fp.b && !mono;
  const int backward = -tlc[2] > f->fp.b && !mono;
  if (wait_ev) ORBG_HIP(hipStreamWaitEvent(st, wait_ev, 0));
  rc = run_search(f, m, [&](int list_cap, int* cnt, int* cnt_next) {
    hipLaunchKernelGGL(search_frame_kernel, dim3((m + 3) / 4), dim3(256), 0, st, f->fp, frame_dev(f), L, Pc, th, forward, backward,
                       cnt, cnt_next, f->list.d, list_cap, f->results.d);
  });
  if (rc) return rc;
  cache_keypoint_fields(f);
  f->claimed_buf.assign((size_t)std::max(n, 1), 0);
  uint8_t* claimed = f->claimed_buf.data();
  RotHist rotHist(f->rot_entries);
  int nmatches = 0;
  const QResult* R = f->results.h;
  auto is_claimed = [&](int idx) { return claimed[idx] != 0; };
  for (int i = 0; i < m; i++) {
    __builtin_prefetch(&R[i + 16]);
    const QResult& r = R[i];
    if (r.n_top == 0) continue;
    Pick pk;
    if ((rc = pick_unclaimed(f, r, 1, is_claimed, &pk))) return rc;
    if (pk.idx1 < 0) continue;
    const int bestDist = pk.dist1, bestIdx = pk.idx1;
    if (bestDist <= TH_HIGH) {
      assigned_mp[bestIdx] = i;
      assigned_obs[bestIdx] = n_obs_last[i];
      if (n_obs_last[i] > 0) claimed[bestIdx] = 1;
      nmatches++;
      if (check_orientation) rotHist.add(rot_bin(angle_last[i], f->hk_angle[bestIdx]), bestIdx);
    }
  }
  if (check_orientation)
    rotHist.reject_outside_three_maxima([&](int idx) { assigned_mp[idx] = -1; assigned_obs[idx] = 0; nmatches--; });
  if (nmatches_out) *nmatches_out = nmatches;
  return ORBG_OK;
}

extern "C" int orbm_search_by_projection_frame(orbm_frame* f, const float* Tcw_cur, const orbm_lastframe_view* last, float th,
                                               int mono, int check_orientation, int32_t* assigned_mp, int32_t* assigned_obs,
                                               int* nmatches_out) {
  if (!f || !Tcw_cur || !last || !assigned_mp || !assigned_obs || last->n < 0) return ORBG_BAD_ARG;
  int rc = select_device(f->device);
  if (rc) return rc;
  const int m = last->n;
  if (nmatches_out) *nmatches_out = 0;
  if (m == 0) return ORBG_OK;
  const int n = f->fp.n;
  if ((rc = stage_begin(f, (size_t)n * 8 + (size_t)m * (2 + 32 + 12 + 4)))) return rc;
  stage_occupancy(f, assigned_mp, assigned_obs, n);
  LastDev L;
  L.n = m;
  L.mp_valid = stage_add(f, last->mp_valid, m); L.outlier = stage_add(f, last->outlier, m);
  L.desc = stage_add(f, last->desc, (size_t)m * 32);
  L.world_pos = stage_add(f, last->world_pos, (size_t)m * 3);
  L.octave = stage_add(f, last->octave, m);
  if ((rc = stage_commit(f))) return rc;
  return search_frame_common(f, Tcw_cur, last->Tcw, m, L, last->n_obs, last->angle, nullptr, th, mono, check_orientation, assigned_mp,
                             assigned_obs, nmatches_out);
}

struct orbm_lastview {
  int device = 0;
  hipStream_t stream = nullptr;
  bool ext_stream = false;
  DevBuf<uint8_t> arena;
  PinnedBuf<uint8_t> stage;
  hipEvent_t ev = nullptr;
  bool pending = false;
  int n = 0;
  size_t o_valid = 0, o_outl = 0, o_desc = 0, o_pos = 0, o_oct = 0, bytes = 0;
  std::vector<int32_t> n_obs;
  std::vector<float> angle;
  float Tcw[16] = {0};
};

extern "C" int orbm_lastview_create(int device, int cap_features, orbm_lastview** out) {
  if (!out || cap_features < 0) return ORBG_BAD_ARG;
  int rc = select_device(device);
  if (rc) return rc;
  orbm_lastview* v = new orbm_lastview();
  v->device = device;
  if (orbg::create_stream(&v->stream, "map") != hipSuccess) { delete v; return ORBG_HIP_ERROR; }
  if (hipEventCreateWithFlags(&v->ev, hipEventDisableTiming) != hipSuccess) { orbg::release_stream(v->stream); delete v; return ORBG_HIP_ERROR; }
  const size_t need = (size_t)std::max(cap_features, 16) * 64 + 256;
  if ((rc = v->arena.reserve(need)) || (rc = v->stage.reserve(need))) { v->arena.release(); v->stage.release(); (void)hipEventDestroy(v->ev); orbg::release_stream(v->stream); delete v; return rc; }
  *out = v;
  return ORBG_OK;
}

extern "C" int orbm_lastview_destroy(orbm_lastview* v) {
  if (!v) return ORBG_BAD_ARG;
  (void)hipSetDevice(v->device);
  (void)hipStreamSynchronize(v->stream);
  v->arena.release(); v->stage.release();
  if (v->ev) (void)hipEventDestroy(v->ev);
  if (!v->ext_stream) orbg::release_stream(v->stream);
  delete v;
  return ORBG_OK;
}

extern "C" int orbm_lastview_upload(orbm_lastview* v, const orbm_lastframe_view* last) {
  if (!v || !last || last->n < 0) return ORBG_BAD_ARG;
  const size_t m = (size_t)last->n;
  if (m > 0 && (!last->mp_valid || !last->outlier || !last->world_pos || !last->desc || !last->octave || !last->angle || !last->n_obs)) return ORBG_BAD_ARG;
  int rc = select_device(v->device);
  if (rc) return rc;
  if (v->pending) { ORBG_HIP(hipEventSynchronize(v->ev)); v->pending = false; }
  auto al = [](size_t x) { return (x + 15) & ~(size_t)15; };
  v->o_valid = 0; v->o_outl = al(m); v->o_desc = v->o_outl + al(m); v->o_pos = v->o_desc + al(32 * m); v->o_oct = v->o_pos + al(12 * m);
  v->bytes = v->o_oct + al(4 * m);
  if ((rc = v->arena.reserve(v->bytes + 64)) || (rc = v->stage.reserve(v->bytes + 64))) return rc;
  v->n = last->n;
  v->n_obs.assign(last->n_obs, last->n_obs + m);
  v->angle.assign(last->angle, last->angle + m);
  memcpy(v->Tcw, last->Tcw, sizeof(v->Tcw));
  if (m > 0) {
    uint8_t* S = v->stage.h;
    memcpy(S + v->o_valid, last->mp_valid, m); memcpy(S + v->o_outl, last->outlier, m); memcpy(S + v->o_desc, last->desc, 32 * m);
    memcpy(S + v->o_pos, last->world_pos, 12 * m); memcpy(S + v->o_oct, last->octave, 4 * m);
    const int n16 = (int)((v->bytes + 15) / 16);
    hipLaunchKernelGGL(lastview_copy_kernel, dim3((n16 + 255) / 256), dim3(256), 0, v->stream, reinterpret_cast<const uint4*>(v->stage.d),
                       reinterpret_cast<uint4*>(v->arena.p), n16);
    ORBG_HIP(hipGetLastError());
    ORBG_HIP(hipEventRecord(v->ev, v->stream));
    v->pending = true;
  }
  return ORBG_OK;
}

extern "C" int orbm_search_by_projection_frame_resident(orbm_frame* f, const float* Tcw_cur, orbm_lastview* v, float th, int mono,
                                                        int check_orientation, int32_t* assigned_mp, int32_t* assigned_obs, int* nmatches_out) {
  if (!f || !Tcw_cur || !v || !assigned_mp || !assigned_obs || f->device != v->device) return ORBG_BAD_ARG;
  int rc = select_device(f->device);
  if (rc) return rc;
  const int m = v->n;
  if (nmatches_out) *nmatches_out = 0;
  if (m == 0) return ORBG_OK;
  const int n = f->fp.n;
  if ((rc = stage_begin(f, (size_t)n * 8))) return rc;
  stage_occupancy(f, assigned_mp, assigned_obs, n);
  if ((rc = stage_commit(f))) return rc;
  const uint8_t* A = v->arena.p;
  LastDev L;
  L.n = m;
  L.mp_valid = A + v->o_valid; L.outlier = A + v->o_outl; L.desc = A + v->o_desc;
  L.world_pos = reinterpret_cast<const float*>(A + v->o_pos); L.octave = reinterpret_cast<const int*>(A + v->o_oct);
  hipEvent_t wait_ev = nullptr;
  if (v->pending) {
    if (hipEventQuery(v->ev) == hipSuccess) v->pending = false;
    else { (void)hipGetLastError(); wait_ev = v->ev; }
  }
  return search_frame_common(f, Tcw_cur, v->Tcw, m, L, v->n_obs.data(), v->angle.data(), wait_ev, th, mono, check_orientation, assigned_mp,
                             assigned_obs, nmatches_out);
}

static int bow_common(orbm_frame* f, const orbm_featvec_view* fvF, const uint8_t* t_valid, const uint8_t* kf_desc, int nkf,
                      const uint8_t* kf_mp_valid, const float* kf_angle, const orbm_featvec_view* fvK, float nnratio,
                      int check_orientation, bool by_query, int32_t* matches, int* nmatches_out, int n_left = -1) {
  int rc = select_device(f->device);
  if (rc) return rc;
  const int n = f->fp.n;
  const int n_out = by_query ? nkf : n;
  for (int i = 0; i < n_out; i++) matches[i] = -1;
  if (nmatches_out) *nmatches_out = 0;
  std::vector<BowJob> jobs;
  {
    int k = 0, ff = 0;
    while (k < fvK->n_nodes && ff < fvF->n_nodes) {
      if (fvK->node_id[k] == fvF->node_id[ff]) {
        for (uint32_t a = fvK->start[k]; a < fvK->start[k + 1]; a++) {
          const uint32_t kfi = fvK->feat_idx[a];
          if ((int)kfi >= nkf) return ORBG_BAD_ARG;
          if (!kf_mp_valid[kfi]) continue;
          jobs.push_back(BowJob{(int)kfi, (int)fvF->start[ff], (int)fvF->start[ff + 1]});
        }
        k++; ff++;
      } else if (fvK->node_id[k] < fvF->node_id[ff]) {
        k = (int)(std::lower_bound(fvK->node_id, fvK->node_id + fvK->n_nodes, fvF->node_id[ff]) - fvK->node_id);
      } else {
        ff = (int)(std::lower_bound(fvF->node_id, fvF->node_id + fvF->n_nodes, fvK->node_id[k]) - fvF->node_id);
      }
    }
  }
  const int nq = (int)jobs.size();
  if (nq == 0) return ORBG_OK;
  if (n_left >= 0) jobs.insert(jobs.end(), jobs.begin(), jobs.begin() + nq);
  const int nj = (int)jobs.size();
  const int nfi = (int)fvF->start[fvF->n_nodes];
  for (int i = 0; i < nfi; i++)
    if ((int)fvF->feat_idx[i] >= n) return ORBG_BAD_ARG;
  if ((rc = stage_begin(f, (size_t)nj * sizeof(BowJob) + (size_t)nfi * 4 + (size_t)nkf * 32 + (size_t)n))) return rc;
  hipStream_t st = f->stream;
  const uint32_t* d_fidx = stage_add(f, fvF->feat_idx, nfi, true);
  const uint8_t* d_tvalid = t_valid ? stage_add(f, t_valid, n, true) : nullptr;
  const BowJob* d_jobs = stage_add(f, jobs.data(), nj);
  const uint8_t* d_kfdesc = stage_add(f, kf_desc, (size_t)nkf * 32);
  if ((rc = stage_commit(f))) return rc;
  rc = run_search(f, nj, [&](int list_cap, int* cnt, int* cnt_next) {
    hipLaunchKernelGGL(search_bow_kernel, dim3((nj + 3) / 4), dim3(256), 0, st, f->desc_p, d_fidx, d_tvalid, d_kfdesc,
                       d_jobs, nj, cnt, cnt_next, f->list.d, list_cap, f->results.d, n_left);
  });
  if (rc) return rc;
  cache_keypoint_fields(f);
  RotHist rotHist(f->rot_entries);
  f->claimed_buf.assign((size_t)std::max(n, 1), 0);
  uint8_t* taken = f->claimed_buf.data();
  int nmatches = 0;
  const QResult* R = f->results.h;
  auto is_taken = [&](int idx) { return taken[idx] != 0; };
  if (n_left >= 0) {
    for (int j = 0; j < nq; j++) {
      Pick pl, pr;
      if (R[j].n_top == 0) continue;
      if ((rc = pick_unclaimed(f, R[j], 2, is_taken, &pl))) return rc;
      if (pl.idx1 < 0 || pl.dist1 > TH_LOW) continue;
      if (R[nq + j].n_top && (rc = pick_unclaimed(f, R[nq + j], 1, is_taken, &pr))) return rc;
      const int q = jobs[j].kf_idx;
      if (static_cast<float>(pl.dist1) < nnratio * static_cast<float>(pl.dist2)) {
        taken[pl.idx1] = 1; matches[pl.idx1] = q;
        if (check_orientation) rotHist.add(rot_bin(kf_angle[q], f->hk_angle[pl.idx1]), pl.idx1);
        nmatches++;
      }
      if (pr.idx1 >= 0 && pr.dist1 <= TH_LOW) {
        taken[pr.idx1] = 1; matches[pr.idx1] = q;
        if (check_orientation) rotHist.add(rot_bin(kf_angle[q], f->hk_angle[pr.idx1]), pr.idx1);
        nmatches++;
      }
    }
    if (check_orientation) rotHist.reject_outside_three_maxima([&](int idx) { matches[idx] = -1; nmatches--; });
    if (nmatches_out) *nmatches_out = nmatches;
    return ORBG_OK;
  }
  for (int j = 0; j < nj; j++) {
    __builtin_prefetch(&R[j + 16]);
    const QResult& r = R[j];
    if (r.n_top == 0) continue;
// ... 186 lines not shown
```

Baseline: 9141.

## Launch frame projection search early on the extractor stream, split submit/collect

Adds submit/collect entry points for the resident last-frame projection search. The agent loop now enqueues the search kernel right after extraction work is enqueued and before waiting on the extractor, then collects results later. This removes the host round trip between extraction and search. The extractor marks the early search stale if it re-runs, which forces a relaunch. Separately, the Schur kernel gets a specialized diagonal path that accumulates only the 21 upper-triangular entries, cutting registers and reduction passes. The changes add state-machine complexity around pending early searches and stale results.

After: 9114. About the same (-0.3%).

```diff
diff --git a/include/orbgpu.h b/include/orbgpu.h
--- a/include/orbgpu.h
+++ b/include/orbgpu.h
@@ -110,6 +110,7 @@
 int orbx_frame_stereo_dev_submit(orbx_handle* h, orbm_frame* frame, const orbm_frame_view* view, const uint8_t* d_img_left,
                                  const uint8_t* d_img_right, int width, int height, int stride, float bf, float b);
 int orbx_frame_stereo_dev_wait(orbx_handle* h, int* n_left, int* n_right);
+int orbx_frame_wait_enqueued(orbx_handle* h);
 #define ORBX_SUBMIT_ASYNC 1
 int orbx_set_frame_outputs(orbx_handle* h, orbx_keypoint* kps_left, uint8_t* desc_left, float* uright, float* depth, int cap_left);
 int orbx_frame_stereo_submit(orbx_handle* h, orbm_frame* frame, const orbm_frame_view* view, const uint8_t* img_left,
@@ -201,6 +202,9 @@
 int orbm_lastview_upload(orbm_lastview* v, const orbm_lastframe_view* last);
 int orbm_search_by_projection_frame_resident(orbm_frame* cur, const float* Tcw_cur, orbm_lastview* last, float th, int mono,
                                              int check_orientation, int32_t* assigned_mp, int32_t* assigned_obs, int* nmatches);
+int orbm_search_by_projection_frame_resident_submit(orbm_frame* cur, const float* Tcw_cur, orbm_lastview* last, float th, int mono);
+int orbm_search_by_projection_frame_resident_collect(orbm_frame* cur, int check_orientation, int32_t* assigned_mp, int32_t* assigned_obs,
+                                                     int* nmatches);
 
 typedef struct orbm_featvec_view {
   int32_t n_nodes;
diff --git a/multi_orbslam3_amd/_capi.py b/multi_orbslam3_amd/_capi.py
--- a/multi_orbslam3_amd/_capi.py
+++ b/multi_orbslam3_amd/_capi.py
@@ -242,7 +242,8 @@
     "orbd_database_create", "orbd_database_destroy", "orbd_detect_n_best_candidates",
     "orbx_set_stream", "orbm_frame_set_stream", "orbm_map_set_stream", "lba_set_stream", "orbv_vocab_set_stream", "orbd_database_set_stream",
     "pose_opt_set_stream", "orbx_get_ctor_timeline", "orbm_map_set_observations", "orbm_search_by_projection_reloc", "orbm_search_by_projection_reloc_cam", "orbm_search_by_projection_sim3_cam", "orbm_lastview_create", "orbm_lastview_destroy", "orbm_lastview_upload",
-    "orbm_search_by_projection_frame_resident", "orbg_quiesce", "orbg_set_wait_policy", "orbg_get_wait_policy",
+    "orbm_search_by_projection_frame_resident", "orbm_search_by_projection_frame_resident_submit",
+    "orbm_search_by_projection_frame_resident_collect", "orbx_frame_wait_enqueued", "orbg_quiesce", "orbg_set_wait_policy", "orbg_get_wait_policy",
     "orbx_frame_mono", "orbx_frame_mono_dev", "orbx_frame_mono_submit", "orbx_frame_mono_dev_submit", "orbx_frame_mono_wait",
     "orbx_set_frame_outputs_un", "orbx_undistort_points",
     "orbm_sim3_create", "orbm_sim3_destroy", "orbm_sim3_set_stream", "orbm_sim3_set_problem", "orbm_sim3_set_ransac_parameters",
diff --git a/multi_orbslam3_amd/api.py b/multi_orbslam3_amd/api.py
--- a/multi_orbslam3_amd/api.py
+++ b/multi_orbslam3_amd/api.py
@@ -171,6 +171,9 @@
 
     def frame_mono_wait(self):
         return self.frame_stereo_dev_wait()[0]
+
+    def frame_wait_enqueued(self):
+        capi.check(self.lib.orbx_frame_wait_enqueued(self.h), "orbx_frame_wait_enqueued")
 
     def frame_stereo_dev_wait(self):
         nl, nr = C.c_int(0), C.c_int(0)
@@ -514,6 +517,21 @@
                    "orbm_search_by_projection_frame_resident")
         return amp, aob, n.value
 
+    def SearchByProjectionFrameResidentSubmit(self, CurrentFrame, Tcw_cur, last_on_device, th, bMono):
+        T = np.ascontiguousarray(Tcw_cur, np.float32).reshape(16)
+        capi.check(self.lib.orbm_search_by_projection_frame_resident_submit(CurrentFrame.h, _vp(T), last_on_device.h, C.c_float(th),
+                                                                            int(bool(bMono))),
+                   "orbm_search_by_projection_frame_resident_submit")
+
+    def SearchByProjectionFrameResidentCollect(self, CurrentFrame, n_features):
+        amp = np.full(max(int(n_features), 1), -1, np.int32)
+        aob = np.zeros(max(int(n_features), 1), np.int32)
+        n = C.c_int(0)
+        capi.check(self.lib.orbm_search_by_projection_frame_resident_collect(CurrentFrame.h, int(self.mbCheckOrientation), _vp(amp), _vp(aob),
+                                                                             C.byref(n)),
+                   "orbm_search_by_projection_frame_resident_collect")
+        return amp[: int(n_features)], aob[: int(n_features)], n.value
+
     def SearchByBoW(self, F, fvF, kf_desc, kf_mp_valid, kf_angle, fvK):
         kf_desc = np.ascontiguousarray(kf_desc, np.uint8)
         kf_mp_valid = np.ascontiguousarray(kf_mp_valid, np.uint8)
diff --git a/multi_orbslam3_amd/csrc/agent_loop.cpp b/multi_orbslam3_amd/csrc/agent_loop.cpp
--- a/multi_orbslam3_amd/csrc/agent_loop.cpp
+++ b/multi_orbslam3_amd/csrc/agent_loop.cpp
@@ -1,6 +1,7 @@
 #include <time.h>
 
 #include <cstdint>
+#include <cstdlib>
 #include <cstring>
 #include <vector>
 
@@ -81,6 +82,8 @@
 int agent_run(agent_cfg* c, int64_t first_step, int n_steps, int last_is_final, int timed, double* step_s, agent_stats* st) {
   if (!c || !st || n_steps < 0) return ORBG_BAD_ARG;
   int rc = ORBG_OK, s_done = 0;
+  const char* env_early = getenv("ORBG_EARLY_SEARCH");
+  const bool early = c->pipelined && c->last_view_dev && !(env_early && env_early[0] == '0');
   for (int s = 0; s < n_steps && rc == ORBG_OK; s++) {
     s_done = s;
     const int64_t i = first_step + s;
@@ -88,6 +91,7 @@
     const agent_frame_in& fin = c->frames[k];
     const double t0 = now_s();
     int nl = 0, nr = 0, cur = 0;
+    double t_early = 0;
     if (c->pipelined) {
       const int ring = c->ring < 2 ? 2 : c->ring > 4 ? 4 : c->ring, ahead = c->ahead < 1 ? 1 : c->ahead > ring - 1 ? ring - 1 : c->ahead;
       cur = (int)(i % ring);
@@ -102,7 +106,18 @@
         return ORBG_OK;
       };
       if ((rc = submit_ahead(0, 0))) break;
-      if (!c->submit_first || (rc = submit_ahead(1, ahead)) == ORBG_OK) rc = orbx_frame_stereo_dev_wait(c->ex[cur], &nl, &nr);
+      if (c->submit_first && (rc = submit_ahead(1, ahead))) break;
+      if (early) {
+        const double a = now_s();
+        if (c->last_view_frame != k_last) {
+          if ((rc = orbm_lastview_upload(c->last_view_dev, c->frames[k_last].last_view))) break;
+          c->last_view_frame = k_last;
+        }
+        if ((rc = orbx_frame_wait_enqueued(c->ex[cur]))) break;
+        if ((rc = orbm_search_by_projection_frame_resident_submit(c->fr[cur], fin.Tcw_guess, c->last_view_dev, c->th_frame, c->mono))) break;
+        t_early = now_s() - a;
+      }
+      rc = orbx_frame_stereo_dev_wait(c->ex[cur], &nl, &nr);
       if (rc) break;
       c->in_flight[cur] = 0;
       if (!c->submit_first && (rc = submit_ahead(1, ahead))) break;
@@ -125,7 +140,9 @@
     for (int j = 0; j < nl; j++) c->amp[j] = -1;
     memset(c->aob, 0, sizeof(int32_t) * (size_t)nl);
     int n1 = 0, n2 = 0;
-    if (c->last_view_dev) {
+    if (early) {
+      if ((rc = orbm_search_by_projection_frame_resident_collect(F, 1, c->amp, c->aob, &n1))) break;
+    } else if (c->last_view_dev) {
       if (c->last_view_frame != k_last) {
         if ((rc = orbm_lastview_upload(c->last_view_dev, c->frames[k_last].last_view))) break;
         c->last_view_frame = k_last;
@@ -173,7 +190,7 @@
     }
     st->last_nl = nl; st->last_nr = nr; st->last_n1 = n1; st->last_n2 = n2;
     if (timed) {
-      st->stage_s[0] += t1 - t0; st->stage_s[1] += t2 - t1; st->stage_s[2] += t3 - t2b; st->stage_s[3] += t_po;
+      st->stage_s[0] += t1 - t0 - t_early; st->stage_s[1] += t2 - t1 + t_early; st->stage_s[2] += t3 - t2b; st->stage_s[3] += t_po;
       st->stage_s[4] += t5 - t4; st->stage_s[5] += t6 - t5; st->stage_s[6] += t_lv;
       st->kp += nl + nr; st->m_frame += n1; st->m_map += n2;
       const double t_step = now_s() - t0;
@@ -181,7 +198,7 @@
       if (t_step > st->worst_step_s) {
         st->worst_step_s = t_step;
         st->worst_step_index = i;
-        const double w[8] = {t1 - t0, t2 - t1, t3 - t2b, t_po, t5 - t4, t6 - t5, t_lv, 0.0};
+        const double w[8] = {t1 - t0 - t_early, t2 - t1 + t_early, t3 - t2b, t_po, t5 - t4, t6 - t5, t_lv, 0.0};
         for (int q = 0; q < 8; q++) st->worst_stage_s[q] = w[q];
       }
     }
diff --git a/multi_orbslam3_amd/csrc/extractor.hip b/multi_orbslam3_amd/csrc/extractor.hip
--- a/multi_orbslam3_amd/csrc/extractor.hip
+++ b/multi_orbslam3_amd/csrc/extractor.hip
@@ -1951,6 +1951,7 @@
   return ORBG_OK;
 }
 void orbm_internal_set_n(orbm_frame* f, int n);
+void orbm_internal_early_search_void(orbm_frame* f);
 int orbx_internal_kp_capacity(orbx_handle* h);
 static int launch_stereo(orbx_handle* h, float bf, float b, hipStream_t st, bool device_counts, float* host_mirror,
                          StereoFinalizeArgs* defer_finalize = nullptr);
@@ -2555,18 +2556,28 @@
   return ORBG_OK;
 }
 
+static int wait_ingest_enqueued(orbx_handle* h) {
+  for (unsigned spins = 0; h->ingest_state.load(std::memory_order_acquire) != 2; spins++) {
+#if defined(__x86_64__)
+    __builtin_ia32_pause();
+#endif
+    if (!IngestWorker::spin_ok() || (spins & 0xFFFF) == 0xFFFF) std::this_thread::yield();
+  }
+  return h->ingest_rc;
+}
+
+extern "C" int orbx_frame_wait_enqueued(orbx_handle* h) {
+  if (!h) return ORBG_BAD_ARG;
+  if (h->ingest_state.load(std::memory_order_acquire) != 0) return wait_ingest_enqueued(h);
+  return h->pending && (h->pending->active || h->pending->finished) ? ORBG_OK : ORBG_BAD_ARG;
+}
+
 extern "C" int orbx_frame_stereo_dev_wait(orbx_handle* h, int* n_left, int* n_right) {
   if (!h) return ORBG_BAD_ARG;
   int rc;
   const double t_wait0 = host_now_us();
   if (h->ingest_state.load(std::memory_order_acquire) != 0) {
-    for (unsigned spins = 0; h->ingest_state.load(std::memory_order_acquire) != 2; spins++) {
-#if defined(__x86_64__)
-      __builtin_ia32_pause();
-#endif
-      if (!IngestWorker::spin_ok() || (spins & 0xFFFF) == 0xFFFF) std::this_thread::yield();
-    }
-    rc = h->ingest_rc;
+    rc = wait_ingest_enqueued(h);
     h->ingest_state.store(0, std::memory_order_release);
     if (rc) return rc;
   }
@@ -2806,6 +2817,7 @@
   const PostOps* post = c.has_post ? &c.post : nullptr;
   if (h->h_nkp.h[2]) {
     ORBG_HIP(hipMemsetAsync(h->d_overflow.p, 0, sizeof(int), st));
+    if (post && post->frame) orbm_internal_early_search_void(post->frame);
     return extract_core(h, c.cams_mask, c.d_img0, c.d_img1, c.w, c.hgt, c.stride, c.lap, c.kps_out, c.desc_out, c.cap, c.n_out, c.n_mono_out,
                         post, true, false);
   }
diff --git a/multi_orbslam3_amd/csrc/lba.hip b/multi_orbslam3_amd/csrc/lba.hip
--- a/multi_orbslam3_amd/csrc/lba.hip
+++ b/multi_orbslam3_amd/csrc/lba.hip
@@ -988,6 +988,18 @@
   build_items_block((int)blockIdx.x, nP, nL, lm_mask, pf_start, pf_edges, pf_col, items, cap, pair_count);
 }
 
+__device__ __forceinline__ double sum_segment(const double* r) {
+  double s = 0;
+#pragma unroll
+  for (int k0 = 0; k0 < 64; k0 += 16) {
+    double v[16];
+#pragma unroll
+    for (int u = 0; u < 16; u++) v[u] = r[k0 + u];
+#pragma unroll
+    for (int u = 0; u < 16; u++) s += v[u];
+  }
+  return s;
+}
 template <int PASSES>
 __global__ __launch_bounds__(kSchurThreads) void k_schur(int nP, const int* __restrict__ pair_i1, const int* __restrict__ pair_i2,
                                                         const int* __restrict__ pair_start, const PairItem* __restrict__ items,
@@ -1014,89 +1026,126 @@
     i2 = i1 + rem;
   }
   const int tid = threadIdx.x;
-  double acc[36], cacc[6];
-#pragma unroll
-  for (int i = 0; i < 36; i++) acc[i] = 0;
-#pragma unroll
-  for (int i = 0; i < 6; i++) cacc[i] = 0;
   const bool diag = i1 == i2;
   const int j0 = pair_start ? pair_start[pr] : pr * item_cap;
   const int j1 = pair_start ? pair_start[pr + 1] : j0 + pair_count[pr];
-  for (int j = j0 + tid; j < j1; j += kSchurThreads) {
-    const PairItem it = items[j];
-    double Dinv[9];
-    inv3_sym(Hll + 6 * (size_t)it.l, lambda, Dinv);
-    const double* Bi = EB + (size_t)it.ea * kEB;
-    const double* Bj = EB + (size_t)it.eb * kEB;
-    double BD[18];
-#pragma unroll
-    for (int a = 0; a < 6; a++)
-#pragma unroll
-      for (int c = 0; c < 3; c++) BD[3 * a + c] = Bi[3 * a] * Dinv[c] + Bi[3 * a + 1] * Dinv[3 + c] + Bi[3 * a + 2] * Dinv[6 + c];
-#pragma unroll
-    for (int a = 0; a < 6; a++)
-#pragma unroll
-      for (int c = 0; c < 6; c++) acc[6 * a + c] += BD[3 * a] * Bj[3 * c] + BD[3 * a + 1] * Bj[3 * c + 1] + BD[3 * a + 2] * Bj[3 * c + 2];
-    if (diag) {
+  const int slot = (tid >> 6) * kSeg + (tid & 63);
+  const int n = 6 * nP;
+  if (diag) {
+    double acc[21], cacc[6];
+#pragma unroll
+    for (int i = 0; i < 21; i++) acc[i] = 0;
+#pragma unroll
+    for (int i = 0; i < 6; i++) cacc[i] = 0;
+    for (int j = j0 + tid; j < j1; j += kSchurThreads) {
+      const PairItem it = items[j];
+      double Dinv[9];
+      inv3_sym(Hll + 6 * (size_t)it.l, lambda, Dinv);
+      const double* Bp = EB + (size_t)it.ea * kEB;
+      double B[18];
+#pragma unroll
+      for (int i = 0; i < 18; i++) B[i] = Bp[i];
+      double BD[18];
+#pragma unroll
+      for (int a = 0; a < 6; a++)
+#pragma unroll
+        for (int c = 0; c < 3; c++) BD[3 * a + c] = B[3 * a] * Dinv[c] + B[3 * a + 1] * Dinv[3 + c] + B[3 * a + 2] * Dinv[6 + c];
+#pragma unroll
+      for (int a = 0; a < 6; a++)
+#pragma unroll
+        for (int c = a; c < 6; c++)
+          acc[a * 6 - a * (a - 1) / 2 + (c - a)] += BD[3 * a] * B[3 * c] + BD[3 * a + 1] * B[3 * c + 1] + BD[3 * a + 2] * B[3 * c + 2];
       const double* b = bl + 3 * (size_t)it.l;
 #pragma unroll
       for (int a = 0; a < 6; a++) cacc[a] += BD[3 * a] * b[0] + BD[3 * a + 1] * b[1] + BD[3 * a + 2] * b[2];
     }
-  }
-  LBA_PROF_PHASE(0, 0);
-  const int slot = (tid >> 6) * kSeg + (tid & 63);
-  const int nval = diag ? 42 : 36;
-#pragma unroll
-  for (int ps = 0; ps < PASSES; ps++) {
-    if (ps == 1) __syncthreads();
-#pragma unroll
-    for (int i = 0; i < kPass; i++) {
-      const int v = ps * kPass + i;
-      red[i * kRow + slot] = v < 36 ? acc[v < 36 ? v : 0] : cacc[v >= 36 ? v - 36 : 0];
+    LBA_PROF_PHASE(0, 0);
+#pragma unroll
+    for (int ps = 0; ps < PASSES; ps++) {
+      if (ps == 1) __syncthreads();
+#pragma unroll
+      for (int i = 0; i < kPass; i++) {
+        const int v = ps * kPass + i;
+        if (v < 27) red[i * kRow + slot] = v < 21 ? acc[v < 21 ? v : 0] : cacc[v >= 21 ? v - 21 : 0];
+      }
+      __syncthreads();
+      if (tid < 4 * kPass && ps * kPass + (tid >> 2) < 27) {
+        const int o = tid >> 2, q = tid & 3;
+        part[ps * kPass + o][q] = sum_segment(red + o * kRow + q * kSeg);
+      }
     }
     __syncthreads();
-    if (tid < 4 * kPass && ps * kPass + (tid >> 2) < nval) {
-      const int o = tid >> 2, q = tid & 3;
-      const double* r = red + o * kRow + q * kSeg;
-      double s = 0;
-#pragma unroll
-      for (int k0 = 0; k0 < 64; k0 += 16) {
-        double v[16];
-#pragma unroll
-        for (int u = 0; u < 16; u++) v[u] = r[k0 + u];
-#pragma unroll
-        for (int u = 0; u < 16; u++) s += v[u];
-      }
-      part[ps * kPass + o][q] = s;
-    }
-  }
-  __syncthreads();
-  LBA_PROF_PHASE(0, 1);
-  const int n = 6 * nP;
-  if (tid < 36) {
-    const double s = ((part[tid][0] + part[tid][1]) + part[tid][2]) + part[tid][3];
-    const int a = tid / 6, c = tid % 6;
-    double v = -s;
-    if (diag) {
+    LBA_PROF_PHASE(0, 1);
+    if (tid < 36) {
+      const int a = tid / 6, c = tid % 6;
       const int lo = a < c ? a : c, hi = a < c ? c : a;
       const int u = lo * 6 - lo * (lo - 1) / 2 + (hi - lo);
+      const double s = ((part[u][0] + part[u][1]) + part[u][2]) + part[u][3];
+      double v = -s;
       v += Hpp[21 * (size_t)i1 + u] + (a == c ? lambda : 0.0);
-    }
-    if (St) {
-      const int r = 6 * i1 + a, cc = 6 * i2 + c;
-      const int p0 = ldltm::tile_image_pos(r, cc), p1 = ldltm::tile_image_pos(cc, r);
-      if (p0 >= 0) St[p0] = v;
-      if (p1 >= 0 && r != cc) St[p1] = v;
-    } else {
-      S[(size_t)(6 * i1 + a) * n + 6 * i2 + c] = v;
-      if (!diag) S[(size_t)(6 * i2 + c) * n + 6 * i1 + a] = v;
-    }
-  } else if (diag && tid < 42) {
-    const int a = tid - 36;
-    const double s = ((part[tid][0] + part[tid][1]) + part[tid][2]) + part[tid][3];
-    const double v = bp[6 * (size_t)i1 + a] - s;
-    bs[6 * i1 + a] = v;
-    if (St) ldltm::image_put_rhs(St, n, 6 * i1 + a, v);
+      const int r = 6 * i1 + a, cc = 6 * i1 + c;
+      if (St) {
+        const int p0 = ldltm::tile_image_pos(r, cc);
+        if (p0 >= 0) St[p0] = v;
+      } else {
+        S[(size_t)r * n + cc] = v;
+      }
+    } else if (tid < 42) {
+      const int a = tid - 36, u = 21 + a;
+      const double s = ((part[u][0] + part[u][1]) + part[u][2]) + part[u][3];
+      const double v = bp[6 * (size_t)i1 + a] - s;
+      bs[6 * i1 + a] = v;
+      if (St) ldltm::image_put_rhs(St, n, 6 * i1 + a, v);
+    }
+  } else {
+    double acc[36];
+#pragma unroll
+    for (int i = 0; i < 36; i++) acc[i] = 0;
+    for (int j = j0 + tid; j < j1; j += kSchurThreads) {
+      const PairItem it = items[j];
+      double Dinv[9];
+      inv3_sym(Hll + 6 * (size_t)it.l, lambda, Dinv);
+      const double* Bi = EB + (size_t)it.ea * kEB;
+      const double* Bj = EB + (size_t)it.eb * kEB;
+      double BD[18];
+#pragma unroll
+      for (int a = 0; a < 6; a++)
+#pragma unroll
+        for (int c = 0; c < 3; c++) BD[3 * a + c] = Bi[3 * a] * Dinv[c] + Bi[3 * a + 1] * Dinv[3 + c] + Bi[3 * a + 2] * Dinv[6 + c];
+#pragma unroll
+      for (int a = 0; a < 6; a++)
+#pragma unroll
+        for (int c = 0; c < 6; c++) acc[6 * a + c] += BD[3 * a] * Bj[3 * c] + BD[3 * a + 1] * Bj[3 * c + 1] + BD[3 * a + 2] * Bj[3 * c + 2];
+    }
+#pragma unroll
+    for (int ps = 0; ps < PASSES; ps++) {
+      if (ps == 1) __syncthreads();
+#pragma unroll
+      for (int i = 0; i < kPass; i++) {
+        const int v = ps * kPass + i;
+        if (v < 36) red[i * kRow + slot] = acc[v < 36 ? v : 0];
+      }
+      __syncthreads();
+      if (tid < 4 * kPass && ps * kPass + (tid >> 2) < 36) {
+        const int o = tid >> 2, q = tid & 3;
+        part[ps * kPass + o][q] = sum_segment(red + o * kRow + q * kSeg);
+      }
+    }
+    __syncthreads();
+    if (tid < 36) {
+      const double s = ((part[tid][0] + part[tid][1]) + part[tid][2]) + part[tid][3];
+      const int a = tid / 6, c = tid % 6;
+      const double v = -s;
+      if (St) {
+        const int r = 6 * i1 + a, cc = 6 * i2 + c;
+        const int p0 = ldltm::tile_image_pos(r, cc), p1 = ldltm::tile_image_pos(cc, r);
+        if (p0 >= 0) St[p0] = v;
+        if (p1 >= 0) St[p1] = v;
+      } else {
+        S[(size_t)(6 * i1 + a) * n + 6 * i2 + c] = v;
+        S[(size_t)(6 * i2 + c) * n + 6 * i1 + a] = v;
+      }
+    }
   }
   LBA_PROF_END();
 }
diff --git a/multi_orbslam3_amd/csrc/matcher.hip b/multi_orbslam3_amd/csrc/matcher.hip
--- a/multi_orbslam3_amd/csrc/matcher.hip
+++ b/multi_orbslam3_amd/csrc/matcher.hip
@@ -292,7 +292,7 @@
 };
 
 __device__ __forceinline__ bool feature_occupied(const FrameDev& F, int idx) {
-  if (F.use_mask) return (F.occ[idx >> 5] >> (idx & 31)) & 1u;
+  if (F.use_mask) return idx < kOccBits && ((F.occ[idx >> 5] >> (idx & 31)) & 1u);
   return F.assigned_mp[idx] >= 0 && (!F.assigned_obs || F.assigned_obs[idx] > 0);
 }
 
@@ -889,6 +889,7 @@
 }
 
 
+struct orbm_lastview;
 struct orbm_frame {
   hipStream_t own_stream = nullptr;
   bool ext_stream = false;
@@ -933,6 +934,18 @@
   PinnedBuf<uint32_t> list;
   PinnedBuf<QResult> results;
   float last_ms = 0;
+  struct EarlySearch {
+    bool pending = false;
+    bool launched = false;
+    bool stale = false;
+    bool redo_next = false;
+    orbm_lastview* view = nullptr;
+    PoseF Pc;
+    float th = 0;
+    int forward = 0, backward = 0, m = 0;
+    hipStream_t stream = nullptr;
+  } early;
+  bool n_pending = false;
 };
 
 static int frame_set_params(orbm_frame* f, const orbm_frame_view* v, int n) {
@@ -990,9 +1003,16 @@
   return ORBG_OK;
 }
 
+static void drain_early_search(orbm_frame* f) {
+  if (!f->early.pending) return;
+  if (f->early.launched) (void)f->sig.wait(f->early.stream);
+  f->early = orbm_frame::EarlySearch();
+}
+
 extern "C" int orbm_frame_destroy(orbm_frame* f) {
   if (!f) return ORBG_BAD_ARG;
   (void)hipSetDevice(f->device);
+  drain_early_search(f);
   (void)hipStreamSynchronize(f->stream);
   if (f->own_stream != f->stream) (void)hipStreamSynchronize(f->own_stream);
   f->d_kps.release(); f->d_desc.release(); f->d_uright.release(); f->d_depth.release(); f->d_cell_of.release();
@@ -1019,6 +1039,8 @@
   if (!f || !v || v->n < 0 || (v->n > 0 && (!v->kps || !v->desc))) return ORBG_BAD_ARG;
   int rc = select_device(f->device);
   if (rc) return rc;
+  drain_early_search(f);
+  f->n_pending = false;
   if ((rc = frame_set_params(f, v, v->n))) return rc;
   if ((rc = frame_reserve(f, v->n))) return rc;
   const int n = v->n;
@@ -1045,6 +1067,8 @@
   const orbx_keypoint* dk; const uint8_t* dd; const float* du; const float* dz; const orbx_keypoint* hk; int n; hipStream_t xs;
   if ((rc = orbx_internal_left_features(h, &dk, &dd, &du, &dz, &hk, &n, &xs))) return rc;
   if (v->n >= 0 && v->n != n) return ORBG_BAD_ARG;
+  drain_early_search(f);
+  f->n_pending = false;
   if ((rc = frame_set_params(f, v, n))) return rc;
   if ((rc = frame_reserve(f, n))) return rc;
   f->has_uright = true;
@@ -1061,6 +1085,9 @@
   const orbx_keypoint* dk; const uint8_t* dd; const float* du; const float* dz; const orbx_keypoint* hk; int n0; hipStream_t xs;
   int rc = orbx_internal_left_features(h, &dk, &dd, &du, &dz, &hk, &n0, &xs);
   if (rc) return rc;
+  if (f->early.redo_next) f->early.redo_next = false;
+  else drain_early_search(f);
+  f->n_pending = n < 0;
   if ((rc = frame_set_params(f, v, n < 0 ? 0 : n))) return rc;
   const int xcap = orbx_internal_kp_capacity(h);
   if (n < 0 && xcap >= ORBG_MAX_FRAME_FEATURES) return ORBG_CAP_EXCEEDED;
@@ -1085,6 +1112,11 @@
 void orbm_internal_set_n(orbm_frame* f, int n) {
   f->fp.n = n; f->hk_cached_n = -1;
   f->stream = f->own_stream;
+  f->n_pending = false;
+}
+
+void orbm_internal_early_search_void(orbm_frame* f) {
+  if (f && f->early.pending) f->early.stale = f->early.redo_next = true;
 }
 
 int orbm_internal_kf_features(orbm_frame* f, const orbx_keypoint** d_kps, const uint8_t** d_desc, const float** d_uright,
@@ -1629,12 +1661,24 @@
   }
 }
 
-template <typename LaunchFn>
-static int run_search(orbm_frame* f, int n_queries, LaunchFn launch, const volatile int* n_scan_host = nullptr) {
+static int reserve_search_buffers(orbm_frame* f, int n_queries) {
   int rc;
   if ((rc = f->results.reserve((size_t)std::max(n_queries, 1)))) return rc;
   const size_t slots = (size_t)n_queries * kSlot;
   if (f->list.cap < slots + (1 << 16) && (rc = f->list.reserve(slots + (1 << 18)))) return rc;
+  return ORBG_OK;
+}
+static size_t list_end(const orbm_frame* f, int n_scan) {
+  size_t total = 0;
+  const QResult* R = f->results.h;
+  for (int i = 0; i < n_scan; i++) total = std::max(total, (size_t)R[i].base + (size_t)(R[i].count & kQCountMask));
+  return total;
+}
+template <typename LaunchFn>
+static int run_search(orbm_frame* f, int n_queries, LaunchFn launch, const volatile int* n_scan_host = nullptr) {
+  int rc;
+  if (f->early.pending) return ORBG_BAD_ARG;
+  if ((rc = reserve_search_buffers(f, n_queries))) return rc;
   for (int attempt = 0; attempt < 3; attempt++) {
     int* cur = f->d_counter.p + (f->search_seq & 1);
     int* nxt = f->d_counter.p + ((f->search_seq + 1) & 1);
@@ -1642,10 +1686,7 @@
     launch((int)std::min<size_t>(f->list.cap, (size_t)1 << 30), cur, nxt);
     ORBG_HIP(hipGetLastError());
     if ((rc = f->sig.sync(f->stream))) return rc;
-    size_t total = 0;
-    const QResult* R = f->results.h;
-    const int n_scan = n_scan_host ? std::min((int)*n_scan_host, n_queries) : n_queries;
-    for (int i = 0; i < n_scan; i++) total = std::max(total, (size_t)R[i].base + (size_t)(R[i].count & kQCountMask));
+    const size_t total = list_end(f, n_scan_host ? std::min((int)*n_scan_host, n_queries) : n_queries);
     if (total <= f->list.cap) return ORBG_OK;
     if ((rc = f->list.reserve(total + total / 4))) return rc;
   }
@@ -1657,9 +1698,8 @@
   int rc;
   orbm_frame* fs[2] = {a, b};
   for (orbm_frame* f : fs) {
-    if ((rc = f->results.reserve((size_t)std::max(n_queries, 1)))) return rc;
-    const size_t slots = (size_t)n_queries * kSlot;
-    if (f->list.cap < slots + (1 << 16) && (rc = f->list.reserve(slots + (1 << 18)))) return rc;
+    if (f->early.pending) return ORBG_BAD_ARG;
+    if ((rc = reserve_search_buffers(f, n_queries))) return rc;
   }
   for (int k = 0; k < 2; k++) {
     orbm_frame* f = fs[k];
@@ -2077,12 +2117,8 @@
   return ORBG_OK;
 }
 
-static int search_frame_common(orbm_frame* f, const float* Tcw_cur, const float* Tcw_last, int m, LastDev L, const int32_t* n_obs_last,
-                               const float* angle_last, hipEvent_t wait_ev, float th, int mono, int check_orientation,
-                               int32_t* assigned_mp, int32_t* assigned_obs, int* nmatches_out) {
-  int rc;
-  const int n = f->fp.n;
-  hipStream_t st = f->stream;
+static void frame_search_direction(const orbm_frame* f, const float* Tcw_cur, const float* Tcw_last, int mono, PoseF* Pc_out, int* forward,
+                                   int* backward) {
   PoseF Pc, Pl;
   make_pose(Tcw_cur, &Pc);
   make_pose(Tcw_last, &Pl);
@@ -2091,14 +2127,15 @@
     const float t0 = Pl.R[3 * i] * Pc.Ow[0] + Pl.R[3 * i + 1] * Pc.Ow[1] + Pl.R[3 * i + 2] * Pc.Ow[2];
     tlc[i] = t0 + Pl.t[i];
   }
-  const int forward = tlc[2] > f->fp.b && !mono;
-  const int backward = -tlc[2] > f->fp.b && !mono;
-  if (wait_ev) ORBG_HIP(hipStreamWaitEvent(st, wait_ev, 0));
-  rc = run_search(f, m, [&](int list_cap, int* cnt, int* cnt_next) {
-    hipLaunchKernelGGL(search_frame_kernel, dim3((m + 3) / 4), dim3(256), 0, st, f->fp, frame_dev(f), L, Pc, th, forward, backward,
-                       cnt, cnt_next, f->list.d, list_cap, f->results.d);
-  });
-  if (rc) return rc;
+  *forward = tlc[2] > f->fp.b && !mono;
+  *backward = -tlc[2] > f->fp.b && !mono;
+  *Pc_out = Pc;
+}
+
+static int commit_frame_search(orbm_frame* f, int m, const int32_t* n_obs_last, const float* angle_last, int check_orientation,
+                               int32_t* assigned_mp, int32_t* assigned_obs, int* nmatches_out) {
+  int rc;
+  const int n = f->fp.n;
   cache_keypoint_fields(f);
   f->claimed_buf.assign((size_t)std::max(n, 1), 0);
   uint8_t* claimed = f->claimed_buf.data();
@@ -2128,10 +2165,27 @@
   return ORBG_OK;
 }
 
+static int search_frame_common(orbm_frame* f, const float* Tcw_cur, const float* Tcw_last, int m, LastDev L, const int32_t* n_obs_last,
+                               const float* angle_last, hipEvent_t wait_ev, float th, int mono, int check_orientation,
+                               int32_t* assigned_mp, int32_t* assigned_obs, int* nmatches_out) {
+  int rc;
+  hipStream_t st = f->stream;
+  PoseF Pc;
+  int forward, backward;
+  frame_search_direction(f, Tcw_cur, Tcw_last, mono, &Pc, &forward, &backward);
+  if (wait_ev) ORBG_HIP(hipStreamWaitEvent(st, wait_ev, 0));
+  rc = run_search(f, m, [&](int list_cap, int* cnt, int* cnt_next) {
+    hipLaunchKernelGGL(search_frame_kernel, dim3((m + 3) / 4), dim3(256), 0, st, f->fp, frame_dev(f), L, Pc, th, forward, backward,
+                       cnt, cnt_next, f->list.d, list_cap, f->results.d);
+  });
+  if (rc) return rc;
+  return commit_frame_search(f, m, n_obs_last, angle_last, check_orientation, assigned_mp, assigned_obs, nmatches_out);
+}
+
 extern "C" int orbm_search_by_projection_frame(orbm_frame* f, const float* Tcw_cur, const orbm_lastframe_view* last, float th,
                                                int mono, int check_orientation, int32_t* assigned_mp, int32_t* assigned_obs,
                                                int* nmatches_out) {
-  if (!f || !Tcw_cur || !last || !assigned_mp || !assigned_obs || last->n < 0) return ORBG_BAD_ARG;
+  if (!f || !Tcw_cur || !last || !assigned_mp || !assigned_obs || last->n < 0 || f->early.pending) return ORBG_BAD_ARG;
   int rc = select_device(f->device);
   if (rc) return rc;
   const int m = last->n;
@@ -2220,9 +2274,23 @@
   return ORBG_OK;
 }
 
+static LastDev lastview_dev(orbm_lastview* v, hipEvent_t* wait_ev) {
+  const uint8_t* A = v->arena.p;
+  LastDev L;
+  L.n = v->n;
+  L.mp_valid = A + v->o_valid; L.outlier = A + v->o_outl; L.desc = A + v->o_desc;
+  L.world_pos = reinterpret_cast<const float*>(A + v->o_pos); L.octave = reinterpret_cast<const int*>(A + v->o_oct);
+  *wait_ev = nullptr;
+  if (v->pending) {
+    if (hipEventQuery(v->ev) == hipSuccess) v->pending = false;
+    else { (void)hipGetLastError(); *wait_ev = v->ev; }
+  }
+  return L;
+}
+
 extern "C" int orbm_search_by_projection_frame_resident(orbm_frame* f, const float* Tcw_cur, orbm_lastview* v, float th, int mono,
                                                         int check_orientation, int32_t* assigned_mp, int32_t* assigned_obs, int* nmatches_out) {
-  if (!f || !Tcw_cur || !v || !assigned_mp || !assigned_obs || f->device != v->device) return ORBG_BAD_ARG;
+  if (!f || !Tcw_cur || !v || !assigned_mp || !assigned_obs || f->device != v->device || f->early.pending) return ORBG_BAD_ARG;
   int rc = select_device(f->device);
   if (rc) return rc;
   const int m = v->n;
@@ -2232,18 +2300,79 @@
   if ((rc = stage_begin(f, (size_t)n * 8))) return rc;
   stage_occupancy(f, assigned_mp, assigned_obs, n);
   if ((rc = stage_commit(f))) return rc;
-  const uint8_t* A = v->arena.p;
-  LastDev L;
-  L.n = m;
-  L.mp_valid = A + v->o_valid; L.outlier = A + v->o_outl; L.desc = A + v->o_desc;
-  L.world_pos = reinterpret_cast<const float*>(A + v->o_pos); L.octave = reinterpret_cast<const int*>(A + v->o_oct);
-  hipEvent_t wait_ev = nullptr;
-  if (v->pending) {
-    if (hipEventQuery(v->ev) == hipSuccess) v->pending = false;
-    else { (void)hipGetLastError(); wait_ev = v->ev; }
-  }
+  hipEvent_t wait_ev;
+  const LastDev L = lastview_dev(v, &wait_ev);
   return search_frame_common(f, Tcw_cur, v->Tcw, m, L, v->n_obs.data(), v->angle.data(), wait_ev, th, mono, check_orientation, assigned_mp,
                              assigned_obs, nmatches_out);
+}
+
+static void empty_occupancy(orbm_frame* f) {
+  f->occ_mask = true;
+  memset(f->occ, 0, sizeof(f->occ));
+  f->d_assigned_mp = nullptr; f->d_assigned_obs = nullptr;
+}
+
+extern "C" int orbm_search_by_projection_frame_resident_submit(orbm_frame* f, const float* Tcw_cur, orbm_lastview* v, float th, int mono) {
+  if (!f || !Tcw_cur || !v || f->device != v->device || f->early.pending) return ORBG_BAD_ARG;
+  int rc = select_device(f->device);
+  if (rc) return rc;
+  orbm_frame::EarlySearch e;
+  e.view = v; e.m = v->n; e.th = th; e.stream = f->stream;
+  frame_search_direction(f, Tcw_cur, v->Tcw, mono, &e.Pc, &e.forward, &e.backward);
+  if (e.m > 0) {
+    const int m = e.m;
+    empty_occupancy(f);
+    hipEvent_t wait_ev;
+    const LastDev L = lastview_dev(v, &wait_ev);
+    if (wait_ev) ORBG_HIP(hipStreamWaitEvent(e.stream, wait_ev, 0));
+    if ((rc = reserve_search_buffers(f, m))) return rc;
+    int* cur = f->d_counter.p + (f->search_seq & 1);
+    int* nxt = f->d_counter.p + ((f->search_seq + 1) & 1);
+    f->search_seq++;
+    hipLaunchKernelGGL(search_frame_kernel, dim3((m + 3) / 4), dim3(256), 0, e.stream, f->fp, frame_dev(f), L, e.Pc, th, e.forward, e.backward,
+                       cur, nxt, f->list.d, (int)std::min<size_t>(f->list.cap, (size_t)1 << 30), f->results.d);
+    ORBG_HIP(hipGetLastError());
+    if ((rc = f->sig.post(e.stream))) return rc;
+    e.launched = true;
+  }
+  e.pending = true;
+  f->early = e;
+  return ORBG_OK;
+}
+
+extern "C" int orbm_search_by_projection_frame_resident_collect(orbm_frame* f, int check_orientation, int32_t* assigned_mp,
+                                                                int32_t* assigned_obs, int* nmatches_out) {
+  if (!f || !assigned_mp || !assigned_obs || !f->early.pending || f->n_pending) return ORBG_BAD_ARG;
+  int rc = select_device(f->device);
+  if (rc) return rc;
+  const orbm_frame::EarlySearch e = f->early;
+  if (nmatches_out) *nmatches_out = 0;
+  if (e.launched) rc = f->sig.wait(e.stream);
+  f->early = orbm_frame::EarlySearch();
+  if (rc || e.m == 0) return rc;
+  orbm_lastview* v = e.view;
+  const int m = e.m;
+  bool again = e.stale;
+  if (!again) {
+    const size_t total = list_end(f, m);
+    if (total > f->list.cap) {
+      if ((rc = f->list.reserve(total + total / 4))) return rc;
+      again = true;
+    }
+  }
+  if (again) {
+    hipStream_t st = f->stream;
+    empty_occupancy(f);
+    hipEvent_t wait_ev;
+    const LastDev L = lastview_dev(v, &wait_ev);
+    if (wait_ev) ORBG_HIP(hipStreamWaitEvent(st, wait_ev, 0));
+    rc = run_search(f, m, [&](int list_cap, int* cnt, int* cnt_next) {
+      hipLaunchKernelGGL(search_frame_kernel, dim3((m + 3) / 4), dim3(256), 0, st, f->fp, frame_dev(f), L, e.Pc, e.th, e.forward, e.backward,
+                         cnt, cnt_next, f->list.d, list_cap, f->results.d);
+    });
+    if (rc) return rc;
+  }
+  return commit_frame_search(f, m, v->n_obs.data(), v->angle.data(), check_orientation, assigned_mp, assigned_obs, nmatches_out);
 }
 
 static int bow_common(orbm_frame* f, const orbm_featvec_view* fvF, const uint8_t* t_valid, const uint8_t* kf_desc, int nkf,
```
